# mp3guy/Kintinuous

Measured on AMD Instinct MI355X. Metric: RGB-D frames/sec @640x480, 512^3 TSDF, higher is better.
Workload: dtype f32; 1 GPU; orbit512: 640x480 synthetic orbit sequence, ICP-only tracking, 512^3 TSDF, inputs resident in HBM, 1 stream per GPU (BASELINE.json configs[1]), log playback with 1 frame of read-ahead; volume=512, cols=640, rows=480, unique_frames=120, pose_gather_bytes=56384, side_gate=0, odometry_fallbacks=0

## Files before the change

kintinuous_amd/abi.py:

```python
from __future__ import annotations

import ctypes as C
import os
from typing import Optional, Sequence, Tuple

import numpy as np

_HERE = os.path.dirname(os.path.abspath(__file__))
LIB_PATH = os.environ.get("KT_HIP_LIB") or os.path.join(_HERE, "libkt_hip.so")

KT_OK = 0
KT_ERR_CAPACITY = 5


class KtError(RuntimeError):
    def __init__(self, msg: str, status: int = 0):
        super().__init__(msg)
        self.status = status


class Intr(C.Structure):
    _fields_ = [("fx", C.c_float), ("fy", C.c_float), ("cx", C.c_float), ("cy", C.c_float)]

    def level(self, l: int) -> "Intr":
        d = np.float32(1 << l)
        return Intr(np.float32(self.fx) / d, np.float32(self.fy) / d, np.float32(self.cx) / d, np.float32(self.cy) / d)


class Mat33(C.Structure):
    _fields_ = [("m", C.c_float * 9)]

    @staticmethod
    def from_np(a) -> "Mat33":
        a = np.asarray(a, dtype=np.float32).reshape(9)
        return Mat33((C.c_float * 9)(*a.tolist()))


class LoopIcpInfo(C.Structure):
    _fields_ = [("n_source", C.c_int), ("n_target", C.c_int), ("iterations", C.c_int), ("converged", C.c_int)]


class LoopMatchParams(C.Structure):
    _fields_ = [("fast_threshold", C.c_int), ("max_keypoints", C.c_int), ("max_hamming", C.c_int), ("ratio_num", C.c_int), ("ratio_den", C.c_int),
                ("n_hypotheses", C.c_int), ("reproj_px", C.c_float), ("max_dist", C.c_float), ("seed", C.c_uint32)]


class LoopMatchInfo(C.Structure):
    _fields_ = [("n_kp_old", C.c_int), ("n_kp_new", C.c_int), ("n_matches", C.c_int), ("n_inliers", C.c_int), ("best_hypothesis", C.c_int)]


class JpegLayout(C.Structure):
    _fields_ = [("width", C.c_int32), ("height", C.c_int32), ("ncomp", C.c_int32), ("hmax", C.c_int32), ("vmax", C.c_int32),
                ("h", C.c_int32 * 3), ("v", C.c_int32 * 3), ("tq", C.c_int32 * 3), ("blocks_w", C.c_int32 * 3), ("blocks_h", C.c_int32 * 3),
                ("comp_width", C.c_int32 * 3), ("comp_height", C.c_int32 * 3), ("coef_offset", C.c_uint32 * 3), ("n_coef", C.c_uint32),
                ("qt", (C.c_uint16 * 64) * 4)]


class TrackerConfig(C.Structure):
    _fields_ = [
        ("cols", C.c_int), ("rows", C.c_int), ("N", C.c_int),
        ("fx", C.c_float), ("fy", C.c_float), ("cx", C.c_float), ("cy", C.c_float),
        ("volume_size", C.c_float), ("voxel_shift", C.c_int), ("overlap", C.c_int), ("static_mode", C.c_int),
        ("use_rgbd", C.c_int), ("use_rgbd_icp", C.c_int), ("fast_odometry", C.c_int), ("disable_color_angle", C.c_int),
        ("max_slice_points", C.c_int), ("dynamic_cube", C.c_int), ("place_recognition", C.c_int),
    ]


DATATERM_DTYPE = np.dtype([("zero", np.int16, 2), ("one", np.int16, 2), ("diff", np.float32), ("valid", np.uint8), ("pad", np.uint8, 3)])
POINT_DTYPE = np.dtype([("xyz", np.float32, 3), ("pad0", np.float32), ("bgra", np.uint8, 4), ("pad1", np.uint32, 3)])
MESH_VERTEX_DTYPE = np.dtype([("xyz", np.float32, 3), ("rgb", np.uint32)])
assert DATATERM_DTYPE.itemsize == 16 and POINT_DTYPE.itemsize == 32 and MESH_VERTEX_DTYPE.itemsize == 16

_vp, _i, _f, _d, _sz, _u64 = C.c_void_p, C.c_int, C.c_float, C.c_double, C.c_size_t, C.c_uint64
_pf = C.POINTER(C.c_float)
_pd = C.POINTER(C.c_double)
_pi = C.POINTER(C.c_int)
_pI = C.POINTER(Intr)
_pM = C.POINTER(Mat33)

_PROTOS = {
    "kt_last_error": (C.c_char_p, []),
    "kt_version": (C.c_char_p, []),
    "kt_device_count": (_i, [_pi]),
    "kt_ctx_create": (_i, [_i, C.POINTER(_vp)]),
    "kt_ctx_destroy": (_i, [_vp]),
    "kt_ctx_set_stream": (_i, [_vp, _vp]),
    "kt_ctx_stream": (_vp, [_vp]),
    "kt_sync": (_i, [_vp]),
    "kt_malloc": (_i, [_vp, _sz, C.POINTER(_vp)]),
    "kt_free": (_i, [_vp, _vp]),
    "kt_memset": (_i, [_vp, _vp, _i, _sz]),
    "kt_upload": (_i, [_vp, _vp, _vp, _sz]),
    "kt_download": (_i, [_vp, _vp, _vp, _sz]),
    "kt_upload2d": (_i, [_vp, _vp, _vp, _sz, _sz, _i]),
    "kt_download2d": (_i, [_vp, _vp, _sz, _vp, _sz, _i]),
    "kt_bilateral_filter": (_i, [_vp, _vp, _vp, _i, _i]),
    "kt_pyr_down": (_i, [_vp, _vp, _i, _i, _vp]),
    "kt_create_vmap": (_i, [_vp, _pI, _vp, _i, _i, _vp]),
    "kt_create_nmap": (_i, [_vp, _vp, _i, _i, _vp]),
    "kt_transform_maps": (_i, [_vp, _vp, _vp, _i, _i, _pM, _pf, _vp, _vp]),
    "kt_resize_vmap": (_i, [_vp, _vp, _i, _i, _vp]),
    "kt_resize_nmap": (_i, [_vp, _vp, _i, _i, _vp]),
    "kt_generate_image": (_i, [_vp, _vp, _vp, _vp, _i, _i, _pf, _i, _vp, _vp]),
    "kt_generate_depth": (_i, [_vp, _pM, _pf, _vp, _vp, _i, _i, _vp]),
    "kt_depth_to_metres": (_i, [_vp, _vp, _vp, _i, _i, _i]),
    "kt_bgr_to_intensity": (_i, [_vp, _vp, _vp, _i, _i]),
    "kt_pyr_down_gauss_f32": (_i, [_vp, _vp, _i, _i, _vp]),
    "kt_pyr_down_gauss_u8": (_i, [_vp, _vp, _i, _i, _vp]),
    "kt_derivative_images": (_i, [_vp, _vp, _i, _i, _vp, _vp]),
    "kt_project_to_cloud": (_i, [_vp, _vp, _i, _i, _vp, _d, _d, _d, _d, _i]),
    "kt_build_pyramid": (_i, [_vp, _pI, _vp, _i, _i, C.POINTER(_vp), C.POINTER(_vp), C.POINTER(_vp)]),
    "kt_icp_step": (_i, [_vp, _pM, _pf, _vp, _vp, _pM, _pf, _pI, _vp, _vp, _i, _i, _f, _f, _pf, _pf, _pf]),
    "kt_rgb_residual": (_i, [_vp, _f, _vp, _vp, _vp, _vp, _vp, _vp, _i, _i, _vp, _f, _pf, _pM, _pi, _pi]),
    "kt_rgb_step": (_i, [_vp, _vp, _f, _vp, _f, _f, _vp, _vp, _f, _i, _i, _pf, _pf]),
    "kt_init_volume": (_i, [_vp, _vp, _i]),
    "kt_init_color_volume": (_i, [_vp, _vp, _i]),
    "kt_icp_track": (_i, [_vp, C.POINTER(_vp), C.POINTER(_vp), C.POINTER(_vp), C.POINTER(_vp), _i, _i, _pI, _pM, _pf, _pi, _f, _f, _pM, _pf, _pf, _pf]),
    "kt_integrate_tsdf": (_i, [_vp, _vp, _i, _i, _pI, _pf, _pM, _pf, _f, _vp, _vp, _pi, _vp, _vp, _vp, _i, _i]),
    "kt_raycast": (_i, [_vp, _pI, _pM, _pf, _f, _pf, _vp, _vp, _vp, _i, _i, _pi, _vp, _vp, _i]),
    "kt_clear_volume": (_i, [_vp, _vp, _i, _i, _i, _i, _i, _i]),
    "kt_extract_cloud_slice": (_i, [_vp, _vp, _pf, _vp, _sz, _pi, _vp, _i, _i, _i, _i, _i, _i, _i, _pi, _i, C.POINTER(_sz)]),
    "kt_extract_mesh": (_i, [_vp, _vp, _pf, _pi, _vp, _pi, _pi, _pi, _i, _vp, _sz, _vp, _sz, C.POINTER(_sz), C.POINTER(_sz)]),
    "kt_tracker_create": (_i, [_vp, C.POINTER(TrackerConfig), C.POINTER(_vp)]),
    "kt_tracker_destroy": (_i, [_vp]),
    "kt_tracker_reset": (_i, [_vp]),
    "kt_tracker_process_frame": (_i, [_vp, _vp, _vp, _u64]),
    "kt_tracker_process_frame_host": (_i, [_vp, _vp, _vp, _u64]),
    "kt_tracker_load_trajectory": (_i, [_vp, _i, _vp, _vp]),
    "kt_tracker_finalise": (_i, [_vp]),
    "kt_tracker_get_volume_basis": (_i, [_vp, _pf]),
    "kt_host_reposition_cube": (None, [_pf, _pf, _f, _pf, _i, _pf]),
    "kt_tracker_get_pose": (_i, [_vp, _pf, _pf, _pf]),
    "kt_tracker_num_poses": (_i, [_vp]),
    "kt_tracker_get_dense_pose": (_i, [_vp, _i, C.POINTER(_u64), _pf, _pi]),
    "kt_tracker_get_voxel_wrap": (_i, [_vp, _pi]),
    "kt_tracker_num_slices": (_i, [_vp]),
    "kt_tracker_slice_info": (_i, [_vp, _i, C.POINTER(_sz), _pi]),
    "kt_tracker_slice_points": (_i, [_vp, _i, _vp]),
    "kt_tracker_volume": (_vp, [_vp]),
    "kt_tracker_color_volume": (_vp, [_vp]),
    "kt_tracker_vmap_g_prev": (_vp, [_vp, _i]),
    "kt_tracker_vmap_curr_color": (_vp, [_vp]),
    "kt_tracker_nmap_g_prev": (_vp, [_vp, _i]),
    "kt_tracker_trunc_dist": (_f, [_vp]),
    "kt_tracker_enable_profiling": (_i, [_vp, _i]),
    "kt_tracker_stage_ms": (_i, [_vp, _pf]),
    "kt_tracker_stage_counts": (_i, [_vp, C.POINTER(C.c_longlong)]),
    "kt_tracker_enable_counts": (_i, [_vp, _i]),
    "kt_tracker_last_counts": (_i, [_vp, C.POINTER(C.c_ulonglong), C.POINTER(C.c_ulonglong)]),
    "kt_tracker_debug_counts": (_i, [_vp, C.POINTER(C.c_uint)]),
    "kt_tracker_debug_state": (_i, [_vp, _pf]),
    "kt_tracker_debug_bricks": (_i, [_vp, _vp]),
    "kt_tracker_plan_stats": (_i, [_vp, C.POINTER(C.c_longlong)]),
    "kt_tracker_odometry_fallbacks": (_i, [_vp, C.POINTER(C.c_longlong)]),
    "kt_debug_wait_limit": (_i, [_vp, C.c_uint]),
    "kt_tracker_debug_side_gate": (_i, [_vp]),
    "kt_tracker_enable_slice_stage": (_i, [_vp, _i, _i, _i]),
    "kt_tracker_slice_processed_info": (_i, [_vp, _i, C.POINTER(C.c_longlong)]),
    "kt_tracker_slice_processed": (_i, [_vp, _i, _vp]),
    "kt_tracker_enable_mesh_stage": (_i, [_vp, _i, C.c_longlong, C.c_longlong]),
    "kt_tracker_slice_mesh_info": (_i, [_vp, _i, C.POINTER(C.c_longlong), C.POINTER(C.c_longlong)]),
    "kt_tracker_slice_mesh": (_i, [_vp, _i, _vp, _vp]),
    "kt_tracker_debug_pose_log": (_i, [_vp, _i, _pf, _i, C.POINTER(C.c_int)]),
    "kt_tracker_debug_plan_truth": (_i, [_vp, _pf, _i, C.c_float, C.c_float, C.c_float, C.c_float, C.c_uint]),
    "kt_debug_tsdf_lean": (_i, [_i]),
    "kt_debug_tsdf_kernel": (C.c_char_p, []),
    "kt_debug_tsdf_contract": (_i, [_i]),
    "kt_debug_tsdf_wcl": (_i, [_i]),
    "kt_debug_tsdf_wcl_pick": (_i, [_i, _i, _i, _i]),
    "kt_debug_sq_threshold": (_f, [_f, _i]),
    "kt_debug_icp_levels": (_i, [_i]),
    "kt_debug_ri_levels": (_i, [_i]),
    "kt_tracker_debug_icp_levels": (_i, [_vp]),
    "kt_debug_icp_wg_times": (_i, [_vp, C.POINTER(C.c_ulonglong)]),
    "kt_debug_tsdf_timeline": (_i, [_vp, C.POINTER(C.c_ulonglong), _i]),
    "kt_debug_solve_check": (_i, [_vp, _i, _vp, _vp, _vp, C.POINTER(_i)]),
    "kt_debug_unpack_table": (_i, [_vp, _pf]),
    "kt_debug_rcp_check": (_i, [_vp, C.POINTER(C.c_uint)]),
    "kt_debug_handoff_fault": (_i, [_vp, _i, _i, C.c_uint, C.POINTER(C.c_uint)]),
    "kt_tracker_num_pr_samples": (_i, [_vp]),
    "kt_tracker_pr_sample": (_i, [_vp, _i, C.POINTER(_u64), _pf, _pf, C.POINTER(C.c_int)]),
    "kt_tracker_slice_pr_id": (_i, [_vp, _i, C.POINTER(C.c_int)]),
    "kt_host_place_recognition_movement": (_f, [_pf, _pf, _pf, _pf]),
    "kt_slice_process": (_i, [_vp, _vp, _sz, _i, _f, _i, _vp, C.POINTER(_sz)]),
    "kt_slice_ws_create": (_i, [_vp, _sz, _vp, C.POINTER(_vp)]),
    "kt_slice_ws_destroy": (_i, [_vp]),
    "kt_slice_ws_stream": (_vp, [_vp]),
    "kt_slice_process_device": (_i, [_vp, _vp, _vp, _sz, _i, _f, _i]),
    "kt_slice_ws_count": (_i, [_vp, C.POINTER(_sz)]),
    "kt_slice_ws_output": (_vp, [_vp]),
    "kt_host_voxel_grid_normal": (_i, [_vp, _sz, _f, _vp, C.POINTER(_sz)]),
    "kt_host_save_pcd": (_i, [C.c_char_p, _vp, _sz]),
    "kt_host_save_ply": (_i, [C.c_char_p, _vp, _sz, _vp, _sz]),
    "kt_comm_unique_id": (_i, [C.POINTER(C.c_ubyte)]),
    "kt_comm_init": (_i, [_vp, _i, _i, C.POINTER(C.c_ubyte), C.POINTER(_vp)]),
    "kt_pose_gather": (_i, [_vp, _vp, _i, _pf]),
    "kt_comm_barrier": (_i, [_vp]),
    "kt_comm_destroy": (_i, [_vp]),
    "kt_tracker_host_times": (_i, [_vp, _pd, _i]),
    "kt_tracker_prefetch_frame": (_i, [_vp, _vp, _vp]),
    "kt_tracker_prefetch_frame_host": (_i, [_vp, _vp, _vp]),
    "kt_tracker_slice_pose": (_i, [_vp, _i, _pf, _pf, C.POINTER(_u64)]),
    "kt_tracker_set_parked": (_i, [_vp, _i]),
    "kt_host_ldlt_solve6": (_i, [_pd, _pd, _pd]),
    "kt_host_rodrigues": (_i, [_pd, _pd]),
    "kt_host_mat33_inverse": (_i, [_pf, _pf]),
    "kt_host_pose_update": (_i, [_pd, _pd, _pf, _pf, _pf, _pf]),
    "kt_host_compute_krk": (_i, [_pd, C.c_double, C.c_double, C.c_double, C.c_double, _pf, _pf]),
    "kt_host_trajectory_pose": (None, [_pf, _pf]),
    "kt_host_ground_truth_pose": (None, [_pf, _pf, _pf, _pf, _pf, _pf]),
    "kt_tracker_export_poses_device": (_i, [_vp, _i, _vp]),
    "kt_loop_icp_depth_frames": (_i, [_vp, _vp, _vp, _i, _i, _pI, _pf, _f, _f, _i, _pf, _pf, _vp]),
    "kt_depth_to_cloud_grid": (_i, [_vp, _vp, _i, _i, _pI, _f, _f, _vp, _sz, C.POINTER(_sz)]),
    "kt_cloud_nearest": (_i, [_vp, _vp, _sz, _vp, _sz, _vp, _vp]),
    "kt_host_rigid_fit": (_i, [_pd, _d, _pd]),
    "kt_loop_match_params_default": (_i, [_vp]),
    "kt_loop_match_frames": (_i, [_vp, _vp, _vp, _vp, _vp, _i, _i, _pI, _vp, _pf, _pf, _vp, _vp, _sz, _vp]),
    "kt_frame_keypoints": (_i, [_vp, _vp, _vp, _i, _i, _vp, _vp, _vp, _vp, _sz, C.POINTER(_sz)]),
    "kt_descriptor_match": (_i, [_vp, _vp, _sz, _vp, _sz, _vp, _vp, _vp, _vp]),
    "kt_host_jpeg_entropy_decode": (_i, [_vp, _sz, _i, _i, _vp, _vp, _sz, C.POINTER(_sz)]),
    "kt_jpeg_ws_create": (_i, [_vp, _i, _i, _vp, C.POINTER(_vp)]),
    "kt_jpeg_ws_destroy": (_i, [_vp]),
    "kt_jpeg_ws_stream": (_vp, [_vp]),
    "kt_jpeg_ws_order": (_i, [_vp, _vp]),
    "kt_jpeg_reconstruct": (_i, [_vp, _vp, _vp, _i, _vp]),
    "kt_jpeg_decode": (_i, [_vp, _vp, _sz, _i, _i, _i, _vp]),
}

ABI_SYMBOLS = tuple(_PROTOS.keys())

_MEASURE_PROTOS = {
    "kt_debug_stream": (_i, [_vp, _vp, _sz, _i, _i]),
    "kt_debug_stream_rows": (_i, [_vp, _vp, _i, _i, _i, _i, _i]),
    "kt_debug_valu_rates": (_i, [_vp, _i, _i, _i, _pd]),
    "kt_debug_div_check": (_i, [_vp, C.POINTER(C.c_uint)]),
    "kt_debug_brick_count": (_i, [_i]),
    "kt_debug_integrate_bricks": (_i, [_vp, _vp, _i, _i, _pI, _pf, _pM, _pf, _f, _vp, _vp, _pi, _vp, _vp, _vp, _i, _i, _vp]),
    "kt_debug_raycast_bricks": (_i, [_vp, _pI, _pM, _pf, _f, _pf, _vp, _vp, _vp, _i, _i, _pi, _vp, _vp, _i, _vp, C.POINTER(C.c_ulonglong)]),
}
MEASURE_SYMBOLS = tuple(_MEASURE_PROTOS.keys())
MEASURE_LIB_PATH = os.path.join(os.path.dirname(os.path.abspath(__file__)), "libkt_debug.so")
_mlib = None


def measure_lib() -> C.CDLL:
    global _mlib
    if _mlib is None:
        lib()
        if not os.path.exists(MEASURE_LIB_PATH):
            raise KtError(f"{MEASURE_LIB_PATH} not found: run `python -c 'import __graft_entry__ as g; g.build()'` first")
        l = C.CDLL(MEASURE_LIB_PATH, mode=C.RTLD_GLOBAL)
        for name, (res, args) in _MEASURE_PROTOS.items():
            f = getattr(l, name)
            f.restype, f.argtypes = res, args
        _mlib = l
    return _mlib

_lib = None


def lib() -> C.CDLL:
    global _lib
    if _lib is None:
        if not os.path.exists(LIB_PATH):
            raise KtError(f"{LIB_PATH} not found: run `python -c 'import __graft_entry__ as g; g.build()'` first")
        l = C.CDLL(LIB_PATH, mode=C.RTLD_GLOBAL)
        for name, (res, args) in _PROTOS.items():
            if name.startswith("kt_debug_") and os.environ.get("KT_HIP_LIB") and not hasattr(l, name):
                continue
            fn = getattr(l, name)
            fn.restype = res
            fn.argtypes = args
        _lib = l
    return _lib


def _chk(status: int) -> None:
    if status != KT_OK:
        raise KtError(f"kt status {status}: {lib().kt_last_error().decode(errors='replace')}", status)


def _fp(a) -> "C.Array":
    a = np.ascontiguousarray(a, dtype=np.float32).reshape(-1)
    return (C.c_float * a.size)(*a.tolist())


def _ip(a) -> "C.Array":
    a = np.ascontiguousarray(a, dtype=np.int32).reshape(-1)
    return (C.c_int * a.size)(*a.tolist())


def _count(n: int) -> int:
    if n < 0:
        raise KtError(lib().kt_last_error().decode() or "tracker error")
    return n


class DevBuf:

    def __init__(self, ctx: "Ctx", nbytes: int, ptr: Optional[int] = None):
        self.ctx, self.nbytes = ctx, int(nbytes)
        self.owned = ptr is None
        if ptr is None:
            p = _vp()
            _chk(lib().kt_malloc(ctx.h, self.nbytes, C.byref(p)))
            ptr = p.value
        self.ptr = ptr

    def free(self) -> None:
        if self.owned and self.ptr:
            lib().kt_free(self.ctx.h, self.ptr)
            self.ptr = None

    def __del__(self):
        try:
            self.free()
        except Exception:
            pass


class Ctx:

    def __init__(self, device: int = 0):
        h = _vp()
        _chk(lib().kt_ctx_create(device, C.byref(h)))
        self.h = h
        self.device = device

    def close(self) -> None:
        if self.h:
            lib().kt_ctx_destroy(self.h)
            self.h = None

    def sync(self) -> None:
        _chk(lib().kt_sync(self.h))

    def empty(self, nbytes: int) -> DevBuf:
        return DevBuf(self, nbytes)

    def zeros(self, nbytes: int) -> DevBuf:
        b = DevBuf(self, nbytes)
        _chk(lib().kt_memset(self.h, b.ptr, 0, nbytes))
        return b

    def upload(self, a: np.ndarray, into: Optional[DevBuf] = None) -> DevBuf:
        a = np.ascontiguousarray(a)
        b = into if into is not None else DevBuf(self, a.nbytes)
        _chk(lib().kt_upload(self.h, b.ptr, a.ctypes.data, a.nbytes))
        return b

    def download(self, b, dtype, shape) -> np.ndarray:
        out = np.empty(shape, dtype=dtype)
        ptr = b.ptr if isinstance(b, DevBuf) else int(b)
        _chk(lib().kt_download(self.h, out.ctypes.data, ptr, out.nbytes))
        return out

    def bilateral_filter(self, src: DevBuf, dst: DevBuf, cols: int, rows: int) -> None:
        _chk(lib().kt_bilateral_filter(self.h, src.ptr, dst.ptr, cols, rows))

    def pyr_down(self, src: DevBuf, scols: int, srows: int, dst: DevBuf) -> None:
        _chk(lib().kt_pyr_down(self.h, src.ptr, scols, srows, dst.ptr))

    def create_vmap(self, intr: Intr, depth: DevBuf, cols: int, rows: int, vmap: DevBuf) -> None:
        _chk(lib().kt_create_vmap(self.h, C.byref(intr), depth.ptr, cols, rows, vmap.ptr))

    def create_nmap(self, vmap: DevBuf, cols: int, rows: int, nmap: DevBuf) -> None:
        _chk(lib().kt_create_nmap(self.h, vmap.ptr, cols, rows, nmap.ptr))

    def transform_maps(self, vs, ns, cols, rows, R, t, vd, nd) -> None:
        _chk(lib().kt_transform_maps(self.h, vs.ptr, ns.ptr, cols, rows, C.byref(Mat33.from_np(R)), _fp(t), vd.ptr, nd.ptr))

    def resize_vmap(self, src, in_cols, in_rows, dst) -> None:
        _chk(lib().kt_resize_vmap(self.h, src.ptr, in_cols, in_rows, dst.ptr))

    def resize_nmap(self, src, in_cols, in_rows, dst) -> None:
        _chk(lib().kt_resize_nmap(self.h, src.ptr, in_cols, in_rows, dst.ptr))

    def generate_image(self, vmap, nmap, vmap_color, cols, rows, light_pos, light_number, dst, dst_color) -> None:
        _chk(lib().kt_generate_image(self.h, vmap.ptr, nmap.ptr, vmap_color.ptr, cols, rows, _fp(light_pos), light_number, dst.ptr, dst_color.ptr))

    def generate_depth(self, R_inv, t, vmap, nmap, cols, rows, dst) -> None:
        _chk(lib().kt_generate_depth(self.h, C.byref(Mat33.from_np(R_inv)), _fp(t), vmap.ptr, nmap.ptr, cols, rows, dst.ptr))

    def depth_to_metres(self, src, dst, cols, rows, cutoff) -> None:
        _chk(lib().kt_depth_to_metres(self.h, src.ptr, dst.ptr, cols, rows, cutoff))

    def bgr_to_intensity(self, src, dst, cols, rows) -> None:
        _chk(lib().kt_bgr_to_intensity(self.h, src.ptr, dst.ptr, cols, rows))

    def pyr_down_gauss_f32(self, src, scols, srows, dst) -> None:
        _chk(lib().kt_pyr_down_gauss_f32(self.h, src.ptr, scols, srows, dst.ptr))

    def pyr_down_gauss_u8(self, src, scols, srows, dst) -> None:
        _chk(lib().kt_pyr_down_gauss_u8(self.h, src.ptr, scols, srows, dst.ptr))

    def derivative_images(self, src, cols, rows, dx, dy) -> None:
        _chk(lib().kt_derivative_images(self.h, src.ptr, cols, rows, dx.ptr, dy.ptr))

    def project_to_cloud(self, depth, cols, rows, cloud, fx, fy, cx, cy, level) -> None:
        _chk(lib().kt_project_to_cloud(self.h, depth.ptr, cols, rows, cloud.ptr, fx, fy, cx, cy, level))

    def build_pyramid(self, intr: Intr, depth0, cols, rows, depths_out, vmaps, nmaps) -> None:
        d = (_vp * 3)(*[b.ptr for b in depths_out])
        v = (_vp * 4)(*[b.ptr for b in vmaps])
        n = (_vp * 4)(*[b.ptr for b in nmaps])
        _chk(lib().kt_build_pyramid(self.h, C.byref(intr), depth0.ptr, cols, rows, d, v, n))

    def icp_step(self, Rcurr, tcurr, vmap_curr, nmap_curr, Rprev_inv, tprev, intr: Intr, vmap_g_prev, nmap_g_prev, cols, rows,
                 dist_thres, angle_thres) -> Tuple[np.ndarray, np.ndarray, np.ndarray]:
        A = (C.c_float * 36)()
        b = (C.c_float * 6)()
        r = (C.c_float * 2)()
        _chk(lib().kt_icp_step(self.h, C.byref(Mat33.from_np(Rcurr)), _fp(tcurr), vmap_curr.ptr, nmap_curr.ptr,
                               C.byref(Mat33.from_np(Rprev_inv)), _fp(tprev), C.byref(intr), vmap_g_prev.ptr, nmap_g_prev.ptr,
                               cols, rows, dist_thres, angle_thres, A, b, r))
        return (np.array(A, dtype=np.float32).reshape(6, 6), np.array(b, dtype=np.float32), np.array(r, dtype=np.float32))

    def icp_track(self, vmaps_curr, nmaps_curr, vmaps_g_prev, nmaps_g_prev, cols, rows, intr: Intr, Rprev, tprev, iterations,
                  dist_thres, angle_thres):
        def arr(bufs):
            return (_vp * 4)(*[(b.ptr if b is not None else None) for b in bufs])
        Rc = Mat33()
        tc, A, r = (C.c_float * 3)(), (C.c_float * 36)(), (C.c_float * 2)()
        it = (C.c_int * 4)(*[int(v) for v in iterations])
        _chk(lib().kt_icp_track(self.h, arr(vmaps_curr), arr(nmaps_curr), arr(vmaps_g_prev), arr(nmaps_g_prev), cols, rows, C.byref(intr),
                                C.byref(Mat33.from_np(Rprev)), _fp(tprev), it, dist_thres, angle_thres, C.byref(Rc), tc, A, r))
        return (np.array(Rc.m, np.float32).reshape(3, 3), np.array(tc, np.float32), np.array(A, np.float32).reshape(6, 6), np.array(r, np.float32))

    def rgb_residual(self, min_scale, dIdx, dIdy, last_depth, next_depth, last_image, next_image, cols, rows, corres,
                     max_depth_delta, kt, krkinv) -> Tuple[int, int]:
        sigma, count = C.c_int(0), C.c_int(0)
        _chk(lib().kt_rgb_residual(self.h, min_scale, dIdx.ptr, dIdy.ptr, last_depth.ptr, next_depth.ptr, last_image.ptr,
                                   next_image.ptr, cols, rows, corres.ptr, max_depth_delta, _fp(kt),
                                   C.byref(Mat33.from_np(krkinv)), C.byref(sigma), C.byref(count)))
        return sigma.value, count.value

    def rgb_step(self, corres, sigma, cloud, fx, fy, dIdx, dIdy, sobel_scale, cols, rows) -> Tuple[np.ndarray, np.ndarray]:
        A = (C.c_float * 36)()
        b = (C.c_float * 6)()
        _chk(lib().kt_rgb_step(self.h, corres.ptr, sigma, cloud.ptr, fx, fy, dIdx.ptr, dIdy.ptr, sobel_scale, cols, rows, A, b))
        return np.array(A, dtype=np.float32).reshape(6, 6), np.array(b, dtype=np.float32)

    def init_volume(self, vol: DevBuf, N: int) -> None:
        _chk(lib().kt_init_volume(self.h, vol.ptr, N))

    def init_color_volume(self, cvol: DevBuf, N: int) -> None:
        _chk(lib().kt_init_color_volume(self.h, cvol.ptr, N))

    def integrate_tsdf(self, depth, cols, rows, intr: Intr, volume_size, Rcurr_inv, tcurr, tranc_dist, volume, depth_scaled,
                       voxel_wrap, color_volume, colors, nmap_curr, angle_color, N) -> None:
        _chk(lib().kt_integrate_tsdf(self.h, depth.ptr, cols, rows, C.byref(intr), _fp(volume_size), C.byref(Mat33.from_np(Rcurr_inv)),
                                     _fp(tcurr), tranc_dist, volume.ptr, depth_scaled.ptr, _ip(voxel_wrap), color_volume.ptr,
                                     colors.ptr, nmap_curr.ptr, int(angle_color), N))

    def raycast(self, intr: Intr, Rcurr, tcurr, tranc_dist, volume_size, volume, vmap, nmap, cols, rows, voxel_wrap, vmap_color,
                color_volume, N) -> None:
        _chk(lib().kt_raycast(self.h, C.byref(intr), C.byref(Mat33.from_np(Rcurr)), _fp(tcurr), tranc_dist, _fp(volume_size),
                              volume.ptr, vmap.ptr, nmap.ptr, cols, rows, _ip(voxel_wrap), vmap_color.ptr, color_volume.ptr, N))

    def integrate_tsdf_bricks(self, depth, cols, rows, intr: Intr, volume_size, Rcurr_inv, tcurr, tranc_dist, volume, depth_scaled,
                              voxel_wrap, color_volume, colors, nmap_curr, angle_color, N, bricks) -> None:
        _chk(measure_lib().kt_debug_integrate_bricks(self.h, depth.ptr, cols, rows, C.byref(intr), _fp(volume_size), C.byref(Mat33.from_np(Rcurr_inv)),
                                                     _fp(tcurr), tranc_dist, volume.ptr, depth_scaled.ptr, _ip(voxel_wrap), color_volume.ptr,
                                                     colors.ptr, nmap_curr.ptr, int(angle_color), N, bricks.ptr if bricks is not None else None))

    def raycast_bricks(self, intr: Intr, Rcurr, tcurr, tranc_dist, volume_size, volume, vmap, nmap, cols, rows, voxel_wrap, vmap_color,
                       color_volume, N, bricks) -> Tuple[int, int, int, int]:
        counts = (C.c_ulonglong * 4)()
        _chk(measure_lib().kt_debug_raycast_bricks(self.h, C.byref(intr), C.byref(Mat33.from_np(Rcurr)), _fp(tcurr), tranc_dist, _fp(volume_size),
                                                   volume.ptr, vmap.ptr, nmap.ptr, cols, rows, _ip(voxel_wrap), vmap_color.ptr, color_volume.ptr, N,
                                                   bricks.ptr if bricks is not None else None, counts))
        return tuple(int(v) for v in counts)

    def clear_volume(self, vol, elem_size, N, axis, back, current_wrap, delta_wrap) -> None:
        _chk(lib().kt_clear_volume(self.h, vol.ptr, elem_size, N, axis, int(back), current_wrap, delta_wrap))

    def extract_cloud_slice(self, volume, volume_size, out: DevBuf, cap: int, voxel_wrap, color_volume, minX, maxX, minY, maxY,
                            minZ, maxZ, subsample, real_voxel_wrap, N) -> int:
        n = _sz(0)
        _chk(lib().kt_extract_cloud_slice(self.h, volume.ptr, _fp(volume_size), out.ptr, cap, _ip(voxel_wrap), color_volume.ptr,
                                          minX, maxX, minY, maxY, minZ, maxZ, subsample, _ip(real_voxel_wrap), N, C.byref(n)))
        return int(n.value)

    def extract_mesh(self, volume, volume_size, voxel_wrap, color_volume, lo, hi, real_voxel_wrap, N, vertices=None, v_cap: int = 0,
                     triangles=None, t_cap: int = 0):
        nv, nt = _sz(0), _sz(0)
        vp = vertices.ptr if isinstance(vertices, DevBuf) else vertices
        tp = triangles.ptr if isinstance(triangles, DevBuf) else triangles
        vol = volume.ptr if isinstance(volume, DevBuf) else volume
        col = color_volume.ptr if isinstance(color_volume, DevBuf) else color_volume
        s = lib().kt_extract_mesh(self.h, vol, _fp(volume_size), _ip(voxel_wrap), col, _ip(lo), _ip(hi), _ip(real_voxel_wrap), N, vp,
                                  v_cap, tp, t_cap, C.byref(nv), C.byref(nt))
        if s not in (KT_OK, KT_ERR_CAPACITY):
            _chk(s)
        return s, int(nv.value), int(nt.value)

    def mesh(self, volume, volume_size, voxel_wrap, color_volume, lo, hi, real_voxel_wrap, N):
        s, nv, nt = self.extract_mesh(volume, volume_size, voxel_wrap, color_volume, lo, hi, real_voxel_wrap, N)
        vb = DevBuf(self, max(nv, 1) * 16)
        tb = DevBuf(self, max(nt, 1) * 12)
        try:
            s, nv2, nt2 = self.extract_mesh(volume, volume_size, voxel_wrap, color_volume, lo, hi, real_voxel_wrap, N, vb, nv, tb, nt)
            _chk(s)
            assert (nv2, nt2) == (nv, nt)
            v = np.zeros(max(nv, 1), MESH_VERTEX_DTYPE)
            t = np.zeros((max(nt, 1), 3), np.uint32)
            _chk(lib().kt_download(self.h, v.ctypes.data_as(C.c_void_p), vb.ptr, nv * 16))
            _chk(lib().kt_download(self.h, t.ctypes.data_as(C.c_void_p), tb.ptr, nt * 12))
        finally:
            vb.free()
            tb.free()
        return v[:nv], t[:nt]


    def depth_to_cloud_grid(self, frame: np.ndarray, intr: Intr, leaf: float, max_dist: float = 4.0, capacity: Optional[int] = None, out=None):
        frame = np.ascontiguousarray(frame, np.uint16)
        rows, cols = frame.shape
        cap = rows * cols if capacity is None else int(capacity)
        buf = out if out is not None else np.zeros((max(cap, 1), 3), np.float32)
        n = _sz(0)
        s = lib().kt_depth_to_cloud_grid(self.h, frame.ctypes.data, cols, rows, C.byref(intr), float(leaf), float(max_dist), buf.ctypes.data, cap, C.byref(n))
        if s not in (KT_OK, KT_ERR_CAPACITY):
            _chk(s)
        return s, (buf[: n.value] if s == KT_OK else None), int(n.value)

    def cloud_nearest(self, src: np.ndarray, dst: np.ndarray):
        src = np.ascontiguousarray(src, np.float32).reshape(-1, 3)
        dst = np.ascontiguousarray(dst, np.float32).reshape(-1, 3)
        idx, d2 = np.zeros(max(len(src), 1), np.uint32), np.zeros(max(len(src), 1), np.float32)
        _chk(lib().kt_cloud_nearest(self.h, src.ctypes.data, len(src), dst.ctypes.data, len(dst), idx.ctypes.data, d2.ctypes.data))
        return idx[: len(src)], d2[: len(src)]

    def loop_icp_depth_frames(self, frame1: np.ndarray, frame2: np.ndarray, intr: Intr, bootstrap, leaf: float, max_dist: float = 4.0,
                              max_iterations: int = 10):
        frame1, frame2 = np.ascontiguousarray(frame1, np.uint16), np.ascontiguousarray(frame2, np.uint16)
        assert frame1.shape == frame2.shape and frame1.ndim == 2
        rows, cols = frame1.shape
        M, score, info = (C.c_float * 16)(), C.c_float(0), LoopIcpInfo()
        _chk(lib().kt_loop_icp_depth_frames(self.h, frame1.ctypes.data, frame2.ctypes.data, cols, rows, C.byref(intr), _fp(np.asarray(bootstrap).reshape(16)),
                                            float(leaf), float(max_dist), int(max_iterations), M, C.byref(score), C.byref(info)))
        return (np.array(M, np.float32).reshape(4, 4), float(score.value),
                dict(n_source=info.n_source, n_target=info.n_target, iterations=info.iterations, converged=bool(info.converged)))

    def frame_keypoints(self, rgb: np.ndarray, depth: np.ndarray, params: Optional[LoopMatchParams] = None, capacity: Optional[int] = None):
        params = params or loop_match_params()
        depth = np.ascontiguousarray(depth, np.uint16)
        rows, cols = depth.shape
        rgb = np.ascontiguousarray(rgb, np.uint8).reshape(rows, cols, 3)
        cap = params.max_keypoints if capacity is None else int(capacity)
        uv, score, desc = np.full((max(cap, 1), 2), -7, np.int32), np.full(max(cap, 1), -7, np.int32), np.full((max(cap, 1), 8), 7, np.uint32)
        n = _sz(0)
        s = lib().kt_frame_keypoints(self.h, rgb.ctypes.data, depth.ctypes.data, cols, rows, C.byref(params), uv.ctypes.data, score.ctypes.data, desc.ctypes.data,
                                     cap, C.byref(n))
        if s not in (KT_OK, KT_ERR_CAPACITY):
            _chk(s)
        if s == KT_ERR_CAPACITY:
            assert (uv == -7).all() and (score == -7).all() and (desc == 7).all()
            return s, None, int(n.value)
        return s, (uv[: n.value], score[: n.value], desc[: n.value]), int(n.value)

    def descriptor_match(self, desc_new: np.ndarray, desc_old: np.ndarray, params: Optional[LoopMatchParams] = None):
        params = params or loop_match_params()
        dn = np.ascontiguousarray(desc_new, np.uint32).reshape(-1, 8)
        do = np.ascontiguousarray(desc_old, np.uint32).reshape(-1, 8)
        idx, d1, d2 = (np.zeros(max(len(dn), 1), np.int32) for _ in range(3))
        _chk(lib().kt_descriptor_match(self.h, dn.ctypes.data, len(dn), do.ctypes.data, len(do), C.byref(params), idx.ctypes.data, d1.ctypes.data, d2.ctypes.data))
        return idx[: len(dn)], d1[: len(dn)], d2[: len(dn)]

    def loop_match_frames(self, rgb_old, depth_old, rgb_new, depth_new, intr: Intr, params: Optional[LoopMatchParams] = None):
        params = params or loop_match_params()
        depth_old, depth_new = np.ascontiguousarray(depth_old, np.uint16), np.ascontiguousarray(depth_new, np.uint16)
        assert depth_old.shape == depth_new.shape and depth_old.ndim == 2
        rows, cols = depth_old.shape
        rgb_old, rgb_new = (np.ascontiguousarray(a, np.uint8).reshape(rows, cols, 3) for a in (rgb_old, rgb_new))
        cap = params.max_keypoints
        pose, boot, info = (C.c_float * 16)(), (C.c_float * 16)(), LoopMatchInfo()
        matches, inlier = np.zeros((cap, 4), np.int32), np.zeros(cap, np.uint8)
        _chk(lib().kt_loop_match_frames(self.h, rgb_old.ctypes.data, depth_old.ctypes.data, rgb_new.ctypes.data, depth_new.ctypes.data, cols, rows, C.byref(intr),
                                        C.byref(params), pose, boot, matches.ctypes.data, inlier.ctypes.data, cap, C.byref(info)))
        n = info.n_matches
        return dict(pose=np.array(pose, np.float32).reshape(4, 4), bootstrap=np.array(boot, np.float32).reshape(4, 4), matches=matches[:n].copy(),
                    inlier=inlier[:n].astype(bool), info={k: int(getattr(info, k)) for k, _ in LoopMatchInfo._fields_})


def loop_match_params(**kw) -> LoopMatchParams:
    p = LoopMatchParams()
    _chk(lib().kt_loop_match_params_default(C.byref(p)))
    for k, v in kw.items():
        assert hasattr(p, k), k
        setattr(p, k, v)
    return p


class Tracker:

    STAGES = ("pyramid", "odometry", "shift", "integrate", "raycast", "resize", "tsdf23")

    def __init__(self, ctx: Ctx, cfg: TrackerConfig):
        self.ctx, self.cfg = ctx, cfg
        h = _vp()
        _chk(lib().kt_tracker_create(ctx.h, C.byref(cfg), C.byref(h)))
        self.h = h

    def close(self) -> None:
        if self.h:
            lib().kt_tracker_destroy(self.h)
            self.h = None

    def __del__(self):
        try:
            self.close()
        except Exception:
            pass

    def reset(self) -> None:
        _chk(lib().kt_tracker_reset(self.h))

    def process_frame(self, depth_dev, rgb_dev, timestamp: int) -> None:
        d = depth_dev.ptr if isinstance(depth_dev, DevBuf) else int(depth_dev)
        r = rgb_dev.ptr if isinstance(rgb_dev, DevBuf) else int(rgb_dev)
        _chk(lib().kt_tracker_process_frame(self.h, d, r, timestamp))

    def host_times(self, reset: bool = False):
        o = (C.c_double * 2)()
        _chk(lib().kt_tracker_host_times(self.h, o, 1 if reset else 0))
        return float(o[0]), float(o[1])

    def enable_slice_stage(self, on: bool, weight_cull: int = 8, k: int = 20) -> None:
        _chk(lib().kt_tracker_enable_slice_stage(self.h, int(on), int(weight_cull), int(k)))

    def slice_processed(self, i: int):
        n = C.c_longlong(0)
        _chk(lib().kt_tracker_slice_processed_info(self.h, i, C.byref(n)))
        if n.value < 0:
            return None
        out = np.zeros(max(int(n.value), 1), NPOINT_DTYPE)
        _chk(lib().kt_tracker_slice_processed(self.h, i, out.ctypes.data_as(C.c_void_p)))
        return out[: int(n.value)]

    def enable_mesh_stage(self, on: bool, max_vertices: int = 0, max_triangles: int = 0) -> None:
        _chk(lib().kt_tracker_enable_mesh_stage(self.h, int(on), int(max_vertices), int(max_triangles)))

    def slice_mesh_info(self, i: int):
        nv, nt = C.c_longlong(0), C.c_longlong(0)
        _chk(lib().kt_tracker_slice_mesh_info(self.h, i, C.byref(nv), C.byref(nt)))
        return int(nv.value), int(nt.value)

    def slice_mesh(self, i: int):
        nv, nt = self.slice_mesh_info(i)
        if nv < 0:
            return None
        v = np.zeros(max(nv, 1), MESH_VERTEX_DTYPE)
        t = np.zeros((max(nt, 1), 3), np.uint32)
        _chk(lib().kt_tracker_slice_mesh(self.h, i, v.ctypes.data_as(C.c_void_p), t.ctypes.data_as(C.c_void_p)))
        return v[:nv], t[:nt]

    def pose_log(self, enable: Optional[bool] = None, fetch: bool = False):
        if not fetch:
            _chk(lib().kt_tracker_debug_pose_log(self.h, -1 if enable is None else int(enable), None, 0, None))
            return None
        n = C.c_int(0)
        _chk(lib().kt_tracker_debug_pose_log(self.h, -1 if enable is None else int(enable), None, 0, C.byref(n)))
        out = np.zeros((n.value, 12), np.float32)
        if n.value:
            _chk(lib().kt_tracker_debug_pose_log(self.h, -1, out.ctypes.data_as(_pf), n.value, None))
        return out

    def plan_truth(self, poses12, fr: float, ft: float, theta_fixed: float = 0.0, tau_fixed: float = 0.0, seed: int = 1) -> None:
        p = np.ascontiguousarray(poses12, np.float32).reshape(-1, 12)
        _chk(lib().kt_tracker_debug_plan_truth(self.h, p.ctypes.data_as(_pf), len(p), fr, ft, theta_fixed, tau_fixed, seed))

    def plan_stats(self) -> Tuple[int, int]:
        out = (C.c_longlong * 2)()
        _chk(lib().kt_tracker_plan_stats(self.h, out))
        return int(out[0]), int(out[1])

    def odometry_fallbacks(self) -> int:
        out = C.c_longlong(0)
        _chk(lib().kt_tracker_odometry_fallbacks(self.h, C.byref(out)))
        return int(out.value)

    def prefetch_frame(self, depth_dev, rgb_dev) -> None:
        d = depth_dev.ptr if isinstance(depth_dev, DevBuf) else int(depth_dev)
        r = rgb_dev.ptr if isinstance(rgb_dev, DevBuf) else int(rgb_dev)
        _chk(lib().kt_tracker_prefetch_frame(self.h, d, r))

    def prefetch_frame_host(self, depth: np.ndarray, rgb: np.ndarray) -> None:
        assert depth.dtype == np.uint16 and rgb.dtype == np.uint8 and depth.flags.c_contiguous and rgb.flags.c_contiguous
        _chk(lib().kt_tracker_prefetch_frame_host(self.h, depth.ctypes.data, rgb.ctypes.data))

    def process_frame_host(self, depth: np.ndarray, rgb: np.ndarray, timestamp: int) -> None:
        depth = np.ascontiguousarray(depth, dtype=np.uint16)
        rgb = np.ascontiguousarray(rgb, dtype=np.uint8)
        _chk(lib().kt_tracker_process_frame_host(self.h, depth.ctypes.data, rgb.ctypes.data, timestamp))

    def load_trajectory(self, utimes, pose7) -> None:
        utimes = np.ascontiguousarray(utimes, dtype=np.uint64)
        pose7 = np.ascontiguousarray(pose7, dtype=np.float32).reshape(-1, 7)
        assert len(utimes) == len(pose7)
        _chk(lib().kt_tracker_load_trajectory(self.h, len(utimes), utimes.ctypes.data, pose7.ctypes.data))

    def finalise(self) -> None:
        _chk(lib().kt_tracker_finalise(self.h))

    def volume_basis(self) -> np.ndarray:
        b = (C.c_float * 3)()
        _chk(lib().kt_tracker_get_volume_basis(self.h, b))
        return np.array(b, dtype=np.float32)

    def pose(self) -> Tuple[np.ndarray, np.ndarray, np.ndarray]:
        R, t, g = (C.c_float * 9)(), (C.c_float * 3)(), (C.c_float * 3)()
        _chk(lib().kt_tracker_get_pose(self.h, R, t, g))
        return np.array(R, dtype=np.float32).reshape(3, 3), np.array(t, dtype=np.float32), np.array(g, dtype=np.float32)

    def num_poses(self) -> int:
        return _count(lib().kt_tracker_num_poses(self.h))

    def dense_pose(self, i: int) -> Tuple[int, np.ndarray, bool]:
        ts, p, il = _u64(0), (C.c_float * 16)(), C.c_int(0)
        _chk(lib().kt_tracker_get_dense_pose(self.h, i, C.byref(ts), p, C.byref(il)))
        return ts.value, np.array(p, dtype=np.float32).reshape(4, 4), bool(il.value)

    def voxel_wrap(self) -> np.ndarray:
        w = (C.c_int * 3)()
        _chk(lib().kt_tracker_get_voxel_wrap(self.h, w))
        return np.array(w, dtype=np.int32)

    def num_slices(self) -> int:
        return _count(lib().kt_tracker_num_slices(self.h))

    def slice_info(self, i: int) -> Tuple[int, int]:
        n, dim = _sz(0), C.c_int(0)
        _chk(lib().kt_tracker_slice_info(self.h, i, C.byref(n), C.byref(dim)))
        return n.value, dim.value

    def slice(self, i: int) -> Tuple[np.ndarray, int]:
        n, dim = _sz(0), C.c_int(0)
        _chk(lib().kt_tracker_slice_info(self.h, i, C.byref(n), C.byref(dim)))
        out = np.zeros(n.value, dtype=POINT_DTYPE)
        if n.value:
            _chk(lib().kt_tracker_slice_points(self.h, i, out.ctypes.data))
        return out, dim.value

    def pr_samples(self):
        out = []
        for i in range(_count(lib().kt_tracker_num_pr_samples(self.h))):
            ut, tr, ro, pi = _u64(0), (C.c_float * 3)(), (C.c_float * 9)(), C.c_int(0)
            _chk(lib().kt_tracker_pr_sample(self.h, i, C.byref(ut), tr, ro, C.byref(pi)))
            out.append((ut.value, np.array(tr, np.float32), np.array(ro, np.float32).reshape(3, 3), pi.value))
        return out

    def slice_pr_id(self, i: int) -> int:
        v = C.c_int(0)
        _chk(lib().kt_tracker_slice_pr_id(self.h, i, C.byref(v)))
        return v.value

    def volume(self) -> np.ndarray:
        N = self.cfg.N
        return self.ctx.download(lib().kt_tracker_volume(self.h), np.int16, (N, N, N))

    def color_volume(self) -> np.ndarray:
        N = self.cfg.N
        return self.ctx.download(lib().kt_tracker_color_volume(self.h), np.uint8, (N, N, N, 4))

    def vmap_g_prev(self, level: int = 0) -> np.ndarray:
        c, r = self.cfg.cols >> level, self.cfg.rows >> level
        return self.ctx.download(lib().kt_tracker_vmap_g_prev(self.h, level), np.float32, (3 * r, c))

    def nmap_g_prev(self, level: int = 0) -> np.ndarray:
        c, r = self.cfg.cols >> level, self.cfg.rows >> level
        return self.ctx.download(lib().kt_tracker_nmap_g_prev(self.h, level), np.float32, (3 * r, c))

    def trunc_dist(self) -> float:
        return float(lib().kt_tracker_trunc_dist(self.h))

    def enable_profiling(self, mode: int) -> None:
        _chk(lib().kt_tracker_enable_profiling(self.h, mode))

    def stage_ms(self) -> dict:
        ms = (C.c_float * 7)()
        n = (C.c_longlong * 7)()
        _chk(lib().kt_tracker_stage_ms(self.h, ms))
        _chk(lib().kt_tracker_stage_counts(self.h, n))
        return {k: (float(ms[i]), int(n[i])) for i, k in enumerate(self.STAGES)}

    def enable_counts(self, on: bool) -> None:
        _chk(lib().kt_tracker_enable_counts(self.h, int(on)))

    def last_counts(self) -> Tuple[int, int]:
        U, S = C.c_ulonglong(0), C.c_ulonglong(0)
        _chk(lib().kt_tracker_last_counts(self.h, C.byref(U), C.byref(S)))
        return int(U.value), int(S.value)

    def debug_state(self):
        o = (C.c_float * 29)()
        _chk(lib().kt_tracker_debug_state(self.h, o))
        return [float(v) for v in o]

    def debug_bricks(self) -> np.ndarray:
        nb = (self.cfg.N + 31) // 32
        out = np.zeros((nb, nb, nb), np.uint8)
        _chk(lib().kt_tracker_debug_bricks(self.h, out.ctypes.data))
        return out

    def debug_counts(self):
        o = (C.c_uint * 8)()
        _chk(lib().kt_tracker_debug_counts(self.h, o))
        return [int(v) for v in o]

    def export_poses_device(self, k: int, dst_ptr: int) -> None:
        _chk(lib().kt_tracker_export_poses_device(self.h, k, dst_ptr))


def _dp(a):
    return a.ctypes.data_as(_pd)


def host_ldlt_solve6(A, b) -> np.ndarray:
    A = np.ascontiguousarray(A, np.float64).reshape(36)
    b = np.ascontiguousarray(b, np.float64).reshape(6)
    x = np.zeros(6, np.float64)
    _chk(lib().kt_host_ldlt_solve6(_dp(A), _dp(b), _dp(x)))
    return x


def host_rodrigues(r) -> np.ndarray:
    r = np.ascontiguousarray(r, np.float64).reshape(3)
    R = np.zeros(9, np.float64)
    _chk(lib().kt_host_rodrigues(_dp(r), _dp(R)))
    return R.reshape(3, 3)


def host_mat33_inverse(m) -> np.ndarray:
    m = np.ascontiguousarray(m, np.float32).reshape(9)
    o = np.zeros(9, np.float32)
    _chk(lib().kt_host_mat33_inverse(m.ctypes.data_as(_pf), o.ctypes.data_as(_pf)))
    return o.reshape(3, 3)


def host_reposition_cube(R, tlast, volume_size, voxel_size, thresh, basis) -> np.ndarray:
    R = np.ascontiguousarray(R, np.float32).reshape(9)
    t = np.ascontiguousarray(tlast, np.float32)
    v = np.ascontiguousarray(voxel_size, np.float32)
    b = np.ascontiguousarray(basis, np.float32).copy()
    lib().kt_host_reposition_cube(R.ctypes.data_as(_pf), t.ctypes.data_as(_pf), float(volume_size), v.ctypes.data_as(_pf), int(thresh), b.ctypes.data_as(_pf))
    return b


def host_pose_update(x, result_rt, Rprev, tprev):
    x = np.ascontiguousarray(x, np.float64).reshape(6)
    rt = np.array(result_rt, np.float64).reshape(16).copy()
    Rp = np.ascontiguousarray(Rprev, np.float32).reshape(9)
    tp = np.ascontiguousarray(tprev, np.float32).reshape(3)
    Rc, tc = np.zeros(9, np.float32), np.zeros(3, np.float32)
    _chk(lib().kt_host_pose_update(_dp(x), _dp(rt), Rp.ctypes.data_as(_pf), tp.ctypes.data_as(_pf),
                                   Rc.ctypes.data_as(_pf), tc.ctypes.data_as(_pf)))
    return rt.reshape(4, 4), Rc.reshape(3, 3), tc


def host_rigid_fit(sums, n) -> np.ndarray:
    sums = np.ascontiguousarray(sums, np.float64).reshape(15)
    dM = np.zeros(16, np.float64)
    _chk(lib().kt_host_rigid_fit(_dp(sums), float(n), _dp(dM)))
    return dM.reshape(4, 4)


NPOINT_DTYPE = np.dtype([("xyz", np.float32, 3), ("one", np.float32), ("normal", np.float32, 3), ("zero", np.float32), ("bgra", np.uint8, 4),
                         ("curvature", np.float32), ("pad", np.float32, 2)])
assert NPOINT_DTYPE.itemsize == 48


def host_compute_krk(result_rt, fx, fy, cx, cy):
    rt = np.ascontiguousarray(result_rt, np.float64).reshape(16)
    krk, kt = np.zeros(9, np.float32), np.zeros(3, np.float32)
    _chk(lib().kt_host_compute_krk(_dp(rt), float(fx), float(fy), float(cx), float(cy), krk.ctypes.data_as(_pf), kt.ctypes.data_as(_pf)))
    return krk.reshape(3, 3), kt


def host_trajectory_pose(pose7) -> np.ndarray:
    p = np.ascontiguousarray(pose7, np.float32).reshape(7)
    T = np.zeros(12, np.float32)
    lib().kt_host_trajectory_pose(p.ctypes.data_as(_pf), T.ctypes.data_as(_pf))
    return T


def host_ground_truth_pose(A, B, Rlast, tlast):
    A, B = np.ascontiguousarray(A, np.float32).reshape(12), np.ascontiguousarray(B, np.float32).reshape(12)
    Rl, tl = np.ascontiguousarray(Rlast, np.float32).reshape(9), np.ascontiguousarray(tlast, np.float32).reshape(3)
    R, t = np.zeros(9, np.float32), np.zeros(3, np.float32)
    lib().kt_host_ground_truth_pose(A.ctypes.data_as(_pf), B.ctypes.data_as(_pf), Rl.ctypes.data_as(_pf), tl.ctypes.data_as(_pf),
                                    R.ctypes.data_as(_pf), t.ctypes.data_as(_pf))
    return R.reshape(3, 3), t


def slice_process(ctx: "Ctx", points: np.ndarray, weight_cull: int, leaf: float, k: int = 20) -> np.ndarray:
    points = np.ascontiguousarray(points)
    assert points.dtype == POINT_DTYPE
    out = np.zeros(max(len(points), 1), NPOINT_DTYPE)
    n = C.c_size_t(0)
    _chk(lib().kt_slice_process(ctx.h, points.ctypes.data_as(C.c_void_p), len(points), int(weight_cull), float(leaf), int(k),
                                out.ctypes.data_as(C.c_void_p), C.byref(n)))
    return out[: n.value]


def voxel_grid_normal(points: np.ndarray, leaf: float) -> np.ndarray:
    points = np.ascontiguousarray(points)
    assert points.dtype == NPOINT_DTYPE
    out = np.zeros(max(len(points), 1), NPOINT_DTYPE)
    n = C.c_size_t(0)
    _chk(lib().kt_host_voxel_grid_normal(points.ctypes.data_as(C.c_void_p), len(points), float(leaf), out.ctypes.data_as(C.c_void_p), C.byref(n)))
    return out[: n.value]


def save_pcd(path: str, points: np.ndarray) -> None:
    points = np.ascontiguousarray(points)
    assert points.dtype == NPOINT_DTYPE
    _chk(lib().kt_host_save_pcd(path.encode(), points.ctypes.data_as(C.c_void_p), len(points)))


def save_ply(path: str, meshes) -> None:
    if isinstance(meshes, tuple) and len(meshes) == 2 and isinstance(meshes[0], np.ndarray) and meshes[0].dtype == MESH_VERTEX_DTYPE:
        meshes = [meshes]
    vs, ts, off = [], [], 0
    for v, t in meshes:
        vs.append(np.asarray(v, MESH_VERTEX_DTYPE))
        ts.append(np.asarray(t, np.uint32).reshape(-1, 3) + np.uint32(off))
        off += len(v)
    v = np.ascontiguousarray(np.concatenate(vs) if vs else np.zeros(0, MESH_VERTEX_DTYPE))
    t = np.ascontiguousarray(np.concatenate(ts) if ts else np.zeros((0, 3), np.uint32))
    _chk(lib().kt_host_save_ply(path.encode(), v.ctypes.data_as(C.c_void_p), len(v), t.ctypes.data_as(C.c_void_p), len(t)))


class Comm:

    def __init__(self, ctx: Ctx, rank: int, nranks: int, share=None):
        ident = (C.c_ubyte * 128)()
        if rank == 0:
            _chk(lib().kt_comm_unique_id(ident))
        if share is not None:
            data = share(bytes(ident))
            ident = (C.c_ubyte * 128)(*data)
        self.h = C.c_void_p()
        self.nranks = nranks
        _chk(lib().kt_comm_init(ctx.h, rank, nranks, ident, C.byref(self.h)))

    def gather_poses(self, trk: "Tracker", k: int) -> np.ndarray:
        out = np.zeros((self.nranks, k, 16), np.float32)
        _chk(lib().kt_pose_gather(self.h, trk.h, k, out.ctypes.data_as(C.POINTER(C.c_float))))
        return out

    def barrier(self) -> None:
        _chk(lib().kt_comm_barrier(self.h))

    def close(self) -> None:
        if self.h:
            lib().kt_comm_destroy(self.h)
            self.h = None


def jpeg_entropy_decode(data: bytes, width: int, height: int, capacity: Optional[int] = None) -> Tuple[JpegLayout, np.ndarray]:
    if capacity is None:
        capacity = 3 * (-(-width // 16) * 16) * (-(-height // 16) * 16)
    layout, coef, n = JpegLayout(), np.zeros(max(capacity, 1), np.int16), _sz(0)
    buf = np.frombuffer(data, np.uint8)
    _chk(lib().kt_host_jpeg_entropy_decode(buf.ctypes.data, buf.size, width, height, C.addressof(layout), coef.ctypes.data, capacity, C.byref(n)))
    return layout, coef[:n.value]


class JpegWs:

    def __init__(self, ctx: "Ctx", max_width: int, max_height: int):
        self.ctx = ctx
        h = _vp()
        _chk(lib().kt_jpeg_ws_create(ctx.h, max_width, max_height, None, C.byref(h)))
        self.h = h

    def close(self) -> None:
        if self.h:
            lib().kt_jpeg_ws_destroy(self.h)
            self.h = None

    def sync(self) -> None:
        _chk(lib().kt_jpeg_ws_order(self.h, lib().kt_ctx_stream(self.ctx.h)))
        self.ctx.sync()

    def reconstruct(self, layout: JpegLayout, coef: np.ndarray, swap_rb: int = 0, out: Optional[DevBuf] = None) -> np.ndarray:
        coef = np.ascontiguousarray(coef, np.int16)
        n = 3 * layout.width * layout.height
        buf = out if out is not None else self.ctx.empty(n)
        _chk(lib().kt_jpeg_reconstruct(self.h, C.addressof(layout), coef.ctypes.data, swap_rb, buf.ptr))
        self.sync()
        res = self.ctx.download(buf, np.uint8, (layout.height, layout.width, 3))
        if out is None:
            buf.free()
        return res

    def decode(self, data: bytes, width: int, height: int, swap_rb: int = 0, out: Optional[DevBuf] = None) -> np.ndarray:
        src = np.frombuffer(data, np.uint8)
        buf = out if out is not None else self.ctx.empty(3 * width * height)
        try:
            _chk(lib().kt_jpeg_decode(self.h, src.ctypes.data, src.size, width, height, swap_rb, buf.ptr))
            return self.ctx.download(buf, np.uint8, (height, width, 3))
        finally:
            if out is None:
                buf.free()
```

kintinuous_amd/csrc/kt_debug.h:

```cpp
#ifndef KT_DEBUG_H
#define KT_DEBUG_H

#include "../../include/kt_abi.h"

#ifdef __cplusplus
extern "C" {
#endif

int kt_tracker_debug_counts(kt_tracker* t, unsigned int out8_host[8]);
int kt_tracker_debug_state(kt_tracker* t, float out29_host[29]);
int kt_tracker_debug_bricks(kt_tracker* t, unsigned char* out_host);
int kt_tracker_debug_pose_log(kt_tracker* trk, int enable, float* out12n, int max_frames, int* n_frames);
int kt_tracker_debug_plan_truth(kt_tracker* trk, const float* poses12n, int n_frames, float fr, float ft, float theta_fixed, float tau_fixed, unsigned int seed);
int kt_debug_tsdf_lean(int on);
int kt_debug_tsdf_contract(int tol);
int kt_debug_tsdf_wcl(int wcl);
int kt_debug_tsdf_wcl_pick(int cols, int rows, int N, int rule);
const char* kt_debug_tsdf_kernel(void);
int kt_debug_icp_wg_times(kt_ctx* ctx, unsigned long long* out768_host);
int kt_debug_tsdf_timeline(kt_ctx* ctx, unsigned long long* out_host, int max_words);
int kt_debug_solve_check(kt_ctx* ctx, int n, const void* cases_host, void* serial_out_host, void* wave_out_host, int layout_out[5]);
int kt_debug_unpack_table(kt_ctx* ctx, float* out_host65536);
int kt_debug_rcp_check(kt_ctx* ctx, unsigned int* mismatches_host);
int kt_debug_handoff_fault(kt_ctx* ctx, int skip, int count, unsigned int spin_limit, unsigned int* dirty_out);
int kt_debug_wait_limit(kt_ctx* ctx, unsigned int ticks_100mhz);
int kt_debug_icp_levels(int on);
int kt_debug_ri_levels(int on);
int kt_tracker_debug_icp_levels(kt_tracker* trk);
int kt_tracker_debug_side_gate(kt_tracker* trk);
float kt_debug_sq_threshold(float T, int strict);

#ifdef __cplusplus
}
#endif

#endif
```

kintinuous_amd/csrc/kt_tracker.hip:

```cpp
#include "kt_internal.hpp"
#include "kt_setup.hpp"

#include <limits.h>
#include <stdlib.h>
#include <string.h>

#include <array>
#include <deque>
#include <chrono>
#include <condition_variable>
#include <functional>
#include <mutex>
#include <atomic>
#include <map>
#include <thread>
#include <vector>

namespace {

struct DensePose { uint64_t ts; float pose[16]; int is_loop; };
struct Slice {
    std::vector<kt_point_xyzrgb> pts; int dim; float R[9], cam[3]; uint64_t ts; int pr_id;
    std::vector<kt_point_xyzrgbnormal> processed; bool has_processed = false;
    std::vector<kt_mesh_vertex> mesh_v; std::vector<uint32_t> mesh_t; long long mesh_nv = -1, mesh_nt = -1; bool mesh_fit = false;
};
struct PrSample { uint64_t utime; float trans[3], rot[9]; int pose_index; };

struct FrameSet {
    uint16_t* depths[KT_LEVELS];
    float *vmaps[KT_LEVELS], *nmaps[KT_LEVELS];
    void* rec;
    float* dpmax;
    float* scaled;
    float* depth_m[KT_LEVELS];
    uint8_t* image[KT_LEVELS];
    int16_t *dIdx[KT_LEVELS], *dIdy[KT_LEVELS];
    uint8_t* cand[KT_LEVELS];
    float* cloud[KT_LEVELS];
    hipEvent_t ready;
    long long user;
};
#define KT_NSETS 3

typedef kt_pose_mirror PoseMirror;
struct Pending { const uint16_t* depth; const uint8_t* rgb; int set; const uint16_t* depth_host; const uint8_t* rgb_host; };
#define KT_NSLOTS 4
#define KT_NODO 8

#ifndef KT_SIDE_GATE_DEFAULT
#define KT_SIDE_GATE_DEFAULT 2
#endif
enum { ST_PYRAMID = 0, ST_ODOMETRY, ST_SHIFT, ST_INTEGRATE, ST_RAYCAST, ST_RESIZE, ST_TSDF23, ST_COUNT };

}

static std::atomic<int> kt_live_trackers{0};
struct kt_tracker {
    kt_ctx* ctx;
    kt_tracker_config cfg;
    kt_intr intr;
    int N;
    float volume_size[3], voxel_size[3];
    float tranc_dist;
    float volume_basis[3];
    float initial_rotation[9];
    int voxel_wrap[3], v_wrap_copy[3];
    int global_time;
    uint64_t current_ts = 0;
    bool has_trajectory = false;
    std::map<int, std::array<float, 12>> trajectory;
    uint64_t gt_utime = 0;
    bool parked;
    float Rlast[9], tlast[3];
    float current_global_camera[3];
    int16_t* tsdf; uint8_t* color;
    uint16_t* depths_curr[KT_LEVELS];
    float *vmaps_curr[KT_LEVELS], *nmaps_curr[KT_LEVELS], *vmaps_g_prev[KT_LEVELS], *nmaps_g_prev[KT_LEVELS];
    uint8_t* vmap_curr_color;
    float* depth_raw_scaled;
    void* rec_curr;
    FrameSet sets[KT_NSETS];
    int last_assigned;
    std::vector<Pending> pending;
    long long frames_started;
    long long frames_observed;
    long long out_ordinal;
    hipEvent_t guard_ev;
    hipEvent_t odo_ev[8];
    long long slot_frame[KT_NSLOTS];
    hipStream_t pre_stream;
    kt_ctx pre_ctx;
    size_t cloud_cap;
    int prev_set;
    kt_dataterm* corres[KT_LEVELS];
    kt_track_state* state_dev; kt_track_state* state_host;
    uint16_t* depth_stage[KT_NSLOTS]; uint8_t* rgb_stage[KT_NSLOTS];
    uint16_t* depth_stage_host[KT_NSLOTS]; uint8_t* rgb_stage_host[KT_NSLOTS];
    hipEvent_t slot_uploaded[KT_NSLOTS];
    int next_slot;
    std::vector<DensePose> poses;
    std::deque<Slice> slices;
    struct SliceJob { bool active; bool done; size_t slice; hipError_t status; };
    SliceJob jobs[2];
    std::thread worker;
    std::mutex wmu;
    std::condition_variable wcv, wdone;
    std::deque<std::function<void()>> wq;
    bool wstop;
    kt_point_xyzrgb* cloud_host[2]; unsigned int* cloud_count_host[2]; hipEvent_t cloud_ev[2];
    int cloud_next;
    bool slice_stage; int slice_cull, slice_k;
    kt_slice_ws* slice_ws;
    kt_point_xyzrgb* cloud_dev[2]; unsigned int* cloud_count_dev[2]; hipEvent_t extracted[2];
    kt_point_xyzrgbnormal* proc_host[2]; unsigned int* proc_count_host[2];
    bool mesh_stage; size_t mesh_cap_v, mesh_cap_t;
    kt_mesh_ws* mesh_ws;
    kt_mesh_vertex* mesh_v_host[2]; uint32_t* mesh_t_host[2]; unsigned long long* mesh_count_host[2]; hipEvent_t mesh_ev[2];
    float pr_rot[9], pr_trans[3];
    std::vector<PrSample> pr_samples;
    bool outstanding; uint64_t out_ts; int out_set;
    const uint16_t* out_depth; const uint8_t* out_rgb; int out_thresh;
    bool out_speculated;
    kt_frame_params* fp_dev;
    float* wrkc_carry[2]; int carry_sel;
    struct PlanSlot { kt_tsdf_plan plan; hipEvent_t done; long long ordinal; float R[9], t[3], theta, tau; int wrap[3]; int set; const uint16_t* depth; const uint8_t* rgb; };
    bool icp_levels;
    bool last_icp_levels;
    bool counted;
    int icp_demote, icp_demote_len;
    long long odo_fallbacks;
    int out_last_set;
    hipEvent_t gate_ev; bool gate_armed; int side_gate;
    PlanSlot plans[3]; hipStream_t plan_stream;
    int plan_sel; bool plan_enabled; float plan_margin_scale;
    std::vector<float> plan_truth; float plan_fr = 0.0f, plan_ft = 0.0f, plan_theta_fixed = 0.0f, plan_tau_fixed = 0.0f; bool plan_perturb = false;
    unsigned int plan_rng = 0x9e3779b9u; std::vector<float> pose_log; bool pose_log_on = false;
    float hist_R[2][9], hist_gc[2][3]; int hist_n;
    float pred_err_t, pred_err_r;
    long long plan_hits, plan_misses;
    unsigned char* bricks;
    float *vgz_dev, *zs_dev;
    PoseMirror* mirror;
    unsigned int frame_seq;
    long long prof_frames;
    double host_wait_s, host_call_s; long long host_calls;
    int profiling; int ev_par;
    hipEvent_t ev[2][ST_COUNT][2]; bool ev_rec[2][ST_COUNT];
    double stage_ms_sum[ST_COUNT]; long long stage_n[ST_COUNT]; float stage_ms_last[ST_COUNT];
    int counting;
    unsigned int* upd_dev; unsigned long long* steps_dev;
    unsigned long long last_U, last_S;
};

static int join_slice_jobs(kt_tracker* t);
static int plan_frame(kt_tracker* t, const struct Pending& frame, long long ordinal);
static int lvl_cols(const kt_tracker* t, int l) { return t->cfg.cols >> l; }
static int lvl_rows(const kt_tracker* t, int l) { return t->cfg.rows >> l; }
static kt_intr lvl_intr(kt_intr k, int l)
{
    const int div = 1 << l;
    kt_intr r = {k.fx / div, k.fy / div, k.cx / div, k.cy / div};
    return r;
}


static thread_local hipStream_t g_alloc_stream = nullptr;
template <typename T>
static int dev_alloc(T** p, size_t count, bool zero)
{
    KT_HIP(hipMalloc((void**)p, (count ? count : 1) * sizeof(T)));
    if (zero) KT_HIP(hipMemsetAsync(*p, 0, (count ? count : 1) * sizeof(T), g_alloc_stream));
    return KT_OK;
}

static void select_set(kt_tracker* t, int q)
{
    for (int l = 0; l < KT_LEVELS; ++l) {
        t->depths_curr[l] = t->sets[q].depths[l];
        t->vmaps_curr[l] = t->sets[q].vmaps[l];
        t->nmaps_curr[l] = t->sets[q].nmaps[l];
    }
    t->depth_raw_scaled = t->sets[q].scaled;
    t->rec_curr = t->sets[q].rec;
}

static int pick_free_set(kt_tracker* t)
{
    for (int k = 1; k <= KT_NSETS; ++k) {
        const int q = (t->last_assigned + k) % KT_NSETS;
        bool taken = q == t->prev_set;
        for (const Pending& p : t->pending) taken = taken || p.set == q;
        if (!taken) return q;
    }
    return -1;
}

#ifndef KT_EV_DEVICE
#define KT_EV_DEVICE (hipEventDisableTiming | hipEventDisableSystemFence)
#endif

static int wait_frame_consumed(kt_tracker* t, hipStream_t stream, long long u)
{
    if (u < 0 || stream == t->ctx->stream) return KT_OK;
    if (u + 2 <= t->frames_observed) return KT_OK;
    if (t->has_trajectory && u + 1 < t->frames_started) {
        KT_HIP(hipStreamWaitEvent(stream, t->odo_ev[(u + 1) % KT_NODO], 0));
    } else {
        KT_HIP(hipEventRecord(t->guard_ev, t->ctx->stream));
        KT_HIP(hipStreamWaitEvent(stream, t->guard_ev, 0));
    }
    return KT_OK;
}

static float rgbd_min_scale(int l)
{
    const float min_grad[KT_LEVELS] = {12, 5, 3, 1};
    const double SOBEL_SCALE = 1.0 / pow(2.0, 3);
    return (float)(pow(min_grad[l], 2.0) / pow(SOBEL_SCALE, 2.0));
}

static int build_frame_set(kt_tracker* t, kt_ctx* cx, int q, const uint16_t* depth_raw, const uint8_t* colors)
{
    const int cols = t->cfg.cols, rows = t->cfg.rows;
    FrameSet& fs = t->sets[q];
    const bool icp = !t->has_trajectory && !(t->cfg.use_rgbd || t->cfg.use_rgbd_icp);
    const bool rgbd = !t->has_trajectory && !icp;
    static const bool fused_prepare = []() { const char* e = getenv("KT_PREPARE_FUSED"); return e ? atoi(e) != 0 : true; }();
    if (icp || t->cfg.use_rgbd_icp || !t->cfg.disable_color_angle) {
        KT_TRY(kt_bilateral_filter(cx, depth_raw, fs.depths[0], cols, rows));
        uint16_t* dl[3] = {fs.depths[1], fs.depths[2], fs.depths[3]};
        if (fused_prepare)
            KT_TRY(kt_frame_prepare(cx, &t->intr, fs.depths[0], dl, fs.vmaps, fs.nmaps, depth_raw, colors, cols, rows, !t->cfg.disable_color_angle, fs.scaled, fs.rec, fs.dpmax));
        else {
            KT_TRY(kt_build_pyramid(cx, &t->intr, fs.depths[0], cols, rows, dl, fs.vmaps, fs.nmaps));
            KT_TRY(kt_integrate_prepare(cx, depth_raw, colors, fs.nmaps[0], cols, rows, &t->intr, !t->cfg.disable_color_angle, fs.scaled, fs.rec, fs.dpmax));
        }
    } else
        KT_TRY(kt_integrate_prepare(cx, depth_raw, colors, fs.nmaps[0], cols, rows, &t->intr, !t->cfg.disable_color_angle, fs.scaled, fs.rec, fs.dpmax));
    if (rgbd) {
        KT_TRY(kt_depth_to_metres(cx, depth_raw, fs.depth_m[0], cols, rows, (int)(6.0 * 1000)));
        for (int l = 0; l + 1 < KT_LEVELS; ++l) KT_TRY(kt_pyr_down_gauss_f32(cx, fs.depth_m[l], lvl_cols(t, l), lvl_rows(t, l), fs.depth_m[l + 1]));
        KT_TRY(kt_bgr_to_intensity(cx, colors, fs.image[0], cols, rows));
        for (int l = 0; l + 1 < KT_LEVELS; ++l) KT_TRY(kt_pyr_down_gauss_u8(cx, fs.image[l], lvl_cols(t, l), lvl_rows(t, l), fs.image[l + 1]));
        const double ifx = t->intr.fx, ify = t->intr.fy, icx = t->intr.cx, icy = t->intr.cy;
        for (int l = 0; l < KT_LEVELS; ++l) {
            KT_TRY(kt_derivative_images(cx, fs.image[l], lvl_cols(t, l), lvl_rows(t, l), fs.dIdx[l], fs.dIdy[l]));
            KT_TRY(kt_rgb_residual_candidates(cx, rgbd_min_scale(l), fs.dIdx[l], fs.dIdy[l], fs.depth_m[l], fs.image[l], lvl_cols(t, l),
                                              lvl_rows(t, l), fs.cand[l]));
            KT_TRY(kt_project_to_cloud(cx, fs.depth_m[l], lvl_cols(t, l), lvl_rows(t, l), fs.cloud[l], ifx, ify, icx, icy, l));
        }
    }
    return KT_OK;
}

static void compute_global_camera(kt_tracker* t, const float* tcurr)
{
    for (int k = 0; k < 3; ++k) {
        const float initial_trans = (float)((double)t->volume_basis[k] - (double)t->cfg.volume_size * 0.5);
        t->current_global_camera[k] = initial_trans;
        t->current_global_camera[k] += (float)t->voxel_wrap[k] * t->voxel_size[k];
        if (tcurr) t->current_global_camera[k] += tcurr[k] - t->volume_basis[k];
    }
}

static void v_wrap_copy_update(kt_tracker* t)
{
    for (int k = 0; k < 3; ++k) {
        t->v_wrap_copy[k] = t->voxel_wrap[k];
        if (t->v_wrap_copy[k] < 0) t->v_wrap_copy[k] = t->N - ((-t->v_wrap_copy[k]) % t->N);
    }
}

static void push_pose(kt_tracker* t, uint64_t ts, const float* R, int is_loop)
{
    DensePose p;
    p.ts = ts;
    p.is_loop = is_loop;
    for (int i = 0; i < 16; ++i) p.pose[i] = (i % 5 == 0) ? 1.f : 0.f;
    for (int i = 0; i < 3; ++i) {
        for (int j = 0; j < 3; ++j) p.pose[i * 4 + j] = R[i * 3 + j];
        p.pose[i * 4 + 3] = t->current_global_camera[i];
    }
    t->poses.push_back(p);
}

static bool prof_all(const kt_tracker* t) { return t->profiling == 2 || t->profiling == 3; }
static bool prof_tsdf(const kt_tracker* t) { return t->profiling == 1 || t->profiling == 4 || t->profiling == 5 || t->profiling == 6; }
static int ev_begin(kt_tracker* t, int st)
{
    if (prof_all(t) || (prof_tsdf(t) && st == ST_TSDF23)) {
        KT_HIP(hipEventRecord(t->ev[t->ev_par][st][0], t->ctx->stream));
    }
    return KT_OK;
}
static int ev_end(kt_tracker* t, int st)
{
    if (prof_all(t) || (prof_tsdf(t) && st == ST_TSDF23)) {
        KT_HIP(hipEventRecord(t->ev[t->ev_par][st][1], t->ctx->stream));
        t->ev_rec[t->ev_par][st] = true;
    }
    return KT_OK;
}
static void tsdf23_hook_arm(kt_tracker* t)
{
    kt_tsdf23_hook.on = prof_all(t) || t->profiling == 4 || (t->profiling == 1 && (t->prof_frames++ % 8) == 0) || (t->profiling == 5 && (t->prof_frames++ % 4) == 0) ||
                        (t->profiling == 6 && (t->prof_frames++ % 2) == 0);
    kt_tsdf23_hook.ev[0] = t->ev[t->ev_par][ST_TSDF23][0];
    kt_tsdf23_hook.ev[1] = t->ev[t->ev_par][ST_TSDF23][1];
    if (kt_tsdf23_hook.on) t->ev_rec[t->ev_par][ST_TSDF23] = true;
}
static void ev_collect(kt_tracker* t)
{
    if (!t->profiling) return;
    for (int par = 0; par < 2; ++par)
        for (int st = 0; st < ST_COUNT; ++st)
            if (t->ev_rec[par][st] && hipEventQuery(t->ev[par][st][1]) == hipSuccess) {
                float ms = 0.f;
                if (hipEventElapsedTime(&ms, t->ev[par][st][0], t->ev[par][st][1]) == hipSuccess) {
                    t->stage_ms_sum[st] += ms;
                    t->stage_n[st] += 1;
                    t->stage_ms_last[st] = ms;
                }
                t->ev_rec[par][st] = false;
            }
}

extern "C" {

static int tracker_create_impl(kt_tracker* t, kt_ctx* ctx, const kt_tracker_config* cfg);

int kt_tracker_create(kt_ctx* ctx, const kt_tracker_config* cfg, kt_tracker** out)
{
    KT_ARG(ctx && cfg && out);
    KT_ARG(cfg->cols > 0 && cfg->rows > 0 && cfg->N > 0 && cfg->volume_size > 0);
    KT_ARG((cfg->cols % 8) == 0 && (cfg->rows % 8) == 0);
    KT_ARG(cfg->N <= 1536);
    KT_HIP(hipSetDevice(ctx->device));
    kt_tracker* t = new kt_tracker();
    const int s = tracker_create_impl(t, ctx, cfg);
    if (s != KT_OK) {
        t->ctx = ctx;
        (void)kt_tracker_destroy(t);
        return s;
    }
    *out = t;
    return KT_OK;
}

static int tracker_create_impl(kt_tracker* t, kt_ctx* ctx, const kt_tracker_config* cfg)
{
    t->ctx = ctx;
    g_alloc_stream = ctx->stream;
    t->cfg = *cfg;
    t->N = cfg->N;
    t->intr.fx = cfg->fx; t->intr.fy = cfg->fy; t->intr.cx = cfg->cx; t->intr.cy = cfg->cy;
    for (int k = 0; k < 3; ++k) {
        t->volume_size[k] = cfg->volume_size;
        t->voxel_size[k] = cfg->volume_size / (float)cfg->N;
    }
    for (int k = 0; k < 9; ++k) t->initial_rotation[k] = (k % 4 == 0) ? 1.f : 0.f;
    for (int k = 0; k < 3; ++k) t->volume_basis[k] = t->volume_size[k] * 0.5f;
    if (cfg->static_mode || cfg->dynamic_cube)
        t->volume_basis[2] = t->volume_size[2] * 0.5f - (float)(((double)t->volume_size[2] * 0.5) + (cfg->static_mode ? 0.45 : 0));
    const float default_tranc = fmaxf(0.01f, t->volume_size[0] / 100.0f);
    const float mc = fmaxf(t->voxel_size[0], fmaxf(t->voxel_size[1], t->voxel_size[2]));
    t->tranc_dist = fmaxf(default_tranc, 2.1f * mc);
    t->voxel_wrap[0] = t->voxel_wrap[1] = t->voxel_wrap[2] = 0;

    const size_t nvox = (size_t)cfg->N * cfg->N * cfg->N;
    const size_t P = (size_t)cfg->cols * cfg->rows;
    KT_TRY(dev_alloc(&t->tsdf, nvox, false));
    KT_TRY(dev_alloc(&t->color, nvox * 4, false));
    for (int l = 0; l < KT_LEVELS; ++l) {
        const size_t p = (size_t)lvl_cols(t, l) * lvl_rows(t, l);
        for (int q = 0; q < KT_NSETS; ++q) {
            KT_TRY(dev_alloc(&t->sets[q].depths[l], p, true));
            KT_TRY(dev_alloc(&t->sets[q].vmaps[l], 3 * p, true));
            KT_TRY(dev_alloc(&t->sets[q].nmaps[l], 3 * p, true));
        }
        KT_TRY(dev_alloc(&t->vmaps_g_prev[l], 3 * p, true));
        KT_TRY(dev_alloc(&t->nmaps_g_prev[l], 3 * p, true));
        const bool rgbd = cfg->use_rgbd || cfg->use_rgbd_icp;
        const size_t q = rgbd ? p : 0;
        for (int sidx = 0; sidx < KT_NSETS; ++sidx) {
            KT_TRY(dev_alloc(&t->sets[sidx].depth_m[l], q, true));
            KT_TRY(dev_alloc(&t->sets[sidx].image[l], q, true));
            KT_TRY(dev_alloc(&t->sets[sidx].dIdx[l], q, true));
            KT_TRY(dev_alloc(&t->sets[sidx].dIdy[l], q, true));
            KT_TRY(dev_alloc(&t->sets[sidx].cand[l], q, true));
            KT_TRY(dev_alloc(&t->sets[sidx].cloud[l], 3 * q, true));
        }
        KT_TRY(dev_alloc(&t->corres[l], q, true));
    }
    KT_TRY(dev_alloc(&t->vmap_curr_color, P * 4, true));
    for (int q = 0; q < KT_NSETS; ++q) {
        KT_TRY(dev_alloc(&t->sets[q].scaled, P, true));
        unsigned char* rec = nullptr;
        KT_TRY(dev_alloc(&rec, kt_integrate_rec_bytes(cfg->cols, cfg->rows), true));
        t->sets[q].rec = rec;
        unsigned char* dpm = nullptr;
        KT_TRY(dev_alloc(&dpm, kt_integrate_dpmax_bytes(cfg->cols, cfg->rows), true));
        t->sets[q].dpmax = (float*)dpm;
        KT_HIP(hipEventCreateWithFlags(&t->sets[q].ready, KT_EV_DEVICE));
        t->sets[q].user = -1;
    }
    t->frames_started = 0;
    t->cloud_next = 0;
    t->slice_stage = false; t->slice_ws = nullptr;
    t->mesh_stage = false; t->mesh_ws = nullptr; t->mesh_cap_v = t->mesh_cap_t = 0;
    for (int b = 0; b < 2; ++b) { t->mesh_v_host[b] = nullptr; t->mesh_t_host[b] = nullptr; t->mesh_count_host[b] = nullptr; t->mesh_ev[b] = nullptr; }
    for (int b = 0; b < 2; ++b) { t->cloud_dev[b] = nullptr; t->cloud_count_dev[b] = nullptr; t->extracted[b] = nullptr; t->proc_host[b] = nullptr; t->proc_count_host[b] = nullptr; }
    for (int b = 0; b < 2; ++b) { t->jobs[b].active = false; t->jobs[b].done = true; t->jobs[b].status = hipSuccess; t->cloud_host[b] = nullptr; t->cloud_count_host[b] = nullptr; t->cloud_ev[b] = nullptr; }
    t->wstop = false;
    {
        const int device = ctx->device;
        t->worker = std::thread([t, device]() {
            (void)hipSetDevice(device);
            std::unique_lock<std::mutex> lk(t->wmu);
            for (;;) {
                t->wcv.wait(lk, [t]() { return t->wstop || !t->wq.empty(); });
                if (t->wq.empty()) return;
                std::function<void()> job = std::move(t->wq.front());
                t->wq.pop_front();
                lk.unlock();
                job();
                lk.lock();
                t->wdone.notify_all();
            }
        });
    }
    t->frames_observed = 0;
    t->out_ordinal = -1;
    KT_HIP(hipEventCreateWithFlags(&t->guard_ev, KT_EV_DEVICE));
    for (int k = 0; k < KT_NODO; ++k) KT_HIP(hipEventCreateWithFlags(&t->odo_ev[k], KT_EV_DEVICE));
    for (int k = 0; k < KT_NSLOTS; ++k) t->slot_frame[k] = -1;
    KT_HIP(hipStreamCreateWithFlags(&t->pre_stream, hipStreamNonBlocking));
    KT_TRY(kt_bilateral_lut_ensure(ctx));
    t->pre_ctx = *ctx;
    t->pre_ctx.stream = t->pre_stream;
    t->pre_ctx.own_stream = false;
    t->last_assigned = KT_NSETS - 1;
    select_set(t, 0);
    t->cloud_cap = cfg->max_slice_points > 0 ? (size_t)cfg->max_slice_points : P * 3;
    for (int b = 0; b < 2; ++b) {
        KT_HIP(hipHostMalloc((void**)&t->cloud_host[b], t->cloud_cap * sizeof(kt_point_xyzrgb), hipHostMallocDefault));
        KT_HIP(hipHostMalloc((void**)&t->cloud_count_host[b], sizeof(unsigned int), hipHostMallocDefault));
        KT_HIP(hipEventCreateWithFlags(&t->cloud_ev[b], hipEventDisableTiming));
    }
    KT_TRY(dev_alloc(&t->state_dev, 1, true));
    KT_HIP(hipHostMalloc((void**)&t->state_host, sizeof(kt_track_state), hipHostMallocDefault));
    for (int k = 0; k < KT_NSLOTS; ++k) {
        KT_TRY(dev_alloc(&t->depth_stage[k], P, true));
        KT_TRY(dev_alloc(&t->rgb_stage[k], P * 3, true));
        KT_HIP(hipHostMalloc((void**)&t->depth_stage_host[k], P * sizeof(uint16_t), hipHostMallocDefault));
        KT_HIP(hipHostMalloc((void**)&t->rgb_stage_host[k], P * 3, hipHostMallocDefault));
        KT_HIP(hipEventCreateWithFlags(&t->slot_uploaded[k], hipEventDisableTiming));
    }
    t->next_slot = 0;
    KT_TRY(dev_alloc(&t->upd_dev, 16, true));
    KT_TRY(dev_alloc(&t->steps_dev, 4, true));
    t->profiling = 0;
    t->counting = 0;
    for (int par = 0; par < 2; ++par)
        for (int s = 0; s < ST_COUNT; ++s) {
            KT_HIP(hipEventCreate(&t->ev[par][s][0]));
            KT_HIP(hipEventCreate(&t->ev[par][s][1]));
            t->ev_rec[par][s] = false;
        }
    t->ev_par = 0;
    t->outstanding = false;
    t->host_wait_s = t->host_call_s = 0.0; t->host_calls = 0;
    KT_TRY(dev_alloc(&t->fp_dev, 1, true));
    KT_HIP(hipStreamCreateWithFlags(&t->plan_stream, hipStreamNonBlocking));
    t->icp_levels = kt_icp_levels_selected(ctx->device);
    t->last_icp_levels = false;
    t->icp_demote = 0; t->icp_demote_len = 64; t->odo_fallbacks = 0; t->out_last_set = -1;
    kt_live_trackers.fetch_add(1);
    t->counted = true;
    for (int k = 0; k < 3; ++k) {
        KT_TRY(kt_tsdf_plan_alloc(&t->plans[k].plan, cfg->N));
        KT_HIP(hipEventCreateWithFlags(&t->plans[k].done, KT_EV_DEVICE));
        t->plans[k].ordinal = -1; t->plans[k].set = -1; t->plans[k].depth = nullptr; t->plans[k].rgb = nullptr;
    }
    KT_HIP(hipEventCreateWithFlags(&t->gate_ev, KT_EV_DEVICE));
    t->gate_armed = false;
    {
        const char* e = getenv("KT_SIDE_GATE");
        const int mode = e ? atoi(e) : KT_SIDE_GATE_DEFAULT;
        int wcx = 0, wcy = 0, xg = 0, yg = 0;
        kt_tsdf_plan_shape(nullptr, cfg->cols, cfg->rows, cfg->N, &wcx, &wcy, &xg, &yg);
        const bool dense = wcx == 32 && (long long)cfg->cols * cfg->rows > 640LL * 480LL;
        t->side_gate = mode == 1 || (mode == 2 && dense) ? 1 : 0;
        if (mode == 2 && dense && !kt_icp_levels_forced()) t->icp_levels = false;
    }
    t->plan_enabled = getenv("KT_NO_PLAN") == nullptr;
    t->plan_margin_scale = getenv("KT_PLAN_MARGIN_SCALE") ? (float)atof(getenv("KT_PLAN_MARGIN_SCALE")) : 1.0f;
    t->plan_hits = t->plan_misses = 0;
    KT_TRY(dev_alloc(&t->bricks, kt_brick_count(cfg->N) + 16, true));
    for (int k = 0; k < 2; ++k) KT_TRY(dev_alloc(&t->wrkc_carry[k], (size_t)cfg->cols * cfg->rows, true));
    t->carry_sel = 0;
    KT_TRY(kt_integrate_tables(ctx, cfg->cols, cfg->rows, cfg->N, &t->vgz_dev, &t->zs_dev));
    KT_HIP(hipHostMalloc((void**)&t->mirror, sizeof(PoseMirror), hipHostMallocMapped | hipHostMallocCoherent));
    memset(t->mirror, 0, sizeof(PoseMirror));
    t->frame_seq = 0;
    t->prof_frames = 0;
    KT_TRY(kt_tracker_reset(t));
    {
        const int zero[3] = {0, 0, 0};
        KT_TRY(kt_extract_cloud_slice_async(ctx, t->tsdf, t->volume_size, t->cloud_host[0], t->cloud_cap, zero, t->color, 0, 1, 0, 1, 0, 1, 1, zero, t->N,
                                            &ctx->counters[1]));
        KT_TRY(kt_clear_volume(ctx, t->tsdf, 2, t->N, 0, 0, 0, 0));
        KT_TRY(kt_clear_volume(ctx, t->color, 4, t->N, 0, 0, 0, 0));
        KT_HIP(hipStreamSynchronize(ctx->stream));
    }
    return KT_OK;
}

int kt_tracker_destroy(kt_tracker* t)
{
    if (!t) return KT_OK;
    if (t->counted) kt_live_trackers.fetch_sub(1);
    (void)hipStreamSynchronize(t->ctx->stream);
    (void)join_slice_jobs(t);
    if (t->worker.joinable()) {
        { std::lock_guard<std::mutex> lk(t->wmu); t->wstop = true; }
        t->wcv.notify_all();
        t->worker.join();
    }
    (void)hipFree(t->tsdf); (void)hipFree(t->color);
    for (int l = 0; l < KT_LEVELS; ++l) {
        for (int q = 0; q < KT_NSETS; ++q) { (void)hipFree(t->sets[q].depths[l]); (void)hipFree(t->sets[q].vmaps[l]); (void)hipFree(t->sets[q].nmaps[l]); }
        (void)hipFree(t->vmaps_g_prev[l]); (void)hipFree(t->nmaps_g_prev[l]);
        for (int sidx = 0; sidx < KT_NSETS; ++sidx) {
            (void)hipFree(t->sets[sidx].depth_m[l]); (void)hipFree(t->sets[sidx].image[l]); (void)hipFree(t->sets[sidx].dIdx[l]);
            (void)hipFree(t->sets[sidx].dIdy[l]); (void)hipFree(t->sets[sidx].cloud[l]); (void)hipFree(t->sets[sidx].cand[l]);
        }
        (void)hipFree(t->corres[l]);
    }
    if (t->pre_stream) (void)hipStreamSynchronize(t->pre_stream);
    for (int q = 0; q < KT_NSETS; ++q) {
        (void)hipFree(t->sets[q].scaled); (void)hipFree(t->sets[q].rec); (void)hipFree(t->sets[q].dpmax);
        if (t->sets[q].ready) (void)hipEventDestroy(t->sets[q].ready);
    }
    if (t->guard_ev) (void)hipEventDestroy(t->guard_ev);
    for (int k = 0; k < KT_NODO; ++k)
        if (t->odo_ev[k]) (void)hipEventDestroy(t->odo_ev[k]);
    if (t->pre_stream) (void)hipStreamDestroy(t->pre_stream);
    (void)hipFree(t->vmap_curr_color);
    for (int b = 0; b < 2; ++b) {
        (void)hipHostFree(t->cloud_host[b]); (void)hipHostFree(t->cloud_count_host[b]);
        if (t->cloud_ev[b]) (void)hipEventDestroy(t->cloud_ev[b]);
        (void)hipFree(t->cloud_dev[b]); (void)hipFree(t->cloud_count_dev[b]); (void)hipHostFree(t->proc_host[b]); (void)hipHostFree(t->proc_count_host[b]);
        if (t->extracted[b]) (void)hipEventDestroy(t->extracted[b]);
    }
    if (t->slice_ws) (void)kt_slice_ws_destroy(t->slice_ws);
    for (int b = 0; b < 2; ++b) {
        (void)hipHostFree(t->mesh_v_host[b]); (void)hipHostFree(t->mesh_t_host[b]); (void)hipHostFree(t->mesh_count_host[b]);
        if (t->mesh_ev[b]) (void)hipEventDestroy(t->mesh_ev[b]);
    }
    if (t->mesh_ws) (void)kt_mesh_ws_destroy(t->mesh_ws);
    (void)hipFree(t->state_dev); (void)hipHostFree(t->state_host);
    for (int k = 0; k < KT_NSLOTS; ++k) {
        (void)hipFree(t->depth_stage[k]); (void)hipFree(t->rgb_stage[k]);
        (void)hipHostFree(t->depth_stage_host[k]); (void)hipHostFree(t->rgb_stage_host[k]);
        if (t->slot_uploaded[k]) (void)hipEventDestroy(t->slot_uploaded[k]);
    }
    (void)hipFree(t->upd_dev); (void)hipFree(t->steps_dev);
    for (int par = 0; par < 2; ++par)
        for (int s = 0; s < ST_COUNT; ++s) {
            if (t->ev[par][s][0]) (void)hipEventDestroy(t->ev[par][s][0]);
            if (t->ev[par][s][1]) (void)hipEventDestroy(t->ev[par][s][1]);
        }
    (void)hipHostFree(t->mirror);
    if (t->plan_stream) { (void)hipStreamSynchronize(t->plan_stream); (void)hipStreamDestroy(t->plan_stream); }
    for (int k = 0; k < 3; ++k) {
        kt_tsdf_plan_free(&t->plans[k].plan);
        if (t->plans[k].done) (void)hipEventDestroy(t->plans[k].done);
    }
    (void)hipFree(t->fp_dev);
    if (t->gate_ev) (void)hipEventDestroy(t->gate_ev);
    (void)hipFree(t->bricks);
    for (int k = 0; k < 2; ++k) (void)hipFree(t->wrkc_carry[k]);
    delete t;
    return KT_OK;
}

int kt_tracker_reset(kt_tracker* t)
{
    KT_ARG(t);
    t->outstanding = false;
    KT_TRY(kt_refill_granules(t->ctx));
    KT_HIP(hipStreamSynchronize(t->ctx->stream));
    t->global_time = 0;
    memcpy(t->Rlast, t->initial_rotation, sizeof(t->Rlast));
    memcpy(t->tlast, t->volume_basis, sizeof(t->tlast));
    compute_global_camera(t, nullptr);
    t->voxel_wrap[0] = t->voxel_wrap[1] = t->voxel_wrap[2] = 0;
    t->poses.clear();
    (void)join_slice_jobs(t);
    t->slices.clear();
    t->pr_samples.clear();
    memcpy(t->pr_trans, t->current_global_camera, sizeof(t->pr_trans));
    memcpy(t->pr_rot, t->initial_rotation, sizeof(t->pr_rot));
    KT_HIP(hipStreamSynchronize(t->pre_stream));
    t->pending.clear();
    KT_HIP(hipStreamSynchronize(t->plan_stream));
    t->plan_sel = -1;
    for (int k = 0; k < 3; ++k) { t->plans[k].ordinal = -1; t->plans[k].set = -1; }
    t->hist_n = 0;
    t->pred_err_t = t->pred_err_r = 0.0f;
    t->prev_set = -1;
    t->parked = t->cfg.static_mode != 0;
    t->v_wrap_copy[0] = t->v_wrap_copy[1] = t->v_wrap_copy[2] = 0;
    t->gt_utime = 0;
    t->current_ts = 0;
    for (int k = 0; k < 2; ++k) KT_HIP(hipMemsetAsync(t->wrkc_carry[k], 0, sizeof(float) * (size_t)t->cfg.cols * t->cfg.rows, t->ctx->stream));
    KT_TRY(kt_init_volume(t->ctx, t->tsdf, t->N));
    KT_TRY(kt_init_color_volume(t->ctx, t->color, t->N));
    KT_HIP(hipMemsetAsync(t->bricks, 0, kt_brick_count(t->N), t->ctx->stream));
    memset(t->stage_ms_sum, 0, sizeof(t->stage_ms_sum));
    memset(t->stage_n, 0, sizeof(t->stage_n));
    memset(t->stage_ms_last, 0, sizeof(t->stage_ms_last));
    t->last_U = t->last_S = 0;
    KT_HIP(hipStreamSynchronize(t->ctx->stream));
    return KT_OK;
}

}

static int odometry_begin(kt_tracker* t, const kt_level_k* first_k)
{
    kt_track_state* s = t->state_host;
    memset(s, 0, sizeof(*s));
    memcpy(s->Rprev, t->Rlast, sizeof(s->Rprev));
    memcpy(s->tprev, t->tlast, sizeof(s->tprev));
    memcpy(s->Rcurr, t->Rlast, sizeof(s->Rcurr));
    memcpy(s->tcurr, t->tlast, sizeof(s->tcurr));
    kt_mat33_inverse(s->Rprev, s->Rprev_inv);
    for (int k = 0; k < 16; ++k) s->resultRt[k] = (k % 5 == 0) ? 1.0 : 0.0;
    if (first_k) kt_compute_krk(s->resultRt, *first_k, s->krkinv, s->kt);
    KT_HIP(hipMemcpyAsync(t->state_dev, s, sizeof(*s), hipMemcpyHostToDevice, t->ctx->stream));
    return KT_OK;
}

static int odometry_end(kt_tracker* t)
{
    return ev_end(t, ST_ODOMETRY);
}

static int icp_odometry(kt_tracker* t, bool stepwise_only = false)
{
    int iters[KT_LEVELS] = {10, 5, 4, 0};
    if (t->cfg.fast_odometry) { iters[0] = 0; iters[1] = 10; iters[2] = 5; iters[3] = 0; }
    const float dist_thres = 0.10f;
    const float angle_thres = (float)sin(20.f * 3.14159254f / 180.f);
    kt_track_state init;
    memset(&init, 0, sizeof(init));
    memcpy(init.Rprev, t->Rlast, sizeof(init.Rprev));
    memcpy(init.tprev, t->tlast, sizeof(init.tprev));
    memcpy(init.Rcurr, t->Rlast, sizeof(init.Rcurr));
    memcpy(init.tcurr, t->tlast, sizeof(init.tcurr));
    kt_mat33_inverse(init.Rprev, init.Rprev_inv);
    bool first = true;
    t->last_icp_levels = !stepwise_only && t->icp_levels && t->icp_demote == 0 && kt_live_trackers.load() == 1;
    if (!stepwise_only && t->icp_demote > 0) --t->icp_demote;
    if (t->last_icp_levels) {
        const float* vc[KT_LEVELS]; const float* nc[KT_LEVELS]; const float* vg[KT_LEVELS]; const float* ng[KT_LEVELS];
        kt_intr li[KT_LEVELS]; int cs[KT_LEVELS], rs[KT_LEVELS], its[KT_LEVELS], nl = 0;
        for (int l = KT_LEVELS - 1; l >= 0; --l) {
            if (iters[l] <= 0) continue;
            vc[nl] = t->vmaps_curr[l]; nc[nl] = t->nmaps_curr[l]; vg[nl] = t->vmaps_g_prev[l]; ng[nl] = t->nmaps_g_prev[l];
            li[nl] = lvl_intr(t->intr, l); cs[nl] = lvl_cols(t, l); rs[nl] = lvl_rows(t, l); its[nl] = iters[l];
            ++nl;
        }
        if (nl) KT_TRY(kt_icp_levels_device(t->ctx, t->state_dev, nl, vc, nc, li, vg, ng, cs, rs, its, dist_thres, angle_thres, &init, 1));
        return odometry_end(t);
    }
    for (int l = KT_LEVELS - 1; l >= 0; --l) {
        const kt_intr li = lvl_intr(t->intr, l);
        for (int it = 0; it < iters[l]; ++it) {
            KT_TRY(kt_icp_step_device(t->ctx, t->state_dev, t->vmaps_curr[l], t->nmaps_curr[l], &li, t->vmaps_g_prev[l],
                                      t->nmaps_g_prev[l], lvl_cols(t, l), lvl_rows(t, l), dist_thres, angle_thres, KT_MODE_ICP_SOLVE,
                                      first ? &init : nullptr));
            first = false;
        }
    }
    return odometry_end(t);
}

static int rgbd_odometry(kt_tracker* t, int set, int last_set, bool stepwise_only = false)
{
    int iters[KT_LEVELS];
    if (!t->cfg.use_rgbd_icp) {
        iters[0] = 10; iters[1] = 7; iters[2] = 7; iters[3] = 7;
        if (t->cfg.fast_odometry) { iters[0] = 0; iters[1] = 10; iters[2] = 7; iters[3] = 0; }
    } else {
        iters[0] = 10; iters[1] = 5; iters[2] = 4; iters[3] = 0;
        if (t->cfg.fast_odometry) { iters[0] = 0; iters[1] = 10; iters[2] = 7; iters[3] = 0; }
    }
    const double SOBEL_SCALE = 1.0 / pow(2.0, 3), MAX_DEPTH_DELTA = 0.07;
    const float dist_thres = 0.10f;
    const float angle_thres = (float)sin(20.f * 3.14159254f / 180.f);
    KT_ARG(last_set >= 0);
    const FrameSet& next = t->sets[set];
    const FrameSet& last = t->sets[last_set];

    const double ifx = t->intr.fx, ify = t->intr.fy, icx = t->intr.cx, icy = t->intr.cy;
    kt_level_k lk[KT_LEVELS];
    for (int l = 0; l < KT_LEVELS; ++l) {
        const int div = 1 << l;
        lk[l].fx = ifx / div; lk[l].fy = ify / div; lk[l].cx = icx / div; lk[l].cy = icy / div;
    }
    int sched[64], ns = 0;
    for (int l = KT_LEVELS - 1; l >= 0; --l)
        for (int j = 0; j < iters[l]; ++j) sched[ns++] = l;
    KT_TRY(odometry_begin(t, ns ? &lk[sched[0]] : nullptr));
    const bool ri_levels_env = kt_ri_levels_selected();
    const bool ri_levels = t->cfg.use_rgbd_icp && !stepwise_only && ri_levels_env && t->icp_levels && t->icp_demote == 0 && kt_live_trackers.load() == 1;
    if (t->cfg.use_rgbd_icp && !stepwise_only && t->icp_demote > 0) --t->icp_demote;
    t->last_icp_levels = ri_levels;
    if (ri_levels) {
        for (int q = 0; q < ns;) {
            const int l = sched[q];
            int cnt = 0;
            while (q + cnt < ns && sched[q + cnt] == l) ++cnt;
            const kt_intr li = lvl_intr(t->intr, l);
            const kt_level_k* k_next = &lk[q + cnt < ns ? sched[q + cnt] : l];
            KT_TRY(kt_joint_level_device(t->ctx, t->state_dev, t->vmaps_curr[l], t->nmaps_curr[l], &li, t->vmaps_g_prev[l], t->nmaps_g_prev[l], dist_thres, angle_thres,
                                         t->corres[l], last.cloud[l], next.dIdx[l], next.dIdy[l], (float)SOBEL_SCALE, rgbd_min_scale(l), last.depth_m[l], next.depth_m[l],
                                         last.image[l], next.image[l], (float)MAX_DEPTH_DELTA, next.cand[l], lvl_cols(t, l), lvl_rows(t, l), cnt, &lk[l], k_next));
            q += cnt;
        }
        return odometry_end(t);
    }
    for (int q = 0; q < ns; ++q) {
        const int l = sched[q];
        const int cols = lvl_cols(t, l), rows = lvl_rows(t, l);
        const int first_at_level = q == 0 || sched[q - 1] != l;
        KT_TRY(kt_rgb_residual_device(t->ctx, t->state_dev, rgbd_min_scale(l), next.dIdx[l], next.dIdy[l], last.depth_m[l], next.depth_m[l],
                                      last.image[l], next.image[l], cols, rows, t->corres[l], (float)MAX_DEPTH_DELTA, next.cand[l],
                                      first_at_level));
        const kt_intr li = lvl_intr(t->intr, l);
        const kt_level_k* nk = &lk[q + 1 < ns ? sched[q + 1] : l];
        if (t->cfg.use_rgbd_icp)
            KT_TRY(kt_joint_step_device(t->ctx, t->state_dev, t->vmaps_curr[l], t->nmaps_curr[l], &li, t->vmaps_g_prev[l], t->nmaps_g_prev[l],
                                        dist_thres, angle_thres, t->corres[l], last.cloud[l], next.dIdx[l], next.dIdy[l], (float)SOBEL_SCALE,
                                        cols, rows, nk));
        else
            KT_TRY(kt_rgb_step_device(t->ctx, t->state_dev, t->corres[l], last.cloud[l], li.fx, li.fy, next.dIdx[l], next.dIdy[l],
                                      (float)SOBEL_SCALE, cols, rows, KT_MODE_RGB_SOLVE, nk));
    }
    return odometry_end(t);
}

__global__ __launch_bounds__(256) void kt_frame_setup_kernel(const kt_setup_args a)
{
    if (blockIdx.x > 0) {
        float R[9] = {0, 0, 0, 0, 0, 0, 0, 0, 0}, tv[3] = {0, 0, 0};
        if ((int)blockIdx.x > a.carry_groups) kt_setup_final_pose(a, R, tv);
        kt_setup_side_block(a, (int)blockIdx.x, (int)threadIdx.x, R, tv);
        return;
    }
    if (threadIdx.x >= 128 || a.mode == 2) return;
    float R[9], tv[3];
    if (a.mode == 0) kt_setup_final_pose(a, R, tv);
    else {
        for (int k = 0; k < 9; ++k) R[k] = a.R[k];
        for (int k = 0; k < 3; ++k) tv[k] = a.t[k];
    }
    kt_setup_block0(a, R, tv, a.mode == 0 ? a.st->handoff_timeout : 0, (int)(threadIdx.x >> 6), (int)(threadIdx.x & 63));
}

static int fill_setup_args(kt_tracker* t, int mode, const float* R, const float* tv, kt_setup_args& a)
{
    KT_TRY(kt_integrate_tables(t->ctx, t->cfg.cols, t->cfg.rows, t->N, &t->vgz_dev, &t->zs_dev));
    a.st = t->state_dev; a.fp = t->fp_dev; a.vgz = t->vgz_dev; a.zs = t->zs_dev; a.N = t->N;
    a.mirror = t->mirror; a.seq = t->frame_seq;
    a.cell_z = t->volume_size[2] / t->N;
    a.mode = mode;
    a.rgbd_guard = (t->cfg.use_rgbd || t->cfg.use_rgbd_icp) ? 1 : 0;
    for (int k = 0; k < 9; ++k) a.R[k] = R ? R[k] : 0.f;
    for (int k = 0; k < 3; ++k) a.t[k] = tv ? tv[k] : 0.f;
    for (int k = 0; k < 3; ++k) { a.basis[k] = t->volume_basis[k]; a.voxel[k] = t->voxel_size[k]; }
    a.thresh = t->parked ? INT_MAX : t->cfg.voxel_shift;
    a.rec = (kt_pixrec*)t->sets[t->out_set].rec;
    a.carry_cur = t->wrkc_carry[t->carry_sel];
    a.carry_next = t->wrkc_carry[t->carry_sel ^ 1];
    a.npix = t->cfg.cols * t->cfg.rows;
    a.carry_groups = t->cfg.disable_color_angle ? 0 : (a.npix + 1023) / 1024;
    a.plan_wrange = nullptr; a.plan_walk0 = nullptr;
    a.walk_groups = 0;
    a.wx = a.wy = a.wcx = a.wcy = a.XG = a.YG = 0; a.cell_x = a.cell_y = a.fx = a.fy = 0.0f; a.plan_theta = a.plan_tau = 0.0f;
    memset(a.plan_R, 0, sizeof(a.plan_R)); memset(a.plan_t, 0, sizeof(a.plan_t));
    if (mode == 0 && t->plan_sel >= 0) {
        const kt_tracker::PlanSlot& pl = t->plans[t->plan_sel];
        a.plan_wrange = pl.plan.wrange; a.plan_walk0 = pl.plan.walk0;
        memcpy(a.plan_R, pl.R, sizeof(a.plan_R)); memcpy(a.plan_t, pl.t, sizeof(a.plan_t));
        a.plan_theta = pl.theta; a.plan_tau = pl.tau;
        kt_tsdf_plan_shape(&pl.plan, t->cfg.cols, t->cfg.rows, t->N, &a.wcx, &a.wcy, &a.XG, &a.YG);
        a.wx = t->v_wrap_copy[0] % t->N; a.wy = t->v_wrap_copy[1] % t->N;
        a.cell_x = t->volume_size[0] / t->N; a.cell_y = t->volume_size[1] / t->N;
        a.fx = t->intr.fx; a.fy = t->intr.fy;
        a.walk_groups = (a.XG * a.YG + 3) / 4;
    }
    return KT_OK;
}

static int launch_setup(kt_tracker* t, int mode, const float* R, const float* tv)
{
    kt_setup_args a;
    KT_TRY(fill_setup_args(t, mode, R, tv, a));
    hipLaunchKernelGGL(kt_frame_setup_kernel, dim3(1 + a.carry_groups + a.walk_groups), dim3(256), 0, t->ctx->stream, a);
    KT_LAUNCH_CHECK();
    return KT_OK;
}

static int enqueue_fusion(kt_tracker* t, int set, const uint16_t* depth_raw, const uint8_t* colors, const kt_tsdf_plan* plan)
{
    kt_ctx* c = t->ctx;
    const int cols = t->cfg.cols, rows = t->cfg.rows, N = t->N;
    const bool icp = !t->has_trajectory && !(t->cfg.use_rgbd || t->cfg.use_rgbd_icp);
    const kt_mat33 dummy_R = {{1, 0, 0, 0, 1, 0, 0, 0, 1}};
    const float dummy_t[3] = {0, 0, 0};
    if (t->counting) {
        KT_HIP(hipMemsetAsync(t->upd_dev, 0, 16 * sizeof(unsigned int), c->stream));
        KT_HIP(hipMemsetAsync(t->steps_dev, 0, 4 * sizeof(unsigned long long), c->stream));
    }
    KT_TRY(ev_begin(t, ST_INTEGRATE));
    tsdf23_hook_arm(t);
    KT_TRY(kt_integrate_tsdf_impl(c, depth_raw, cols, rows, &t->intr, t->volume_size, &dummy_R, dummy_t, t->tranc_dist, t->tsdf,
                                  t->sets[set].scaled, t->v_wrap_copy, t->color, colors, t->sets[set].nmaps[0], !t->cfg.disable_color_angle, N,
                                  t->counting ? t->upd_dev : nullptr, t->sets[set].rec, t->fp_dev, t->bricks, t->sets[set].dpmax, plan));
    KT_TRY(ev_end(t, ST_INTEGRATE));
    if (t->side_gate) { KT_HIP(hipEventRecord(t->gate_ev, c->stream)); t->gate_armed = true; }
    KT_TRY(ev_begin(t, ST_RAYCAST));
    const bool pyr = icp || t->cfg.use_rgbd_icp;
    float* vp[3] = {t->vmaps_g_prev[1], t->vmaps_g_prev[2], t->vmaps_g_prev[3]};
    float* np_[3] = {t->nmaps_g_prev[1], t->nmaps_g_prev[2], t->nmaps_g_prev[3]};
    KT_TRY(kt_raycast_impl(c, &t->intr, &dummy_R, dummy_t, t->tranc_dist, t->volume_size, t->tsdf, t->vmaps_g_prev[0], t->nmaps_g_prev[0], cols, rows,
                           t->v_wrap_copy, t->vmap_curr_color, t->color, N, t->counting ? t->steps_dev : nullptr, pyr ? vp : nullptr,
                           pyr ? np_ : nullptr, t->fp_dev, t->bricks));
    KT_TRY(ev_end(t, ST_RAYCAST));
    return KT_OK;
}

static int join_slice_jobs(kt_tracker* t)
{
    int rc = KT_OK;
    for (int b = 0; b < 2; ++b) {
        kt_tracker::SliceJob& j = t->jobs[b];
        if (!j.active) continue;
        { std::unique_lock<std::mutex> lk(t->wmu); t->wdone.wait(lk, [&j]() { return j.done; }); }
        j.active = false;
        if (j.status != hipSuccess) { kt_set_error("slice download: %s", hipGetErrorString(j.status)); rc = KT_ERR_HIP; }
    }
    return rc;
}

static int fetch_slice(kt_tracker* t, const int lo[3], const int hi[3], int dim, const int mlo[3], const int mhi[3])
{
    kt_ctx* c = t->ctx;
    const int b = t->cloud_next;
    t->cloud_next ^= 1;
    kt_tracker::SliceJob& j = t->jobs[b];
    if (j.active) {
        { std::unique_lock<std::mutex> lk(t->wmu); t->wdone.wait(lk, [&j]() { return j.done; }); }
        j.active = false;
        if (j.status != hipSuccess) { kt_set_error("slice download: %s", hipGetErrorString(j.status)); return KT_ERR_HIP; }
    }
    const bool stage = t->slice_stage;
    if (!stage) {
        KT_TRY(kt_extract_cloud_slice_async(c, t->tsdf, t->volume_size, t->cloud_host[b], t->cloud_cap, t->v_wrap_copy, t->color, lo[0], hi[0],
                                            lo[1], hi[1], lo[2], hi[2], 1, t->voxel_wrap, t->N, &c->counters[1]));
        KT_HIP(hipMemcpyAsync(t->cloud_count_host[b], &c->counters[1], sizeof(unsigned int), hipMemcpyDeviceToHost, c->stream));
        KT_HIP(hipEventRecord(t->cloud_ev[b], c->stream));
    } else {
        hipStream_t ss = (hipStream_t)kt_slice_ws_stream(t->slice_ws);
        KT_TRY(kt_extract_cloud_slice_async(c, t->tsdf, t->volume_size, t->cloud_dev[b], t->cloud_cap, t->v_wrap_copy, t->color, lo[0], hi[0],
                                            lo[1], hi[1], lo[2], hi[2], 1, t->voxel_wrap, t->N, t->cloud_count_dev[b]));
        KT_HIP(hipEventRecord(t->extracted[b], c->stream));
        KT_HIP(hipStreamWaitEvent(ss, t->extracted[b], 0));
        KT_TRY(kt_copy_counted(ss, t->cloud_dev[b], t->cloud_host[b], t->cloud_count_dev[b], (unsigned int)t->cloud_cap, (int)sizeof(kt_point_xyzrgb), t->cloud_count_host[b]));
        const float leaf = fmaxf(t->voxel_size[0], fmaxf(t->voxel_size[1], t->voxel_size[2]));
        KT_TRY(kt_slice_process_device(t->slice_ws, t->cloud_dev[b], t->cloud_count_dev[b], t->cloud_cap, t->slice_cull, leaf, t->slice_k));
        KT_TRY(kt_copy_counted(ss, kt_slice_ws_output(t->slice_ws), t->proc_host[b], kt_slice_ws_leaves_dev(t->slice_ws), (unsigned int)t->cloud_cap,
                               (int)sizeof(kt_point_xyzrgbnormal), t->proc_count_host[b]));
        KT_HIP(hipEventRecord(t->cloud_ev[b], ss));
    }
    const bool mesh = t->mesh_stage;
    if (mesh) {
        KT_TRY(kt_mesh_enqueue(t->mesh_ws, c->stream, t->tsdf, t->color, t->volume_size, t->v_wrap_copy, mlo, mhi, t->voxel_wrap, t->N,
                               t->mesh_v_host[b], t->mesh_cap_v, t->mesh_t_host[b], t->mesh_cap_t));
        KT_HIP(hipMemcpyAsync(t->mesh_count_host[b], kt_mesh_ws_total(t->mesh_ws), sizeof(unsigned long long), hipMemcpyDeviceToHost, c->stream));
        KT_HIP(hipEventRecord(t->mesh_ev[b], c->stream));
    }
    t->slices.emplace_back();
    Slice& s = t->slices.back();
    s.dim = dim;
    s.pr_id = -1;
    memcpy(s.R, t->Rlast, sizeof(s.R));
    memcpy(s.cam, t->current_global_camera, sizeof(s.cam));
    s.ts = t->current_ts;
    j.slice = t->slices.size() - 1;
    j.status = hipSuccess;
    j.active = true;
    Slice* dst = &s;
    const kt_point_xyzrgb* src = t->cloud_host[b];
    const unsigned int* cnt = t->cloud_count_host[b];
    const size_t cap = t->cloud_cap;
    hipEvent_t ev = t->cloud_ev[b];
    hipError_t* status = &j.status;
    const kt_point_xyzrgbnormal* psrc = stage ? t->proc_host[b] : nullptr;
    const unsigned int* pcnt = stage ? t->proc_count_host[b] : nullptr;
    hipEvent_t mev = mesh ? t->mesh_ev[b] : nullptr;
    const kt_mesh_vertex* mv = t->mesh_v_host[b];
    const uint32_t* mt = t->mesh_t_host[b];
    const unsigned long long* mcnt = t->mesh_count_host[b];
    const size_t mcap_v = t->mesh_cap_v, mcap_t = t->mesh_cap_t;
    bool* done = &j.done;
    std::mutex* mu = &t->wmu;
    j.done = false;
    {
        std::lock_guard<std::mutex> lk(t->wmu);
        t->wq.emplace_back([dst, src, cnt, cap, ev, status, psrc, pcnt, mev, mv, mt, mcnt, mcap_v, mcap_t, done, mu]() {
            hipError_t e = hipEventSynchronize(ev);
            if (e == hipSuccess && mev) e = hipEventSynchronize(mev);
            if (e != hipSuccess) *status = e;
            else {
                size_t n = (size_t)*cnt;
                if (n > cap) n = cap;
                dst->pts.assign(src, src + n);
                if (psrc) {
                    size_t m = (size_t)*pcnt;
                    if (m > cap) m = cap;
                    dst->processed.assign(psrc, psrc + m);
                    dst->has_processed = true;
                }
                if (mev) {
                    const unsigned long long tot = *mcnt;
                    dst->mesh_nv = (long long)(tot & 0xffffffffull);
                    dst->mesh_nt = (long long)(tot >> 32);
                    dst->mesh_fit = (size_t)dst->mesh_nv <= mcap_v && (size_t)dst->mesh_nt <= mcap_t && dst->mesh_nv <= (1ll << 29);
                    if (dst->mesh_fit) {
                        dst->mesh_v.assign(mv, mv + dst->mesh_nv);
                        dst->mesh_t.assign(mt, mt + 3 * dst->mesh_nt);
                    }
                }
            }
            std::lock_guard<std::mutex> lk2(*mu);
            *done = true;
        });
    }
    t->wcv.notify_one();
    return KT_OK;
}

static int read_counts(kt_tracker* t)
{
    if (!t->counting) return KT_OK;
    kt_ctx* c = t->ctx;
    unsigned int u = 0;
    unsigned long long sdev = 0;
    KT_HIP(hipMemcpyAsync(&u, t->upd_dev, sizeof(u), hipMemcpyDeviceToHost, c->stream));
    KT_HIP(hipMemcpyAsync(&sdev, t->steps_dev, sizeof(sdev), hipMemcpyDeviceToHost, c->stream));
    KT_HIP(hipStreamSynchronize(c->stream));
    t->last_U = u;
    t->last_S = sdev;
    return KT_OK;
}

static void ground_truth_pose(kt_tracker* t, uint64_t timestamp, float Rcurr[9], float tcurr[3])
{
    memcpy(Rcurr, t->Rlast, 9 * sizeof(float));
    memcpy(tcurr, t->tlast, 3 * sizeof(float));
    if (t->gt_utime == 0 || t->trajectory.empty()) return;
    const std::array<float, 12>& A = t->trajectory[(int)(uint32_t)t->gt_utime];
    const std::array<float, 12>& B = t->trajectory[(int)(uint32_t)timestamp];
    kt_host_ground_truth_pose(A.data(), B.data(), t->Rlast, t->tlast, Rcurr, tcurr);
}

static int add_pr_sample(kt_tracker* t)
{
    PrSample ps;
    ps.utime = t->current_ts;
    memcpy(ps.trans, t->pr_trans, sizeof(ps.trans));
    memcpy(ps.rot, t->pr_rot, sizeof(ps.rot));
    ps.pose_index = (int)t->poses.size();
    t->pr_samples.push_back(ps);
    return (int)t->pr_samples.size() - 1;
}

static int finish_pose(kt_tracker* t, float Rcurr[9], float tcurr[3], bool speculated)
{
    kt_ctx* c = t->ctx;
    const int N = t->N;
    t->current_ts = t->out_ts;

    memcpy(t->Rlast, Rcurr, 9 * sizeof(float));
    memcpy(t->tlast, tcurr, 3 * sizeof(float));
    compute_global_camera(t, tcurr);
    if (t->cfg.dynamic_cube)
        kt_host_reposition_cube(Rcurr, t->tlast, t->cfg.volume_size, t->voxel_size,
                                t->parked ? (t->cfg.static_mode ? t->N * 3 : t->N) : t->cfg.voxel_shift, t->volume_basis);

    bool shift_send = false;
    int is_loop = 0;
    if (t->cfg.place_recognition) {
        const float place_recognition_movement = 0.15f;
        if (kt_host_place_recognition_movement(Rcurr, t->current_global_camera, t->pr_rot, t->pr_trans) >= place_recognition_movement) {
            memcpy(t->pr_rot, Rcurr, sizeof(t->pr_rot));
            memcpy(t->pr_trans, t->current_global_camera, sizeof(t->pr_trans));
            add_pr_sample(t);
            is_loop = 1;
        } else {
            shift_send = true;
        }
    }

    float current_translation[3];
    for (int k = 0; k < 3; ++k) current_translation[k] = t->tlast[k] - t->volume_basis[k];
    const int thresh = t->out_thresh;
    int vt[3];
    bool need_shift = false;
    for (int k = 0; k < 3; ++k) {
        vt[k] = voxel_trans(current_translation[k], t->voxel_size[k], thresh);
        need_shift = need_shift || vt[k] >= thresh || vt[k] <= -thresh;
    }
    if (speculated && need_shift != (t->mirror->skip == 1)) {
        kt_set_error("tracker: host and device disagree on the shift decision");
        return KT_ERR_STATE;
    }
    const bool plan_missed = speculated && t->mirror->skip == 2;
    if (speculated && t->plan_sel >= 0) {
        float dr = 0.0f, dt = 0.0f;
        const kt_tracker::PlanSlot& pl = t->plans[t->plan_sel];
        for (int k = 0; k < 9; ++k) dr += (Rcurr[k] - pl.R[k]) * (Rcurr[k] - pl.R[k]);
        for (int k = 0; k < 3; ++k) dt += (tcurr[k] - pl.t[k]) * (tcurr[k] - pl.t[k]);
        t->pred_err_r = sqrtf(dr) * 0.70710678f;
        t->pred_err_t = sqrtf(dt);
        if (plan_missed) ++t->plan_misses; else if (!need_shift) ++t->plan_hits;
    }
    t->plan_sel = -1;
    if (need_shift) {
        const int ov = t->cfg.overlap;
        KT_TRY(ev_begin(t, ST_SHIFT));
        for (int axis = 0; axis < 3; ++axis) {
            v_wrap_copy_update(t);
            bool cycled = false;
            int lo[3] = {0, 0, 0}, hi[3] = {N, N, N};
            int mlo[3] = {0, 0, 0}, mhi[3] = {N - 1, N - 1, N - 1};
            int dim = 0;
            if (vt[axis] >= thresh) {
                lo[axis] = 0; hi[axis] = vt[axis] + 1 + ov;
                dim = axis * 2;
                mlo[axis] = 0; mhi[axis] = vt[axis];
                KT_TRY(fetch_slice(t, lo, hi, dim, mlo, mhi));
                KT_TRY(kt_clear_volume(c, t->tsdf, 2, N, axis, 0, t->voxel_wrap[axis], t->voxel_wrap[axis] + vt[axis]));
                KT_TRY(kt_clear_volume(c, t->color, 4, N, axis, 0, t->voxel_wrap[axis], t->voxel_wrap[axis] + vt[axis]));
                cycled = true;
            } else if (vt[axis] <= -thresh) {
                if (axis == 2) { lo[2] = N + (vt[2] - ov) - 1; hi[2] = N - 1; }
                else { lo[axis] = N + (vt[axis] - ov); hi[axis] = N; }
                dim = axis * 2 + 1;
                mlo[axis] = N + vt[axis] - 1; mhi[axis] = N - 1;
                KT_TRY(fetch_slice(t, lo, hi, dim, mlo, mhi));
                KT_TRY(kt_clear_volume(c, t->tsdf, 2, N, axis, 1, t->voxel_wrap[axis], t->voxel_wrap[axis] + vt[axis]));
                KT_TRY(kt_clear_volume(c, t->color, 4, N, axis, 1, t->voxel_wrap[axis], t->voxel_wrap[axis] + vt[axis]));
                cycled = true;
            }
            if (cycled) {
                if (shift_send) {
                    memcpy(t->pr_rot, Rcurr, sizeof(t->pr_rot));
                    memcpy(t->pr_trans, t->current_global_camera, sizeof(t->pr_trans));
                    t->slices.back().pr_id = add_pr_sample(t);
                    is_loop = 1;
                    shift_send = false;
                }
                const float shift = t->voxel_size[axis] * (float)vt[axis];
                t->tlast[axis] -= shift;
                t->voxel_wrap[axis] += vt[axis];
                tcurr[axis] -= shift;
            }
        }
        v_wrap_copy_update(t);
        KT_TRY(ev_end(t, ST_SHIFT));
    }
    if (need_shift || !speculated || plan_missed) {
        v_wrap_copy_update(t);
        KT_TRY(launch_setup(t, 1, Rcurr, tcurr));
        KT_TRY(enqueue_fusion(t, t->out_set, t->out_depth, t->out_rgb, nullptr));
    }
    v_wrap_copy_update(t);
    ++t->global_time;
    push_pose(t, t->out_ts, Rcurr, is_loop);
    memcpy(t->hist_R[0], t->hist_R[1], sizeof(t->hist_R[0])); memcpy(t->hist_gc[0], t->hist_gc[1], sizeof(t->hist_gc[0]));
    memcpy(t->hist_R[1], Rcurr, sizeof(t->hist_R[1])); memcpy(t->hist_gc[1], t->current_global_camera, sizeof(t->hist_gc[1]));
    if (t->hist_n < 2) ++t->hist_n;
    return KT_OK;
}

static int drop_plans_of_set(kt_tracker* t, int set)
{
    for (int k = 0; k < 3; ++k) {
        kt_tracker::PlanSlot& pl = t->plans[k];
        if (pl.ordinal < 0 || pl.set != set) continue;
        KT_HIP(hipStreamWaitEvent(t->ctx->stream, pl.done, 0));
        KT_HIP(hipStreamWaitEvent(t->pre_stream, pl.done, 0));
        pl.ordinal = -1; pl.set = -1;
    }
    return KT_OK;
}

static float plan_rand(kt_tracker* t)
{
    t->plan_rng = t->plan_rng * 1664525u + 1013904223u;
    return (float)((t->plan_rng >> 8) & 0xffffffu) * (2.0f / 16777216.0f) - 1.0f;
}
static void plan_rand_unit(kt_tracker* t, float v[3])
{
    for (;;) {
        v[0] = plan_rand(t); v[1] = plan_rand(t); v[2] = plan_rand(t);
        const float n2 = v[0] * v[0] + v[1] * v[1] + v[2] * v[2];
        if (n2 > 0.01f && n2 <= 1.0f) { const float s = 1.0f / sqrtf(n2); v[0] *= s; v[1] *= s; v[2] *= s; return; }
    }
}

static int plan_ahead(kt_tracker* t, const Pending& next, long long ordinal)
{
    const int set = next.set;
    kt_tracker::PlanSlot& pl = t->plans[ordinal % 3];
    pl.ordinal = -1; pl.set = -1;
    float D[9], Rp[9], tp[3];
    for (int i = 0; i < 3; ++i)
        for (int j = 0; j < 3; ++j) D[i * 3 + j] = t->hist_R[0][0 * 3 + i] * t->hist_R[1][0 * 3 + j] + t->hist_R[0][1 * 3 + i] * t->hist_R[1][1 * 3 + j] + t->hist_R[0][2 * 3 + i] * t->hist_R[1][2 * 3 + j];
    for (int i = 0; i < 3; ++i)
        for (int j = 0; j < 3; ++j) Rp[i * 3 + j] = t->Rlast[i * 3 + 0] * D[0 * 3 + j] + t->Rlast[i * 3 + 1] * D[1 * 3 + j] + t->Rlast[i * 3 + 2] * D[2 * 3 + j];
    float step = 0.0f, turn = 0.0f;
    for (int k = 0; k < 3; ++k) {
        const float d = t->hist_gc[1][k] - t->hist_gc[0][k];
        tp[k] = t->tlast[k] + d;
        step += d * d;
    }
    for (int k = 0; k < 9; ++k) turn += (D[k] - ((k % 4 == 0) ? 1.0f : 0.0f)) * (D[k] - ((k % 4 == 0) ? 1.0f : 0.0f));
    step = sqrtf(step); turn = sqrtf(turn) * 0.70710678f;
    if (t->plan_hits + t->plan_misses == 0) { t->pred_err_t = 0.5f * step; t->pred_err_r = 0.5f * turn; }
    pl.tau = t->plan_margin_scale * fminf(0.020f, 0.0015f + 3.0f * t->pred_err_t);
    pl.theta = t->plan_margin_scale * fminf(0.02f, 3.0e-4f + 3.0f * t->pred_err_r);
    if (t->plan_theta_fixed > 0.0f) pl.theta = t->plan_theta_fixed;
    if (t->plan_tau_fixed > 0.0f) pl.tau = t->plan_tau_fixed;
    if ((size_t)(ordinal + 1) * 12 <= t->plan_truth.size()) {
        memcpy(Rp, &t->plan_truth[(size_t)ordinal * 12], sizeof(Rp));
        memcpy(tp, &t->plan_truth[(size_t)ordinal * 12 + 9], sizeof(tp));
    }
    if (t->plan_perturb) {
        float ax[3], dir[3], K[9], Rd[9], Rn[9];
        plan_rand_unit(t, ax); plan_rand_unit(t, dir);
        const float phi = t->plan_fr * pl.theta, sn = sinf(phi), cs = cosf(phi);
        const float Kx[9] = {0, -ax[2], ax[1], ax[2], 0, -ax[0], -ax[1], ax[0], 0};
        for (int i = 0; i < 3; ++i)
            for (int j = 0; j < 3; ++j) K[i * 3 + j] = Kx[i * 3 + 0] * Kx[0 * 3 + j] + Kx[i * 3 + 1] * Kx[1 * 3 + j] + Kx[i * 3 + 2] * Kx[2 * 3 + j];
        for (int k = 0; k < 9; ++k) Rd[k] = ((k % 4 == 0) ? 1.0f : 0.0f) + sn * Kx[k] + (1.0f - cs) * K[k];
        for (int i = 0; i < 3; ++i)
            for (int j = 0; j < 3; ++j) Rn[i * 3 + j] = Rp[i * 3 + 0] * Rd[0 * 3 + j] + Rp[i * 3 + 1] * Rd[1 * 3 + j] + Rp[i * 3 + 2] * Rd[2 * 3 + j];
        memcpy(Rp, Rn, sizeof(Rp));
        for (int k = 0; k < 3; ++k) tp[k] += dir[k] * t->plan_ft * pl.tau;
    }
    kt_mat33 Rinv;
    kt_mat33_inverse(Rp, Rinv.m);
    v_wrap_copy_update(t);
    KT_HIP(hipStreamWaitEvent(t->plan_stream, t->sets[set].ready, 0));
    const int made = kt_integrate_plan(t->plan_stream, &pl.plan, t->sets[set].rec, t->sets[set].dpmax, t->cfg.cols, t->cfg.rows, &t->intr, t->volume_size, &Rinv, tp,
                                       t->tranc_dist, t->v_wrap_copy, t->N, pl.theta, pl.tau);
    if (made == KT_NO_PLAN) return KT_OK;
    KT_TRY(made);
    KT_HIP(hipEventRecord(pl.done, t->plan_stream));
    memcpy(pl.R, Rp, sizeof(pl.R)); memcpy(pl.t, tp, sizeof(pl.t));
    memcpy(pl.wrap, t->v_wrap_copy, sizeof(pl.wrap));
    pl.set = set; pl.depth = next.depth; pl.rgb = next.rgb;
    pl.ordinal = ordinal;
    return KT_OK;
}

static int plan_frame(kt_tracker* t, const Pending& frame, long long ordinal)
{
    if (!(t->plan_enabled && t->hist_n >= 2 && !t->cfg.dynamic_cube && !t->has_trajectory)) return KT_OK;
    if (t->side_gate && t->gate_armed) KT_HIP(hipStreamWaitEvent(t->plan_stream, t->gate_ev, 0));
    v_wrap_copy_update(t);
    KT_TRY(plan_ahead(t, frame, ordinal));
    if (t->plans[ordinal % 3].ordinal == ordinal && ordinal == t->frames_started - 1) t->plan_sel = (int)(ordinal % 3);
    return KT_OK;
}

static int wait_for_pose(kt_tracker* t)
{
    const auto w0 = std::chrono::steady_clock::now();
    volatile unsigned int* seq = &t->mirror->seq;
    long long spins = 0;
    while (__atomic_load_n(seq, __ATOMIC_ACQUIRE) != t->frame_seq) {
        if ((++spins & 0xfff) == 0) {
            const double waited = std::chrono::duration<double>(std::chrono::steady_clock::now() - w0).count();
            if (waited > 30.0) {
                const hipError_t e = hipStreamQuery(t->ctx->stream);
                kt_set_error("tracker: no pose from the device after 30 s (stream status: %s)", hipGetErrorString(e));
                return KT_ERR_STATE;
            }
            if (waited > 0.002) std::this_thread::yield();
        }
    }
    t->host_wait_s += std::chrono::duration<double>(std::chrono::steady_clock::now() - w0).count();
    return KT_OK;
}

static int complete_frame(kt_tracker* t)
{
    if (!t->outstanding) return KT_OK;
    t->outstanding = false;
    kt_ctx* c = t->ctx;
    KT_TRY(wait_for_pose(t));
    if (t->out_ordinal + 1 > t->frames_observed) t->frames_observed = t->out_ordinal + 1;
    ev_collect(t);
    if (t->mirror->handoff_timeout) {
        KT_TRY(kt_refill_granules(c));
        ++t->odo_fallbacks;
        t->icp_demote = t->icp_demote_len;
        if (t->icp_demote_len < 65536) t->icp_demote_len *= 2;
        select_set(t, t->out_set);
        const bool icp = !(t->cfg.use_rgbd || t->cfg.use_rgbd_icp);
        if (icp) KT_TRY(icp_odometry(t, true));
        else KT_TRY(rgbd_odometry(t, t->out_set, t->out_last_set, true));
        if (++t->frame_seq == 0) t->frame_seq = 1;
        KT_TRY(launch_setup(t, 0, nullptr, nullptr));
        if (t->out_speculated) KT_TRY(enqueue_fusion(t, t->out_set, t->out_depth, t->out_rgb, t->plan_sel >= 0 ? &t->plans[t->plan_sel].plan : nullptr));
        KT_TRY(wait_for_pose(t));
        if (t->mirror->handoff_timeout) {
            (void)kt_refill_granules(c);
            kt_set_error("odometry: inter-workgroup hand-off timed out (also in the stepwise re-run of the frame)");
            return KT_ERR_STATE;
        }
    }
    float Rcurr[9], tcurr[3];
    memcpy(Rcurr, t->mirror->R, sizeof(Rcurr));
    memcpy(tcurr, t->mirror->t, sizeof(tcurr));
    if (t->pose_log_on) {
        if (t->pose_log.size() < (size_t)(t->out_ordinal + 1) * 12) t->pose_log.resize((size_t)(t->out_ordinal + 1) * 12, 0.0f);
        memcpy(&t->pose_log[(size_t)t->out_ordinal * 12], Rcurr, sizeof(Rcurr));
        memcpy(&t->pose_log[(size_t)t->out_ordinal * 12 + 9], tcurr, sizeof(tcurr));
    }
    return finish_pose(t, Rcurr, tcurr, t->out_speculated);
}

extern "C" {

static int process_frame_impl(kt_tracker* t, const uint16_t* depth_raw, const uint8_t* colors, uint64_t timestamp);

int kt_tracker_process_frame(kt_tracker* t, const uint16_t* depth_raw, const uint8_t* colors, uint64_t timestamp)
{
    KT_ARG(t && depth_raw && colors);
    const auto c0 = std::chrono::steady_clock::now();
    const int r = process_frame_impl(t, depth_raw, colors, timestamp);
    t->host_call_s += std::chrono::duration<double>(std::chrono::steady_clock::now() - c0).count();
    t->host_calls += 1;
    return r;
}

int kt_tracker_host_times(kt_tracker* t, double out2[2], int reset)
{
    KT_ARG(t && out2);
    out2[0] = t->host_calls ? t->host_call_s / (double)t->host_calls : 0.0;
    out2[1] = t->host_calls ? t->host_wait_s / (double)t->host_calls : 0.0;
    if (reset) { t->host_call_s = t->host_wait_s = 0.0; t->host_calls = 0; }
    return KT_OK;
}

static int process_frame_impl(kt_tracker* t, const uint16_t* depth_raw, const uint8_t* colors, uint64_t timestamp)
{
    KT_TRY(complete_frame(t));
    kt_ctx* c = t->ctx;
    const bool gt = t->has_trajectory;
    if (gt && !t->trajectory.count((int)(uint32_t)timestamp)) {
        for (size_t i = 0; i < t->pending.size(); ++i)
            if (t->pending[i].depth == depth_raw && t->pending[i].rgb == colors) {
                KT_HIP(hipStreamWaitEvent(c->stream, t->sets[t->pending[i].set].ready, 0));
                KT_TRY(drop_plans_of_set(t, t->pending[i].set));
                t->pending.erase(t->pending.begin() + i);
                break;
            }
        return KT_OK;
    }
    t->current_ts = timestamp;
    const int cols = t->cfg.cols, rows = t->cfg.rows, N = t->N;
    const bool icp = !gt && !(t->cfg.use_rgbd || t->cfg.use_rgbd_icp);
    const int angle_color = !t->cfg.disable_color_angle;

    int set = -1;
    bool read_ahead = false;
    for (size_t i = 0; i < t->pending.size(); ++i)
        if (t->pending[i].depth == depth_raw && t->pending[i].rgb == colors) {
            read_ahead = true;
            for (size_t j = 0; j < i; ++j) {
                KT_HIP(hipStreamWaitEvent(c->stream, t->sets[t->pending[j].set].ready, 0));
                KT_TRY(drop_plans_of_set(t, t->pending[j].set));
            }
            set = t->pending[i].set;
            t->pending.erase(t->pending.begin(), t->pending.begin() + i + 1);
            if (hipEventQuery(t->sets[set].ready) != hipSuccess) KT_HIP(hipStreamWaitEvent(c->stream, t->sets[set].ready, 0));
            break;
        }
    if (set < 0) {
        set = pick_free_set(t);
        if (set < 0) {
            set = t->pending.front().set;
            KT_HIP(hipStreamWaitEvent(c->stream, t->sets[set].ready, 0));
            KT_TRY(drop_plans_of_set(t, set));
            t->pending.erase(t->pending.begin());
        }
        t->last_assigned = set;
        KT_TRY(ev_begin(t, ST_PYRAMID));
        KT_TRY(build_frame_set(t, c, set, depth_raw, colors));
        KT_TRY(ev_end(t, ST_PYRAMID));
    }
    select_set(t, set);
    const long long ordinal = t->frames_started;
    t->sets[set].user = t->frames_started++;
    for (int k = 0; k < KT_NSLOTS; ++k)
        if (depth_raw == t->depth_stage[k]) t->slot_frame[k] = ordinal;
    const int last_set = t->prev_set;
    t->prev_set = set;
    t->out_set = set;
    t->out_last_set = last_set;
    t->carry_sel ^= 1;

    if (t->global_time == 0) {
        kt_mat33 Rcam, Rcam_inv;
        memcpy(Rcam.m, t->Rlast, sizeof(Rcam.m));
        kt_mat33_inverse(Rcam.m, Rcam_inv.m);
        const int empty[3] = {0, 0, 0};
        if (t->counting) KT_HIP(hipMemsetAsync(t->upd_dev, 0, 16 * sizeof(unsigned int), c->stream));
        KT_TRY(launch_setup(t, 2, nullptr, nullptr));
        KT_TRY(ev_begin(t, ST_INTEGRATE));
        tsdf23_hook_arm(t);
        KT_TRY(kt_integrate_tsdf_impl(c, depth_raw, cols, rows, &t->intr, t->volume_size, &Rcam_inv, t->tlast, t->tranc_dist, t->tsdf,
                                      t->depth_raw_scaled, empty, t->color, colors, t->nmaps_curr[0], angle_color, N,
                                      t->counting ? t->upd_dev : nullptr, t->rec_curr, nullptr, t->bricks, t->sets[set].dpmax));
        KT_TRY(ev_end(t, ST_INTEGRATE));
        for (int l = 0; l < KT_LEVELS; ++l)
            KT_TRY(kt_transform_maps(c, t->vmaps_curr[l], t->nmaps_curr[l], lvl_cols(t, l), lvl_rows(t, l), &Rcam, t->tlast, t->vmaps_g_prev[l],
                                     t->nmaps_g_prev[l]));
        ++t->global_time;
        t->ev_par ^= 1;
        t->gt_utime = timestamp;
        KT_HIP(hipEventRecord(t->odo_ev[ordinal % KT_NODO], c->stream));
        if (t->cfg.place_recognition) add_pr_sample(t);
        push_pose(t, timestamp, t->Rlast, 1);
        if (t->counting) {
            unsigned int u = 0;
            KT_HIP(hipMemcpyAsync(&u, t->upd_dev, sizeof(u), hipMemcpyDeviceToHost, c->stream));
            KT_HIP(hipStreamSynchronize(c->stream));
            t->last_U = u;
            t->last_S = 0;
        }
        return KT_OK;
    }

    t->out_ts = timestamp;
    t->out_set = set;
    t->out_depth = depth_raw;
    t->out_rgb = colors;
    t->out_thresh = t->parked ? INT_MAX : t->cfg.voxel_shift;
    if (gt) {
        float Rcurr[9], tcurr[3];
        ev_collect(t);
        ground_truth_pose(t, timestamp, Rcurr, tcurr);
        t->gt_utime = timestamp;
        KT_HIP(hipEventRecord(t->odo_ev[ordinal % KT_NODO], c->stream));
        KT_TRY(finish_pose(t, Rcurr, tcurr, false));
        t->ev_par ^= 1;
        if (t->counting) KT_TRY(read_counts(t));
        return KT_OK;
    }

    t->plan_sel = -1;
    v_wrap_copy_update(t);
    if (read_ahead) {
        const kt_tracker::PlanSlot& pl = t->plans[ordinal % 3];
        if (pl.ordinal == ordinal && pl.set == set && pl.depth == depth_raw && pl.rgb == colors && memcmp(pl.wrap, t->v_wrap_copy, sizeof(t->v_wrap_copy)) == 0)
            t->plan_sel = (int)(ordinal % 3);
        else
            KT_TRY(plan_frame(t, Pending{depth_raw, colors, set, nullptr, nullptr}, ordinal));
    }
    v_wrap_copy_update(t);
    if (++t->frame_seq == 0) t->frame_seq = 1;
    KT_TRY(ev_begin(t, ST_ODOMETRY));
    if (icp) KT_TRY(icp_odometry(t));
    else KT_TRY(rgbd_odometry(t, set, last_set));
    v_wrap_copy_update(t);
    if (t->plan_sel >= 0 && hipEventQuery(t->plans[t->plan_sel].done) != hipSuccess) KT_HIP(hipStreamWaitEvent(c->stream, t->plans[t->plan_sel].done, 0));
    if (t->side_gate && !t->pending.empty()) KT_HIP(hipStreamWaitEvent(c->stream, t->sets[t->pending.front().set].ready, 0));
    KT_TRY(launch_setup(t, 0, nullptr, nullptr));
    t->out_speculated = !t->cfg.dynamic_cube;
    if (t->out_speculated) KT_TRY(enqueue_fusion(t, set, depth_raw, colors, t->plan_sel >= 0 ? &t->plans[t->plan_sel].plan : nullptr));
    t->outstanding = true;
    t->out_ordinal = ordinal;
    t->gt_utime = timestamp;
    if (!t->out_speculated) KT_TRY(complete_frame(t));
    t->ev_par ^= 1;
    if (t->counting) {
        KT_TRY(complete_frame(t));
        KT_TRY(read_counts(t));
    }
    return KT_OK;
}

static int prefetch_impl(kt_tracker* t, const uint16_t* depth_raw, const uint8_t* colors, const uint16_t* depth_host, const uint8_t* rgb_host);

int kt_tracker_prefetch_frame(kt_tracker* t, const uint16_t* depth_raw, const uint8_t* colors)
{
    KT_ARG(t && depth_raw && colors);
    return prefetch_impl(t, depth_raw, colors, nullptr, nullptr);
}

static int stage_host_frame(kt_tracker* t, hipStream_t stream, const uint16_t* depth_host, const uint8_t* rgb_host, int* slot_out)
{
    const size_t P = (size_t)t->cfg.cols * t->cfg.rows;
    const int slot = t->next_slot;
    t->next_slot = (t->next_slot + 1) % KT_NSLOTS;
    KT_HIP(hipEventSynchronize(t->slot_uploaded[slot]));
    KT_TRY(wait_frame_consumed(t, stream, t->slot_frame[slot]));
    t->slot_frame[slot] = -1;
    memcpy(t->depth_stage_host[slot], depth_host, P * sizeof(uint16_t));
    memcpy(t->rgb_stage_host[slot], rgb_host, P * 3);
    KT_HIP(hipMemcpyAsync(t->depth_stage[slot], t->depth_stage_host[slot], P * sizeof(uint16_t), hipMemcpyHostToDevice, stream));
    KT_HIP(hipMemcpyAsync(t->rgb_stage[slot], t->rgb_stage_host[slot], P * 3, hipMemcpyHostToDevice, stream));
    KT_HIP(hipEventRecord(t->slot_uploaded[slot], stream));
    *slot_out = slot;
    return KT_OK;
}

int kt_tracker_prefetch_frame_host(kt_tracker* t, const uint16_t* depth_host, const uint8_t* rgb_host)
{
    KT_ARG(t && depth_host && rgb_host);
    if (t->pending.size() >= 2) { kt_set_error("kt_tracker_prefetch_frame_host: two read-ahead frames are already outstanding"); return KT_ERR_STATE; }
    KT_TRY(complete_frame(t));
    int slot;
    KT_TRY(stage_host_frame(t, t->pre_stream, depth_host, rgb_host, &slot));
    return prefetch_impl(t, t->depth_stage[slot], t->rgb_stage[slot], depth_host, rgb_host);
}

static int prefetch_impl(kt_tracker* t, const uint16_t* depth_raw, const uint8_t* colors, const uint16_t* depth_host, const uint8_t* rgb_host)
{
    if (t->pending.size() >= 2) { kt_set_error("kt_tracker_prefetch_frame: two read-ahead frames are already outstanding"); return KT_ERR_STATE; }
    KT_TRY(complete_frame(t));
    if (!t->pending.empty() && t->plans[t->frames_started % 3].ordinal != t->frames_started) KT_TRY(plan_frame(t, t->pending.front(), t->frames_started));
    const int set = pick_free_set(t);
    if (set < 0) { kt_set_error("kt_tracker_prefetch_frame: no free frame set"); return KT_ERR_STATE; }
    t->last_assigned = set;
    KT_TRY(wait_frame_consumed(t, t->pre_stream, t->sets[set].user));
    t->pre_ctx.device = t->ctx->device;
    if (t->side_gate && t->gate_armed) {
        KT_HIP(hipStreamWaitEvent(t->pre_stream, t->gate_ev, 0));
    }
    KT_TRY(build_frame_set(t, &t->pre_ctx, set, depth_raw, colors));
    KT_HIP(hipEventRecord(t->sets[set].ready, t->pre_stream));
    t->pending.push_back(Pending{depth_raw, colors, set, depth_host, rgb_host});
    return KT_OK;
}

int kt_tracker_process_frame_host(kt_tracker* t, const uint16_t* depth_host, const uint8_t* rgb_host, uint64_t timestamp)
{
    KT_ARG(t && depth_host && rgb_host);
    for (const Pending& p : t->pending)
        if (p.depth_host == depth_host && p.rgb_host == rgb_host) return kt_tracker_process_frame(t, p.depth, p.rgb, timestamp);
    KT_TRY(complete_frame(t));
    int slot;
    KT_TRY(stage_host_frame(t, t->ctx->stream, depth_host, rgb_host, &slot));
    return kt_tracker_process_frame(t, t->depth_stage[slot], t->rgb_stage[slot], timestamp);
}

int kt_tracker_load_trajectory(kt_tracker* t, int n, const uint64_t* utimes, const float* pose7)
{
    KT_ARG(t && n >= 0 && (n == 0 || (utimes && pose7)));
    KT_TRY(complete_frame(t));
    t->has_trajectory = true;
    for (int i = 0; i < n; ++i) {
        std::array<float, 12> T;
        kt_host_trajectory_pose(pose7 + (size_t)i * 7, T.data());
        t->trajectory[(int)(uint32_t)utimes[i]] = T;
    }
    t->gt_utime = 0;
    return KT_OK;
}

int kt_tracker_get_volume_basis(kt_tracker* t, float* basis)
{
    KT_ARG(t && basis);
    KT_TRY(complete_frame(t));
    memcpy(basis, t->volume_basis, sizeof(t->volume_basis));
    return KT_OK;
}

int kt_tracker_finalise(kt_tracker* t)
{
    KT_ARG(t);
    KT_TRY(complete_frame(t));
    v_wrap_copy_update(t);
    const int lo[3] = {0, 0, 0}, hi[3] = {t->N, t->N, t->N};
    const int mhi[3] = {t->N - 1, t->N - 1, t->N - 1};
    KT_TRY(fetch_slice(t, lo, hi, 7 , lo, mhi));
    if (t->cfg.place_recognition) {
        memcpy(t->pr_rot, t->Rlast, sizeof(t->pr_rot));
        memcpy(t->pr_trans, t->current_global_camera, sizeof(t->pr_trans));
        t->slices.back().pr_id = add_pr_sample(t);
        t->pr_samples.back().pose_index = (int)t->poses.size() - 1;
    }
    return KT_OK;
}

int kt_tracker_num_pr_samples(kt_tracker* t) { return (t && complete_frame(t) == KT_OK) ? (int)t->pr_samples.size() : -1; }
int kt_tracker_pr_sample(kt_tracker* t, int i, uint64_t* utime, float* trans, float* rotation, int* pose_index)
{
    KT_ARG(t && utime && trans && rotation && pose_index);
    KT_TRY(complete_frame(t));
    KT_ARG(i >= 0 && i < (int)t->pr_samples.size());
    const PrSample& ps = t->pr_samples[i];
    *utime = ps.utime;
    memcpy(trans, ps.trans, sizeof(ps.trans));
    memcpy(rotation, ps.rot, sizeof(ps.rot));
    *pose_index = ps.pose_index;
    return KT_OK;
}
int kt_tracker_slice_pr_id(kt_tracker* t, int i, int* pr_id)
{
    KT_ARG(t && pr_id);
    KT_TRY(complete_frame(t));
    KT_ARG(i >= 0 && i < (int)t->slices.size());
    *pr_id = t->slices[i].pr_id;
    return KT_OK;
}

int kt_tracker_get_pose(kt_tracker* t, float* R, float* tv, float* gc)
{
    KT_ARG(t && R && tv && gc);
    KT_TRY(complete_frame(t));
    memcpy(R, t->Rlast, sizeof(t->Rlast));
    memcpy(tv, t->tlast, sizeof(t->tlast));
    memcpy(gc, t->current_global_camera, sizeof(t->current_global_camera));
    return KT_OK;
}
int kt_tracker_num_poses(kt_tracker* t) { return (t && complete_frame(t) == KT_OK) ? (int)t->poses.size() : -1; }
int kt_tracker_get_dense_pose(kt_tracker* t, int i, uint64_t* ts, float* pose16, int* is_loop)
{
    KT_ARG(t);
    KT_TRY(complete_frame(t));
    KT_ARG(t && i >= 0 && i < (int)t->poses.size() && ts && pose16 && is_loop);
    *ts = t->poses[i].ts;
    memcpy(pose16, t->poses[i].pose, sizeof(t->poses[i].pose));
    *is_loop = t->poses[i].is_loop;
    return KT_OK;
}
int kt_tracker_get_voxel_wrap(kt_tracker* t, int* wrap)
{
    KT_ARG(t && wrap);
    KT_TRY(complete_frame(t));
    memcpy(wrap, t->voxel_wrap, sizeof(t->voxel_wrap));
    return KT_OK;
}
int kt_tracker_num_slices(kt_tracker* t) { return (t && complete_frame(t) == KT_OK) ? (int)t->slices.size() : -1; }
int kt_tracker_slice_info(kt_tracker* t, int i, size_t* n_points, int* dimension)
{
    KT_ARG(t);
    KT_TRY(complete_frame(t));
    KT_ARG(t && i >= 0 && i < (int)t->slices.size() && n_points && dimension);
    KT_TRY(join_slice_jobs(t));
    *n_points = t->slices[i].pts.size();
    *dimension = t->slices[i].dim;
    return KT_OK;
}
int kt_tracker_set_parked(kt_tracker* t, int parked)
{
    KT_ARG(t);
    KT_TRY(complete_frame(t));
    t->parked = parked != 0;
    return KT_OK;
}
int kt_tracker_slice_pose(kt_tracker* t, int i, float* R, float* cam, uint64_t* ts)
{
    KT_ARG(t);
    KT_TRY(complete_frame(t));
    KT_ARG(t && i >= 0 && i < (int)t->slices.size());
    if (R) memcpy(R, t->slices[i].R, 9 * sizeof(float));
    if (cam) memcpy(cam, t->slices[i].cam, 3 * sizeof(float));
    if (ts) *ts = t->slices[i].ts;
    return KT_OK;
}
int kt_tracker_slice_points(kt_tracker* t, int i, kt_point_xyzrgb* out)
{
    KT_ARG(t);
    KT_TRY(complete_frame(t));
    KT_ARG(t && i >= 0 && i < (int)t->slices.size() && out);
    KT_TRY(join_slice_jobs(t));
    if (!t->slices[i].pts.empty()) memcpy(out, t->slices[i].pts.data(), t->slices[i].pts.size() * sizeof(kt_point_xyzrgb));
    return KT_OK;
}
int16_t* kt_tracker_volume(kt_tracker* t) { return (t && complete_frame(t) == KT_OK) ? t->tsdf : nullptr; }
uint8_t* kt_tracker_color_volume(kt_tracker* t) { return (t && complete_frame(t) == KT_OK) ? t->color : nullptr; }
float* kt_tracker_vmap_g_prev(kt_tracker* t, int l) { return (t && l >= 0 && l < KT_LEVELS && complete_frame(t) == KT_OK) ? t->vmaps_g_prev[l] : nullptr; }
float* kt_tracker_nmap_g_prev(kt_tracker* t, int l) { return (t && l >= 0 && l < KT_LEVELS && complete_frame(t) == KT_OK) ? t->nmaps_g_prev[l] : nullptr; }
uint8_t* kt_tracker_vmap_curr_color(kt_tracker* t) { return (t && complete_frame(t) == KT_OK) ? t->vmap_curr_color : nullptr; }
float kt_tracker_trunc_dist(kt_tracker* t) { return t ? t->tranc_dist : 0.f; }

int kt_tracker_enable_profiling(kt_tracker* t, int on)
{
    KT_ARG(t);
    KT_TRY(complete_frame(t));
    KT_HIP(hipStreamSynchronize(t->ctx->stream));
    ev_collect(t);
    t->profiling = on;
    memset(t->stage_ms_sum, 0, sizeof(t->stage_ms_sum));
    memset(t->stage_n, 0, sizeof(t->stage_n));
    return KT_OK;
}
int kt_tracker_stage_ms(kt_tracker* t, float* ms)
{
    KT_ARG(t && ms);
    KT_TRY(complete_frame(t));
    KT_HIP(hipStreamSynchronize(t->ctx->stream));
    ev_collect(t);
    for (int s = 0; s < ST_COUNT; ++s) ms[s] = t->stage_n[s] ? (float)(t->stage_ms_sum[s] / (double)t->stage_n[s]) : 0.f;
    return KT_OK;
}
int kt_tracker_stage_counts(kt_tracker* t, long long* n)
{
    KT_ARG(t && n);
    for (int s = 0; s < ST_COUNT; ++s) n[s] = t->stage_n[s];
    return KT_OK;
}
int kt_tracker_enable_counts(kt_tracker* t, int on)
{
    KT_ARG(t);
    t->counting = on;
    return KT_OK;
}
int kt_tracker_debug_state(kt_tracker* t, float* out29)
{
    KT_ARG(t && out29);
    KT_TRY(complete_frame(t));
    KT_HIP(hipStreamSynchronize(t->ctx->stream));
    KT_HIP(hipMemcpy(t->state_host, t->state_dev, sizeof(kt_track_state), hipMemcpyDeviceToHost));
    memcpy(out29, t->state_host->icp29, 29 * sizeof(float));
    return KT_OK;
}
int kt_tracker_enable_slice_stage(kt_tracker* t, int on, int weight_cull, int k)
{
    KT_ARG(t && (!on || (k >= 1 && k <= 64)));
    KT_TRY(complete_frame(t));
    KT_TRY(join_slice_jobs(t));
    if (on && !t->slice_ws) {
        KT_TRY(kt_slice_ws_create(t->ctx, t->cloud_cap, nullptr, &t->slice_ws));
        for (int b = 0; b < 2; ++b) {
            KT_HIP(hipMalloc((void**)&t->cloud_dev[b], t->cloud_cap * sizeof(kt_point_xyzrgb)));
            KT_HIP(hipMalloc((void**)&t->cloud_count_dev[b], sizeof(unsigned int)));
            KT_HIP(hipHostMalloc((void**)&t->proc_host[b], t->cloud_cap * sizeof(kt_point_xyzrgbnormal), hipHostMallocDefault));
            KT_HIP(hipHostMalloc((void**)&t->proc_count_host[b], sizeof(unsigned int), hipHostMallocDefault));
            KT_HIP(hipEventCreateWithFlags(&t->extracted[b], KT_EV_DEVICE));
        }
        KT_HIP(hipMemsetAsync(t->cloud_count_dev[0], 0, sizeof(unsigned int), (hipStream_t)kt_slice_ws_stream(t->slice_ws)));
        const float leaf = fmaxf(t->voxel_size[0], fmaxf(t->voxel_size[1], t->voxel_size[2]));
        KT_TRY(kt_slice_process_device(t->slice_ws, t->cloud_dev[0], t->cloud_count_dev[0], t->cloud_cap, weight_cull, leaf, k));
        KT_HIP(hipStreamSynchronize((hipStream_t)kt_slice_ws_stream(t->slice_ws)));
    }
    t->slice_stage = on != 0;
    t->slice_cull = weight_cull; t->slice_k = k;
    return KT_OK;
}
int kt_tracker_slice_processed_info(kt_tracker* t, int i, long long* n_points)
{
    KT_ARG(t && n_points);
    KT_TRY(complete_frame(t));
    KT_ARG(i >= 0 && i < (int)t->slices.size());
    KT_TRY(join_slice_jobs(t));
    *n_points = t->slices[i].has_processed ? (long long)t->slices[i].processed.size() : -1;
    return KT_OK;
}
int kt_tracker_slice_processed(kt_tracker* t, int i, kt_point_xyzrgbnormal* out)
{
    KT_ARG(t && out);
    KT_TRY(complete_frame(t));
    KT_ARG(i >= 0 && i < (int)t->slices.size());
    KT_TRY(join_slice_jobs(t));
    KT_ARG(t->slices[i].has_processed);
    if (!t->slices[i].processed.empty()) memcpy(out, t->slices[i].processed.data(), t->slices[i].processed.size() * sizeof(kt_point_xyzrgbnormal));
    return KT_OK;
}

int kt_tracker_enable_mesh_stage(kt_tracker* t, int on, long long max_vertices, long long max_triangles)
{
    KT_ARG(t && max_vertices >= 0 && max_triangles >= 0);
    KT_TRY(complete_frame(t));
    KT_TRY(join_slice_jobs(t));
    if (on) {
        const size_t N = (size_t)t->N;
        const size_t cv = max_vertices > 0 ? (size_t)max_vertices : 8 * N * N;
        const size_t ct = max_triangles > 0 ? (size_t)max_triangles : 2 * cv;
        if (!t->mesh_ws) {
            size_t voxels = 0, runs = 0;
            const int lo[3] = {0, 0, 0}, hi[3] = {t->N - 1, t->N - 1, t->N - 1};
            KT_TRY(kt_mesh_check(lo, hi, t->N, &voxels, &runs));
            KT_TRY(kt_mesh_ws_reserve(&t->mesh_ws, voxels, runs));
        }
        if (cv != t->mesh_cap_v || ct != t->mesh_cap_t) {
            for (int b = 0; b < 2; ++b) {
                (void)hipHostFree(t->mesh_v_host[b]); (void)hipHostFree(t->mesh_t_host[b]);
                t->mesh_v_host[b] = nullptr; t->mesh_t_host[b] = nullptr;
            }
            t->mesh_cap_v = t->mesh_cap_t = 0;
            for (int b = 0; b < 2; ++b) {
                KT_HIP(hipHostMalloc((void**)&t->mesh_v_host[b], cv * sizeof(kt_mesh_vertex), hipHostMallocDefault));
                KT_HIP(hipHostMalloc((void**)&t->mesh_t_host[b], ct * 3 * sizeof(uint32_t), hipHostMallocDefault));
            }
            t->mesh_cap_v = cv; t->mesh_cap_t = ct;
        }
        for (int b = 0; b < 2; ++b) {
            if (!t->mesh_count_host[b]) KT_HIP(hipHostMalloc((void**)&t->mesh_count_host[b], sizeof(unsigned long long), hipHostMallocDefault));
            if (!t->mesh_ev[b]) KT_HIP(hipEventCreateWithFlags(&t->mesh_ev[b], hipEventDisableTiming));
        }
    }
    t->mesh_stage = on != 0;
    return KT_OK;
}
int kt_tracker_slice_mesh_info(kt_tracker* t, int i, long long* n_vertices, long long* n_triangles)
{
    KT_ARG(t && n_vertices && n_triangles);
    KT_TRY(complete_frame(t));
    KT_ARG(i >= 0 && i < (int)t->slices.size());
    KT_TRY(join_slice_jobs(t));
    *n_vertices = t->slices[i].mesh_nv;
    *n_triangles = t->slices[i].mesh_nt;
    return KT_OK;
}
int kt_tracker_slice_mesh(kt_tracker* t, int i, kt_mesh_vertex* vertices, uint32_t* triangles)
{
    KT_ARG(t);
    KT_TRY(complete_frame(t));
    KT_ARG(i >= 0 && i < (int)t->slices.size());
    KT_TRY(join_slice_jobs(t));
    const Slice& s = t->slices[i];
    KT_ARG(s.mesh_nv >= 0);
    if (!s.mesh_fit) {
        kt_set_error("slice %d: its mesh (%lld vertices, %lld triangles) exceeded the mesh stage's bounds (%zu / %zu)", i, s.mesh_nv, s.mesh_nt,
                     t->mesh_cap_v, t->mesh_cap_t);
        return KT_ERR_CAPACITY;
    }
    KT_ARG((vertices || s.mesh_v.empty()) && (triangles || s.mesh_t.empty()));
    if (!s.mesh_v.empty()) memcpy(vertices, s.mesh_v.data(), s.mesh_v.size() * sizeof(kt_mesh_vertex));
    if (!s.mesh_t.empty()) memcpy(triangles, s.mesh_t.data(), s.mesh_t.size() * sizeof(uint32_t));
    return KT_OK;
}

int kt_tracker_odometry_fallbacks(kt_tracker* t, long long* out)
{
    KT_ARG(t && out);
    KT_TRY(complete_frame(t));
    *out = t->odo_fallbacks;
    return KT_OK;
}

int kt_tracker_plan_stats(kt_tracker* t, long long out2[2])
{
    KT_ARG(t && out2);
    KT_TRY(complete_frame(t));
    out2[0] = t->plan_hits; out2[1] = t->plan_misses;
    return KT_OK;
}
int kt_tracker_debug_pose_log(kt_tracker* t, int enable, float* out12n, int max_frames, int* n_frames)
{
    KT_ARG(t);
    if (enable >= 0) t->pose_log_on = enable != 0;
    if (out12n || n_frames) {
        KT_TRY(complete_frame(t));
        const int n = (int)(t->pose_log.size() / 12);
        if (n_frames) *n_frames = n;
        if (out12n) memcpy(out12n, t->pose_log.data(), sizeof(float) * 12 * (size_t)(n < max_frames ? n : max_frames));
    }
    return KT_OK;
}
int kt_tracker_debug_plan_truth(kt_tracker* t, const float* poses12n, int n_frames, float fr, float ft, float theta_fixed, float tau_fixed, unsigned int seed)
{
    KT_ARG(t && n_frames >= 0 && (poses12n || n_frames == 0) && fr >= 0 && ft >= 0 && theta_fixed >= 0 && tau_fixed >= 0);
    t->plan_truth.assign(poses12n, poses12n + (size_t)n_frames * 12);
    t->plan_fr = fr; t->plan_ft = ft; t->plan_perturb = fr > 0.0f || ft > 0.0f;
    t->plan_theta_fixed = theta_fixed; t->plan_tau_fixed = tau_fixed;
    t->plan_rng = seed * 2654435761u + 0x9e3779b9u;
    return KT_OK;
}


int kt_tracker_debug_counts(kt_tracker* t, unsigned int* out4)
{
    KT_ARG(t && out4);
    KT_HIP(hipMemcpy(out4, t->upd_dev, 8 * sizeof(unsigned int), hipMemcpyDeviceToHost));
    { unsigned long long h[3] = {0, 0, 0}; KT_HIP(hipMemcpy(h, t->steps_dev + 1, sizeof(h), hipMemcpyDeviceToHost)); out4[7] = (unsigned int)h[0]; out4[5] = (unsigned int)h[1]; out4[6] = (unsigned int)h[2]; }
    return KT_OK;
}
int kt_tracker_debug_bricks(kt_tracker* t, unsigned char* out_host)
{
    KT_ARG(t && out_host);
    KT_TRY(complete_frame(t));
    KT_HIP(hipMemcpyAsync(out_host, t->bricks, kt_brick_count(t->N), hipMemcpyDeviceToHost, t->ctx->stream));
    KT_HIP(hipStreamSynchronize(t->ctx->stream));
    return KT_OK;
}
int kt_tracker_last_counts(kt_tracker* t, unsigned long long* U, unsigned long long* S)
{
    KT_ARG(t && U && S);
    *U = t->last_U;
    *S = t->last_S;
    return KT_OK;
}

int kt_tracker_export_poses_device(kt_tracker* t, int k, float* dst_dev)
{
    KT_ARG(t);
    KT_TRY(complete_frame(t));
    KT_ARG(k > 0 && dst_dev && k <= (int)t->poses.size());
    std::vector<float> tmp((size_t)k * 16);
    for (int i = 0; i < k; ++i) memcpy(&tmp[(size_t)i * 16], t->poses[t->poses.size() - k + i].pose, 16 * sizeof(float));
    KT_HIP(hipMemcpyAsync(dst_dev, tmp.data(), tmp.size() * sizeof(float), hipMemcpyHostToDevice, t->ctx->stream));
    KT_HIP(hipStreamSynchronize(t->ctx->stream));
    return KT_OK;
}

}

extern "C" int kt_tracker_debug_icp_levels(kt_tracker* t) { return t && t->last_icp_levels ? 1 : 0; }
extern "C" int kt_tracker_debug_side_gate(kt_tracker* t) { return t ? t->side_gate : 0; }
```

Measured before the change: 3957 frames/s.

## Defer read-ahead frame build and plan submission until after odometry launch

Prefetch now only records a pending frame and marks its pyramid build and fusion plan as owed. The owed work is submitted lazily, right after the current frame's odometry kernels are enqueued, or at any API sync point via a new settle helper. The aim is to get the critical-path odometry onto the GPU first, so side-stream prefetch and plan work no longer delay it. It also adds submission counters and a debug query that reports where odometry sat in the submission order, which makes the bookkeeping more involved.

```diff
diff --git a/kintinuous_amd/abi.py b/kintinuous_amd/abi.py
--- a/kintinuous_amd/abi.py
+++ b/kintinuous_amd/abi.py
@@ -155,6 +155,7 @@
     "kt_tracker_odometry_fallbacks": (_i, [_vp, C.POINTER(C.c_longlong)]),
     "kt_debug_wait_limit": (_i, [_vp, C.c_uint]),
     "kt_tracker_debug_side_gate": (_i, [_vp]),
+    "kt_tracker_debug_odometry_position": (_i, [_vp, C.c_longlong]),
     "kt_tracker_enable_slice_stage": (_i, [_vp, _i, _i, _i]),
     "kt_tracker_slice_processed_info": (_i, [_vp, _i, C.POINTER(C.c_longlong)]),
     "kt_tracker_slice_processed": (_i, [_vp, _i, _vp]),
diff --git a/kintinuous_amd/csrc/kt_debug.h b/kintinuous_amd/csrc/kt_debug.h
--- a/kintinuous_amd/csrc/kt_debug.h
+++ b/kintinuous_amd/csrc/kt_debug.h
@@ -28,6 +28,7 @@
 int kt_debug_ri_levels(int on);
 int kt_tracker_debug_icp_levels(kt_tracker* trk);
 int kt_tracker_debug_side_gate(kt_tracker* trk);
+int kt_tracker_debug_odometry_position(kt_tracker* trk, long long ordinal);
 float kt_debug_sq_threshold(float T, int strict);
 
 #ifdef __cplusplus
diff --git a/kintinuous_amd/csrc/kt_tracker.hip b/kintinuous_amd/csrc/kt_tracker.hip
--- a/kintinuous_amd/csrc/kt_tracker.hip
+++ b/kintinuous_amd/csrc/kt_tracker.hip
@@ -43,7 +43,7 @@
 #define KT_NSETS 3
 
 typedef kt_pose_mirror PoseMirror;
-struct Pending { const uint16_t* depth; const uint8_t* rgb; int set; const uint16_t* depth_host; const uint8_t* rgb_host; };
+struct Pending { const uint16_t* depth; const uint8_t* rgb; int set; const uint16_t* depth_host; const uint8_t* rgb_host; bool build_owed; };
 #define KT_NSLOTS 4
 #define KT_NODO 8
 
@@ -82,6 +82,8 @@
     FrameSet sets[KT_NSETS];
     int last_assigned;
     std::vector<Pending> pending;
+    bool plan_owed;
+    long long submits, submits_at_pose; std::vector<int> odo_pos;
     long long frames_started;
     long long frames_observed;
     long long out_ordinal;
@@ -153,6 +155,9 @@
 };
 
 static int join_slice_jobs(kt_tracker* t);
+static int complete_frame(kt_tracker* t);
+static int flush_owed(kt_tracker* t);
+static void note_submit(kt_tracker* t) { ++t->submits; }
 static int plan_frame(kt_tracker* t, const struct Pending& frame, long long ordinal);
 static int lvl_cols(const kt_tracker* t, int l) { return t->cfg.cols >> l; }
 static int lvl_rows(const kt_tracker* t, int l) { return t->cfg.rows >> l; }
@@ -203,6 +208,7 @@
 {
     if (u < 0 || stream == t->ctx->stream) return KT_OK;
     if (u + 2 <= t->frames_observed) return KT_OK;
+    note_submit(t);
     if (t->has_trajectory && u + 1 < t->frames_started) {
         KT_HIP(hipStreamWaitEvent(stream, t->odo_ev[(u + 1) % KT_NODO], 0));
     } else {
@@ -223,6 +229,7 @@
 {
     const int cols = t->cfg.cols, rows = t->cfg.rows;
     FrameSet& fs = t->sets[q];
+    note_submit(t);
     const bool icp = !t->has_trajectory && !(t->cfg.use_rgbd || t->cfg.use_rgbd_icp);
     const bool rgbd = !t->has_trajectory && !icp;
     static const bool fused_prepare = []() { const char* e = getenv("KT_PREPARE_FUSED"); return e ? atoi(e) != 0 : true; }();
@@ -289,6 +296,7 @@
 static int ev_begin(kt_tracker* t, int st)
 {
     if (prof_all(t) || (prof_tsdf(t) && st == ST_TSDF23)) {
+        note_submit(t);
         KT_HIP(hipEventRecord(t->ev[t->ev_par][st][0], t->ctx->stream));
     }
     return KT_OK;
@@ -405,6 +413,8 @@
         t->sets[q].user = -1;
     }
     t->frames_started = 0;
+    t->plan_owed = false;
+    t->submits = t->submits_at_pose = 0;
     t->cloud_next = 0;
     t->slice_stage = false; t->slice_ws = nullptr;
     t->mesh_stage = false; t->mesh_ws = nullptr; t->mesh_cap_v = t->mesh_cap_t = 0;
@@ -589,6 +599,7 @@
 {
     KT_ARG(t);
     t->outstanding = false;
+    t->plan_owed = false;
     KT_TRY(kt_refill_granules(t->ctx));
     KT_HIP(hipStreamSynchronize(t->ctx->stream));
     t->global_time = 0;
@@ -810,6 +821,7 @@
 {
     kt_setup_args a;
     KT_TRY(fill_setup_args(t, mode, R, tv, a));
+    note_submit(t);
     hipLaunchKernelGGL(kt_frame_setup_kernel, dim3(1 + a.carry_groups + a.walk_groups), dim3(256), 0, t->ctx->stream, a);
     KT_LAUNCH_CHECK();
     return KT_OK;
@@ -822,6 +834,7 @@
     const bool icp = !t->has_trajectory && !(t->cfg.use_rgbd || t->cfg.use_rgbd_icp);
     const kt_mat33 dummy_R = {{1, 0, 0, 0, 1, 0, 0, 0, 1}};
     const float dummy_t[3] = {0, 0, 0};
+    note_submit(t);
     if (t->counting) {
         KT_HIP(hipMemsetAsync(t->upd_dev, 0, 16 * sizeof(unsigned int), c->stream));
         KT_HIP(hipMemsetAsync(t->steps_dev, 0, 4 * sizeof(unsigned long long), c->stream));
@@ -863,6 +876,7 @@
     const int b = t->cloud_next;
     t->cloud_next ^= 1;
     kt_tracker::SliceJob& j = t->jobs[b];
+    note_submit(t);
     if (j.active) {
         { std::unique_lock<std::mutex> lk(t->wmu); t->wdone.wait(lk, [&j]() { return j.done; }); }
         j.active = false;
@@ -1104,6 +1118,7 @@
     for (int k = 0; k < 3; ++k) {
         kt_tracker::PlanSlot& pl = t->plans[k];
         if (pl.ordinal < 0 || pl.set != set) continue;
+        note_submit(t);
         KT_HIP(hipStreamWaitEvent(t->ctx->stream, pl.done, 0));
         KT_HIP(hipStreamWaitEvent(t->pre_stream, pl.done, 0));
         pl.ordinal = -1; pl.set = -1;
@@ -1184,6 +1199,7 @@
 static int plan_frame(kt_tracker* t, const Pending& frame, long long ordinal)
 {
     if (!(t->plan_enabled && t->hist_n >= 2 && !t->cfg.dynamic_cube && !t->has_trajectory)) return KT_OK;
+    note_submit(t);
     if (t->side_gate && t->gate_armed) KT_HIP(hipStreamWaitEvent(t->plan_stream, t->gate_ev, 0));
     v_wrap_copy_update(t);
     KT_TRY(plan_ahead(t, frame, ordinal));
@@ -1217,6 +1233,7 @@
     t->outstanding = false;
     kt_ctx* c = t->ctx;
     KT_TRY(wait_for_pose(t));
+    t->submits_at_pose = t->submits;
     if (t->out_ordinal + 1 > t->frames_observed) t->frames_observed = t->out_ordinal + 1;
     ev_collect(t);
     if (t->mirror->handoff_timeout) {
@@ -1249,6 +1266,36 @@
     return finish_pose(t, Rcurr, tcurr, t->out_speculated);
 }
 
+static int submit_build(kt_tracker* t, Pending& p)
+{
+    p.build_owed = false;
+    KT_TRY(wait_frame_consumed(t, t->pre_stream, t->sets[p.set].user));
+    t->pre_ctx.device = t->ctx->device;
+    if (t->side_gate && t->gate_armed) {
+        KT_HIP(hipStreamWaitEvent(t->pre_stream, t->gate_ev, 0));
+    }
+    KT_TRY(build_frame_set(t, &t->pre_ctx, p.set, p.depth, p.rgb));
+    KT_HIP(hipEventRecord(t->sets[p.set].ready, t->pre_stream));
+    return KT_OK;
+}
+
+static int flush_owed(kt_tracker* t)
+{
+    if (t->plan_owed) {
+        t->plan_owed = false;
+        if (!t->pending.empty() && t->plans[t->frames_started % 3].ordinal != t->frames_started) KT_TRY(plan_frame(t, t->pending.front(), t->frames_started));
+    }
+    for (Pending& p : t->pending)
+        if (p.build_owed) KT_TRY(submit_build(t, p));
+    return KT_OK;
+}
+
+static int settle(kt_tracker* t)
+{
+    KT_TRY(complete_frame(t));
+    return flush_owed(t);
+}
+
 extern "C" {
 
 static int process_frame_impl(kt_tracker* t, const uint16_t* depth_raw, const uint8_t* colors, uint64_t timestamp);
@@ -1277,9 +1324,12 @@
     KT_TRY(complete_frame(t));
     kt_ctx* c = t->ctx;
     const bool gt = t->has_trajectory;
+    const bool odo_first = !gt && t->global_time != 0 && !t->pending.empty() && t->pending[0].depth == depth_raw && t->pending[0].rgb == colors && !t->pending[0].build_owed;
+    if (!odo_first) KT_TRY(flush_owed(t));
     if (gt && !t->trajectory.count((int)(uint32_t)timestamp)) {
         for (size_t i = 0; i < t->pending.size(); ++i)
             if (t->pending[i].depth == depth_raw && t->pending[i].rgb == colors) {
+                note_submit(t);
                 KT_HIP(hipStreamWaitEvent(c->stream, t->sets[t->pending[i].set].ready, 0));
                 KT_TRY(drop_plans_of_set(t, t->pending[i].set));
                 t->pending.erase(t->pending.begin() + i);
@@ -1298,18 +1348,20 @@
         if (t->pending[i].depth == depth_raw && t->pending[i].rgb == colors) {
             read_ahead = true;
             for (size_t j = 0; j < i; ++j) {
+                note_submit(t);
                 KT_HIP(hipStreamWaitEvent(c->stream, t->sets[t->pending[j].set].ready, 0));
                 KT_TRY(drop_plans_of_set(t, t->pending[j].set));
             }
             set = t->pending[i].set;
             t->pending.erase(t->pending.begin(), t->pending.begin() + i + 1);
-            if (hipEventQuery(t->sets[set].ready) != hipSuccess) KT_HIP(hipStreamWaitEvent(c->stream, t->sets[set].ready, 0));
+            if (hipEventQuery(t->sets[set].ready) != hipSuccess) { note_submit(t); KT_HIP(hipStreamWaitEvent(c->stream, t->sets[set].ready, 0)); }
             break;
         }
     if (set < 0) {
         set = pick_free_set(t);
         if (set < 0) {
             set = t->pending.front().set;
+            note_submit(t);
             KT_HIP(hipStreamWaitEvent(c->stream, t->sets[set].ready, 0));
             KT_TRY(drop_plans_of_set(t, set));
             t->pending.erase(t->pending.begin());
@@ -1329,6 +1381,7 @@
     t->out_set = set;
     t->out_last_set = last_set;
     t->carry_sel ^= 1;
+    t->odo_pos.resize((size_t)ordinal + 1, -1);
 
     if (t->global_time == 0) {
         kt_mat33 Rcam, Rcam_inv;
@@ -1359,6 +1412,7 @@
             t->last_U = u;
             t->last_S = 0;
         }
+        t->submits_at_pose = t->submits;
         return KT_OK;
     }
 
@@ -1376,26 +1430,29 @@
         KT_TRY(finish_pose(t, Rcurr, tcurr, false));
         t->ev_par ^= 1;
         if (t->counting) KT_TRY(read_counts(t));
+        t->submits_at_pose = t->submits;
         return KT_OK;
     }
 
     t->plan_sel = -1;
     v_wrap_copy_update(t);
+    if (++t->frame_seq == 0) t->frame_seq = 1;
+    KT_TRY(ev_begin(t, ST_ODOMETRY));
+    t->odo_pos[(size_t)ordinal] = (int)(t->submits - t->submits_at_pose);
+    if (icp) KT_TRY(icp_odometry(t));
+    else KT_TRY(rgbd_odometry(t, set, last_set));
+    t->plan_owed = false;
     if (read_ahead) {
         const kt_tracker::PlanSlot& pl = t->plans[ordinal % 3];
         if (pl.ordinal == ordinal && pl.set == set && pl.depth == depth_raw && pl.rgb == colors && memcmp(pl.wrap, t->v_wrap_copy, sizeof(t->v_wrap_copy)) == 0)
             t->plan_sel = (int)(ordinal % 3);
         else
-            KT_TRY(plan_frame(t, Pending{depth_raw, colors, set, nullptr, nullptr}, ordinal));
-    }
+            KT_TRY(plan_frame(t, Pending{depth_raw, colors, set, nullptr, nullptr, false}, ordinal));
+    }
+    KT_TRY(flush_owed(t));
     v_wrap_copy_update(t);
-    if (++t->frame_seq == 0) t->frame_seq = 1;
-    KT_TRY(ev_begin(t, ST_ODOMETRY));
-    if (icp) KT_TRY(icp_odometry(t));
-    else KT_TRY(rgbd_odometry(t, set, last_set));
-    v_wrap_copy_update(t);
-    if (t->plan_sel >= 0 && hipEventQuery(t->plans[t->plan_sel].done) != hipSuccess) KT_HIP(hipStreamWaitEvent(c->stream, t->plans[t->plan_sel].done, 0));
-    if (t->side_gate && !t->pending.empty()) KT_HIP(hipStreamWaitEvent(c->stream, t->sets[t->pending.front().set].ready, 0));
+    if (t->plan_sel >= 0 && hipEventQuery(t->plans[t->plan_sel].done) != hipSuccess) { note_submit(t); KT_HIP(hipStreamWaitEvent(c->stream, t->plans[t->plan_sel].done, 0)); }
+    if (t->side_gate && !t->pending.empty()) { note_submit(t); KT_HIP(hipStreamWaitEvent(c->stream, t->sets[t->pending.front().set].ready, 0)); }
     KT_TRY(launch_setup(t, 0, nullptr, nullptr));
     t->out_speculated = !t->cfg.dynamic_cube;
     if (t->out_speculated) KT_TRY(enqueue_fusion(t, set, depth_raw, colors, t->plan_sel >= 0 ? &t->plans[t->plan_sel].plan : nullptr));
@@ -1423,6 +1480,7 @@
 {
     const size_t P = (size_t)t->cfg.cols * t->cfg.rows;
     const int slot = t->next_slot;
+    note_submit(t);
     t->next_slot = (t->next_slot + 1) % KT_NSLOTS;
     KT_HIP(hipEventSynchronize(t->slot_uploaded[slot]));
     KT_TRY(wait_frame_consumed(t, stream, t->slot_frame[slot]));
@@ -1441,6 +1499,7 @@
     KT_ARG(t && depth_host && rgb_host);
     if (t->pending.size() >= 2) { kt_set_error("kt_tracker_prefetch_frame_host: two read-ahead frames are already outstanding"); return KT_ERR_STATE; }
     KT_TRY(complete_frame(t));
+    KT_TRY(flush_owed(t));
     int slot;
     KT_TRY(stage_host_frame(t, t->pre_stream, depth_host, rgb_host, &slot));
     return prefetch_impl(t, t->depth_stage[slot], t->rgb_stage[slot], depth_host, rgb_host);
@@ -1450,18 +1509,12 @@
 {
     if (t->pending.size() >= 2) { kt_set_error("kt_tracker_prefetch_frame: two read-ahead frames are already outstanding"); return KT_ERR_STATE; }
     KT_TRY(complete_frame(t));
-    if (!t->pending.empty() && t->plans[t->frames_started % 3].ordinal != t->frames_started) KT_TRY(plan_frame(t, t->pending.front(), t->frames_started));
+    KT_TRY(flush_owed(t));
     const int set = pick_free_set(t);
     if (set < 0) { kt_set_error("kt_tracker_prefetch_frame: no free frame set"); return KT_ERR_STATE; }
     t->last_assigned = set;
-    KT_TRY(wait_frame_consumed(t, t->pre_stream, t->sets[set].user));
-    t->pre_ctx.device = t->ctx->device;
-    if (t->side_gate && t->gate_armed) {
-        KT_HIP(hipStreamWaitEvent(t->pre_stream, t->gate_ev, 0));
-    }
-    KT_TRY(build_frame_set(t, &t->pre_ctx, set, depth_raw, colors));
-    KT_HIP(hipEventRecord(t->sets[set].ready, t->pre_stream));
-    t->pending.push_back(Pending{depth_raw, colors, set, depth_host, rgb_host});
+    t->plan_owed = !t->pending.empty();
+    t->pending.push_back(Pending{depth_raw, colors, set, depth_host, rgb_host, true});
     return KT_OK;
 }
 
@@ -1471,6 +1524,7 @@
     for (const Pending& p : t->pending)
         if (p.depth_host == depth_host && p.rgb_host == rgb_host) return kt_tracker_process_frame(t, p.depth, p.rgb, timestamp);
     KT_TRY(complete_frame(t));
+    KT_TRY(flush_owed(t));
     int slot;
     KT_TRY(stage_host_frame(t, t->ctx->stream, depth_host, rgb_host, &slot));
     return kt_tracker_process_frame(t, t->depth_stage[slot], t->rgb_stage[slot], timestamp);
@@ -1479,7 +1533,7 @@
 int kt_tracker_load_trajectory(kt_tracker* t, int n, const uint64_t* utimes, const float* pose7)
 {
     KT_ARG(t && n >= 0 && (n == 0 || (utimes && pose7)));
-    KT_TRY(complete_frame(t));
+    KT_TRY(settle(t));
     t->has_trajectory = true;
     for (int i = 0; i < n; ++i) {
         std::array<float, 12> T;
@@ -1493,7 +1547,7 @@
 int kt_tracker_get_volume_basis(kt_tracker* t, float* basis)
 {
     KT_ARG(t && basis);
-    KT_TRY(complete_frame(t));
+    KT_TRY(settle(t));
     memcpy(basis, t->volume_basis, sizeof(t->volume_basis));
     return KT_OK;
 }
@@ -1501,7 +1555,7 @@
 int kt_tracker_finalise(kt_tracker* t)
 {
     KT_ARG(t);
-    KT_TRY(complete_frame(t));
+    KT_TRY(settle(t));
     v_wrap_copy_update(t);
     const int lo[3] = {0, 0, 0}, hi[3] = {t->N, t->N, t->N};
     const int mhi[3] = {t->N - 1, t->N - 1, t->N - 1};
@@ -1515,11 +1569,11 @@
     return KT_OK;
 }
 
-int kt_tracker_num_pr_samples(kt_tracker* t) { return (t && complete_frame(t) == KT_OK) ? (int)t->pr_samples.size() : -1; }
+int kt_tracker_num_pr_samples(kt_tracker* t) { return (t && settle(t) == KT_OK) ? (int)t->pr_samples.size() : -1; }
 int kt_tracker_pr_sample(kt_tracker* t, int i, uint64_t* utime, float* trans, float* rotation, int* pose_index)
 {
     KT_ARG(t && utime && trans && rotation && pose_index);
-    KT_TRY(complete_frame(t));
+    KT_TRY(settle(t));
     KT_ARG(i >= 0 && i < (int)t->pr_samples.size());
     const PrSample& ps = t->pr_samples[i];
     *utime = ps.utime;
@@ -1531,7 +1585,7 @@
 int kt_tracker_slice_pr_id(kt_tracker* t, int i, int* pr_id)
 {
     KT_ARG(t && pr_id);
-    KT_TRY(complete_frame(t));
+    KT_TRY(settle(t));
     KT_ARG(i >= 0 && i < (int)t->slices.size());
     *pr_id = t->slices[i].pr_id;
     return KT_OK;
@@ -1540,17 +1594,17 @@
 int kt_tracker_get_pose(kt_tracker* t, float* R, float* tv, float* gc)
 {
     KT_ARG(t && R && tv && gc);
-    KT_TRY(complete_frame(t));
+    KT_TRY(settle(t));
     memcpy(R, t->Rlast, sizeof(t->Rlast));
     memcpy(tv, t->tlast, sizeof(t->tlast));
     memcpy(gc, t->current_global_camera, sizeof(t->current_global_camera));
     return KT_OK;
 }
-int kt_tracker_num_poses(kt_tracker* t) { return (t && complete_frame(t) == KT_OK) ? (int)t->poses.size() : -1; }
+int kt_tracker_num_poses(kt_tracker* t) { return (t && settle(t) == KT_OK) ? (int)t->poses.size() : -1; }
 int kt_tracker_get_dense_pose(kt_tracker* t, int i, uint64_t* ts, float* pose16, int* is_loop)
 {
     KT_ARG(t);
-    KT_TRY(complete_frame(t));
+    KT_TRY(settle(t));
     KT_ARG(t && i >= 0 && i < (int)t->poses.size() && ts && pose16 && is_loop);
     *ts = t->poses[i].ts;
     memcpy(pose16, t->poses[i].pose, sizeof(t->poses[i].pose));
@@ -1560,15 +1614,15 @@
 int kt_tracker_get_voxel_wrap(kt_tracker* t, int* wrap)
 {
     KT_ARG(t && wrap);
-    KT_TRY(complete_frame(t));
+    KT_TRY(settle(t));
     memcpy(wrap, t->voxel_wrap, sizeof(t->voxel_wrap));
     return KT_OK;
 }
-int kt_tracker_num_slices(kt_tracker* t) { return (t && complete_frame(t) == KT_OK) ? (int)t->slices.size() : -1; }
+int kt_tracker_num_slices(kt_tracker* t) { return (t && settle(t) == KT_OK) ? (int)t->slices.size() : -1; }
 int kt_tracker_slice_info(kt_tracker* t, int i, size_t* n_points, int* dimension)
 {
     KT_ARG(t);
-    KT_TRY(complete_frame(t));
+    KT_TRY(settle(t));
     KT_ARG(t && i >= 0 && i < (int)t->slices.size() && n_points && dimension);
     KT_TRY(join_slice_jobs(t));
     *n_points = t->slices[i].pts.size();
@@ -1578,14 +1632,14 @@
 int kt_tracker_set_parked(kt_tracker* t, int parked)
 {
     KT_ARG(t);
-    KT_TRY(complete_frame(t));
+    KT_TRY(settle(t));
     t->parked = parked != 0;
     return KT_OK;
 }
 int kt_tracker_slice_pose(kt_tracker* t, int i, float* R, float* cam, uint64_t* ts)
 {
     KT_ARG(t);
-    KT_TRY(complete_frame(t));
+    KT_TRY(settle(t));
     KT_ARG(t && i >= 0 && i < (int)t->slices.size());
     if (R) memcpy(R, t->slices[i].R, 9 * sizeof(float));
     if (cam) memcpy(cam, t->slices[i].cam, 3 * sizeof(float));
@@ -1595,23 +1649,23 @@
 int kt_tracker_slice_points(kt_tracker* t, int i, kt_point_xyzrgb* out)
 {
     KT_ARG(t);
-    KT_TRY(complete_frame(t));
+    KT_TRY(settle(t));
     KT_ARG(t && i >= 0 && i < (int)t->slices.size() && out);
     KT_TRY(join_slice_jobs(t));
     if (!t->slices[i].pts.empty()) memcpy(out, t->slices[i].pts.data(), t->slices[i].pts.size() * sizeof(kt_point_xyzrgb));
     return KT_OK;
 }
-int16_t* kt_tracker_volume(kt_tracker* t) { return (t && complete_frame(t) == KT_OK) ? t->tsdf : nullptr; }
-uint8_t* kt_tracker_color_volume(kt_tracker* t) { return (t && complete_frame(t) == KT_OK) ? t->color : nullptr; }
-float* kt_tracker_vmap_g_prev(kt_tracker* t, int l) { return (t && l >= 0 && l < KT_LEVELS && complete_frame(t) == KT_OK) ? t->vmaps_g_prev[l] : nullptr; }
-float* kt_tracker_nmap_g_prev(kt_tracker* t, int l) { return (t && l >= 0 && l < KT_LEVELS && complete_frame(t) == KT_OK) ? t->nmaps_g_prev[l] : nullptr; }
-uint8_t* kt_tracker_vmap_curr_color(kt_tracker* t) { return (t && complete_frame(t) == KT_OK) ? t->vmap_curr_color : nullptr; }
+int16_t* kt_tracker_volume(kt_tracker* t) { return (t && settle(t) == KT_OK) ? t->tsdf : nullptr; }
+uint8_t* kt_tracker_color_volume(kt_tracker* t) { return (t && settle(t) == KT_OK) ? t->color : nullptr; }
+float* kt_tracker_vmap_g_prev(kt_tracker* t, int l) { return (t && l >= 0 && l < KT_LEVELS && settle(t) == KT_OK) ? t->vmaps_g_prev[l] : nullptr; }
+float* kt_tracker_nmap_g_prev(kt_tracker* t, int l) { return (t && l >= 0 && l < KT_LEVELS && settle(t) == KT_OK) ? t->nmaps_g_prev[l] : nullptr; }
+uint8_t* kt_tracker_vmap_curr_color(kt_tracker* t) { return (t && settle(t) == KT_OK) ? t->vmap_curr_color : nullptr; }
 float kt_tracker_trunc_dist(kt_tracker* t) { return t ? t->tranc_dist : 0.f; }
 
 int kt_tracker_enable_profiling(kt_tracker* t, int on)
 {
     KT_ARG(t);
-    KT_TRY(complete_frame(t));
+    KT_TRY(settle(t));
     KT_HIP(hipStreamSynchronize(t->ctx->stream));
     ev_collect(t);
     t->profiling = on;
@@ -1622,7 +1676,7 @@
 int kt_tracker_stage_ms(kt_tracker* t, float* ms)
 {
     KT_ARG(t && ms);
-    KT_TRY(complete_frame(t));
+    KT_TRY(settle(t));
     KT_HIP(hipStreamSynchronize(t->ctx->stream));
     ev_collect(t);
     for (int s = 0; s < ST_COUNT; ++s) ms[s] = t->stage_n[s] ? (float)(t->stage_ms_sum[s] / (double)t->stage_n[s]) : 0.f;
@@ -1637,13 +1691,14 @@
 int kt_tracker_enable_counts(kt_tracker* t, int on)
 {
     KT_ARG(t);
+    KT_TRY(settle(t));
     t->counting = on;
     return KT_OK;
 }
 int kt_tracker_debug_state(kt_tracker* t, float* out29)
 {
     KT_ARG(t && out29);
-    KT_TRY(complete_frame(t));
+    KT_TRY(settle(t));
     KT_HIP(hipStreamSynchronize(t->ctx->stream));
     KT_HIP(hipMemcpy(t->state_host, t->state_dev, sizeof(kt_track_state), hipMemcpyDeviceToHost));
     memcpy(out29, t->state_host->icp29, 29 * sizeof(float));
@@ -1652,7 +1707,7 @@
 int kt_tracker_enable_slice_stage(kt_tracker* t, int on, int weight_cull, int k)
 {
     KT_ARG(t && (!on || (k >= 1 && k <= 64)));
-    KT_TRY(complete_frame(t));
+    KT_TRY(settle(t));
     KT_TRY(join_slice_jobs(t));
     if (on && !t->slice_ws) {
         KT_TRY(kt_slice_ws_create(t->ctx, t->cloud_cap, nullptr, &t->slice_ws));
@@ -1675,7 +1730,7 @@
 int kt_tracker_slice_processed_info(kt_tracker* t, int i, long long* n_points)
 {
     KT_ARG(t && n_points);
-    KT_TRY(complete_frame(t));
+    KT_TRY(settle(t));
     KT_ARG(i >= 0 && i < (int)t->slices.size());
     KT_TRY(join_slice_jobs(t));
     *n_points = t->slices[i].has_processed ? (long long)t->slices[i].processed.size() : -1;
@@ -1684,7 +1739,7 @@
 int kt_tracker_slice_processed(kt_tracker* t, int i, kt_point_xyzrgbnormal* out)
 {
     KT_ARG(t && out);
-    KT_TRY(complete_frame(t));
+    KT_TRY(settle(t));
     KT_ARG(i >= 0 && i < (int)t->slices.size());
     KT_TRY(join_slice_jobs(t));
     KT_ARG(t->slices[i].has_processed);
@@ -1695,7 +1750,7 @@
 int kt_tracker_enable_mesh_stage(kt_tracker* t, int on, long long max_vertices, long long max_triangles)
 {
     KT_ARG(t && max_vertices >= 0 && max_triangles >= 0);
-    KT_TRY(complete_frame(t));
+    KT_TRY(settle(t));
     KT_TRY(join_slice_jobs(t));
     if (on) {
         const size_t N = (size_t)t->N;
@@ -1730,7 +1785,7 @@
 int kt_tracker_slice_mesh_info(kt_tracker* t, int i, long long* n_vertices, long long* n_triangles)
 {
     KT_ARG(t && n_vertices && n_triangles);
-    KT_TRY(complete_frame(t));
+    KT_TRY(settle(t));
     KT_ARG(i >= 0 && i < (int)t->slices.size());
     KT_TRY(join_slice_jobs(t));
     *n_vertices = t->slices[i].mesh_nv;
@@ -1740,7 +1795,7 @@
 int kt_tracker_slice_mesh(kt_tracker* t, int i, kt_mesh_vertex* vertices, uint32_t* triangles)
 {
     KT_ARG(t);
-    KT_TRY(complete_frame(t));
+    KT_TRY(settle(t));
     KT_ARG(i >= 0 && i < (int)t->slices.size());
     KT_TRY(join_slice_jobs(t));
     const Slice& s = t->slices[i];
@@ -1759,7 +1814,7 @@
 int kt_tracker_odometry_fallbacks(kt_tracker* t, long long* out)
 {
     KT_ARG(t && out);
-    KT_TRY(complete_frame(t));
+    KT_TRY(settle(t));
     *out = t->odo_fallbacks;
     return KT_OK;
 }
@@ -1767,7 +1822,7 @@
 int kt_tracker_plan_stats(kt_tracker* t, long long out2[2])
 {
     KT_ARG(t && out2);
-    KT_TRY(complete_frame(t));
+    KT_TRY(settle(t));
     out2[0] = t->plan_hits; out2[1] = t->plan_misses;
     return KT_OK;
 }
@@ -1776,7 +1831,7 @@
     KT_ARG(t);
     if (enable >= 0) t->pose_log_on = enable != 0;
     if (out12n || n_frames) {
-        KT_TRY(complete_frame(t));
+        KT_TRY(settle(t));
         const int n = (int)(t->pose_log.size() / 12);
         if (n_frames) *n_frames = n;
         if (out12n) memcpy(out12n, t->pose_log.data(), sizeof(float) * 12 * (size_t)(n < max_frames ? n : max_frames));
@@ -1804,7 +1859,7 @@
 int kt_tracker_debug_bricks(kt_tracker* t, unsigned char* out_host)
 {
     KT_ARG(t && out_host);
-    KT_TRY(complete_frame(t));
+    KT_TRY(settle(t));
     KT_HIP(hipMemcpyAsync(out_host, t->bricks, kt_brick_count(t->N), hipMemcpyDeviceToHost, t->ctx->stream));
     KT_HIP(hipStreamSynchronize(t->ctx->stream));
     return KT_OK;
@@ -1820,7 +1875,7 @@
 int kt_tracker_export_poses_device(kt_tracker* t, int k, float* dst_dev)
 {
     KT_ARG(t);
-    KT_TRY(complete_frame(t));
+    KT_TRY(settle(t));
     KT_ARG(k > 0 && dst_dev && k <= (int)t->poses.size());
     std::vector<float> tmp((size_t)k * 16);
     for (int i = 0; i < k; ++i) memcpy(&tmp[(size_t)i * 16], t->poses[t->poses.size() - k + i].pose, 16 * sizeof(float));
@@ -1833,3 +1888,7 @@
 
 extern "C" int kt_tracker_debug_icp_levels(kt_tracker* t) { return t && t->last_icp_levels ? 1 : 0; }
 extern "C" int kt_tracker_debug_side_gate(kt_tracker* t) { return t ? t->side_gate : 0; }
+extern "C" int kt_tracker_debug_odometry_position(kt_tracker* t, long long ordinal)
+{
+    return t && ordinal >= 0 && (size_t)ordinal < t->odo_pos.size() ? t->odo_pos[(size_t)ordinal] : -1;
+}
```

Measured after the change: 3955 frames/s. Within noise of the previous version (-0.1%).
